# antonilo/unsupervised_detection

Measured on AMD Instinct MI355X. Metric: frame-pairs/sec per adversarial step, DAVIS 480p batch4, 1/2/4/8 GPU, higher is better.
Workload: dtype f32

## Files before the change

include/udet_debug.h:

```cpp
#ifndef UDET_DEBUG_H
#define UDET_DEBUG_H
#include <stddef.h>
#ifdef __cplusplus
extern "C" {
#endif
void udet_debug_force_conv(int bm, int bn, int ks);
void udet_debug_conv_fp16(int on);
void udet_debug_conv_fp16_grad_scale(float s);
void udet_debug_force_wgrad(int nsplit, int dma);
int udet_debug_last_wgrad(void);
int udet_debug_last_wgrad_reduce(void);
int udet_debug_conv2d_backward_filter_ex(const float* x, int ldx, int x_coff, const float* dy, int ldy, int y_coff, const float* y_saved, int act,
                                         float alpha, const float* w, const float* b, const float* gamma, float bn_c, float* dw, float* db,
                                         float* dgamma, float* dbeta, int n, int h, int wd, int cin, int cout, int k, int stride, int dilation,
                                         int up, void* workspace, size_t workspace_bytes, void* stream);
void udet_debug_upb_min_pixels(long v);
void udet_debug_set_tuning(int on);
void udet_debug_force_pair(int on);
int udet_debug_last_pair(void);
int udet_debug_conv2d_pair(const float* xa, const float* xb, const float* wa, const float* wb, const float* ba, const float* bb, float* ya, float* yb,
                           int na, int nb, int h, int w, int cin, int cout, int k, int stride, int dilation, int act, float alpha, void* workspace,
                           size_t workspace_bytes, void* stream);
#define UDET_DEBUG_UPCONV_WSETS_OFFSET 6400
size_t udet_debug_upconv_lowres_workspace_bytes(int ldx, int cin, int cout);
int udet_debug_upconv_lowres_fwd(const float* x, int ldx, const float* w, const float* bias, int act, float alpha, float* y, int ldy, int y_coff,
                                 float* xhat, int n, int h, int wd, int cin, int cout, int split, void* workspace, size_t workspace_bytes,
                                 void* stream);
int udet_debug_upconv_lowres_bwd(const float* dy, int ldy, int y_coff, const float* w, float* dx, int ldx, float* dxhat, int n, int h, int wd,
                                 int cin, int cout, void* workspace, size_t workspace_bytes, void* stream);
int udet_debug_upconv_tables(int h, int w, int backward, int* nseg, int* seg, int* seg_tap, int* taps, int taps_cap, int* ntaps);
int udet_debug_max_segs(void);
int udet_debug_last_conv(void);
#ifdef __cplusplus
}
#endif
#endif
```

unsupervised_detection_amd/_devel.py:

```python
from __future__ import annotations

import ctypes
import os

from ._ffi import check as _check, lib as _lib

_PATH = os.path.join(os.path.dirname(os.path.abspath(__file__)), "libudet_debug.so")
if not os.path.exists(_PATH):
    raise RuntimeError(f"{_PATH} is missing: build it with `make -C unsupervised_detection_amd/csrc`")
dbg = ctypes.CDLL(_PATH, mode=ctypes.RTLD_GLOBAL)
dbg.udet_debug_force_conv.restype = None
dbg.udet_debug_force_conv.argtypes = [ctypes.c_int, ctypes.c_int, ctypes.c_int]
dbg.udet_debug_last_conv.restype = ctypes.c_int
dbg.udet_debug_last_conv.argtypes = []
dbg.udet_debug_conv_fp16.restype = None
dbg.udet_debug_conv_fp16.argtypes = [ctypes.c_int]
dbg.udet_debug_conv_fp16_grad_scale.restype = None
dbg.udet_debug_conv_fp16_grad_scale.argtypes = [ctypes.c_float]
dbg.udet_debug_force_wgrad.restype = None
dbg.udet_debug_force_wgrad.argtypes = [ctypes.c_int, ctypes.c_int]
dbg.udet_debug_upb_min_pixels.restype = None
dbg.udet_debug_upb_min_pixels.argtypes = [ctypes.c_long]
dbg.udet_debug_set_tuning.restype = None
dbg.udet_debug_set_tuning.argtypes = [ctypes.c_int]
dbg.udet_debug_last_wgrad.restype = ctypes.c_int
dbg.udet_debug_last_wgrad.argtypes = []
dbg.udet_debug_force_pair.restype = None
dbg.udet_debug_force_pair.argtypes = [ctypes.c_int]
dbg.udet_debug_last_pair.restype = ctypes.c_int
dbg.udet_debug_last_pair.argtypes = []
dbg.udet_debug_conv2d_pair.restype = ctypes.c_int
dbg.udet_debug_conv2d_pair.argtypes = [ctypes.c_void_p] * 8 + [ctypes.c_int] * 10 + [ctypes.c_float, ctypes.c_void_p, ctypes.c_size_t, ctypes.c_void_p]
dbg.udet_debug_last_wgrad_reduce.restype = ctypes.c_int
dbg.udet_debug_last_wgrad_reduce.argtypes = []
_p, _i, _f = ctypes.c_void_p, ctypes.c_int, ctypes.c_float
dbg.udet_debug_conv2d_backward_filter_ex.restype = ctypes.c_int
dbg.udet_debug_conv2d_backward_filter_ex.argtypes = ([_p, _i, _i, _p, _i, _i, _p, _i, _f, _p, _p, _p, _f, _p, _p, _p, _p] + [_i] * 9
                                                     + [_p, ctypes.c_size_t, _p])
UPCONV_WSETS_OFFSET = 6400
dbg.udet_debug_upconv_lowres_workspace_bytes.restype = ctypes.c_size_t
dbg.udet_debug_upconv_lowres_workspace_bytes.argtypes = [_i, _i, _i]
dbg.udet_debug_upconv_lowres_fwd.restype = ctypes.c_int
dbg.udet_debug_upconv_lowres_fwd.argtypes = [_p, _i, _p, _p, _i, _f, _p, _i, _i, _p] + [_i] * 6 + [_p, ctypes.c_size_t, _p]
dbg.udet_debug_upconv_lowres_bwd.restype = ctypes.c_int
dbg.udet_debug_upconv_lowres_bwd.argtypes = [_p, _i, _i, _p, _p, _i, _p] + [_i] * 5 + [_p, ctypes.c_size_t, _p]
dbg.udet_debug_upconv_tables.restype = ctypes.c_int
dbg.udet_debug_upconv_tables.argtypes = [_i, _i, _i] + [_p] * 4 + [_i, _p]
dbg.udet_debug_max_segs.restype = ctypes.c_int
dbg.udet_debug_max_segs.argtypes = []


def upconv_tables(h: int, w: int, backward: bool):
    cap = 1024
    nseg, ntaps = ctypes.c_int(0), ctypes.c_int(0)
    seg, seg_tap, taps = (ctypes.c_int * 64)(), (ctypes.c_int * 17)(), (ctypes.c_int * (3 * cap))()
    st = dbg.udet_debug_upconv_tables(h, w, 1 if backward else 0, ctypes.addressof(nseg), ctypes.addressof(seg), ctypes.addressof(seg_tap),
                                      ctypes.addressof(taps), cap, ctypes.addressof(ntaps))
    _check(st)
    ns, nt = nseg.value, ntaps.value
    return dict(nseg=ns, seg=[tuple(seg[4 * s:4 * s + 4]) for s in range(ns)], seg_tap=list(seg_tap[:ns + 1]),
                taps=[tuple(taps[3 * t:3 * t + 3]) for t in range(nt)])
```

unsupervised_detection_amd/csrc/api_plan.hip:

```cpp
#include <stdlib.h>
#include <string.h>

#include "conv_host.h"
#include "elementwise.h"
#include "plan.h"

using namespace udet;

struct udet_plan {
  Plan* p;
};

extern "C" {

int udet_plan_create(const udet_config* c, udet_plan** out) {
  if (!c || !out) { set_error("plan_create: null argument"); return UDET_ERR_ARG; }
  Config k;
  k.batch = c->batch; k.in_h = c->in_h; k.in_w = c->in_w; k.img_h = c->img_h; k.img_w = c->img_w;
  k.flow_normalizer = c->flow_normalizer; k.cbn = c->cbn; k.epsilon = c->epsilon;
  k.lr = c->lr; k.beta1 = c->beta1; k.beta2 = c->beta2; k.adam_eps = c->adam_eps; k.clip = c->clip;
  k.noise_seed = c->noise_seed;
  k.conv_fp16 = c->conv_fp16 ? 1 : 0;
  Plan* P = plan_build(k);
  if (!P) return UDET_ERR_SHAPE;
  *out = new udet_plan{P};
  return UDET_OK;
}
void udet_plan_destroy(udet_plan* h) {
  if (h) { delete h->p; delete h; }
}
size_t udet_workspace_bytes(const udet_plan* h) { return h->p->arena_floats * sizeof(float); }
int udet_plan_init(udet_plan* h, void* ws, void* stream) { return plan_init_workspace(h->p, (float*)ws, (hipStream_t)stream); }

int udet_param_count(int net) { return (net < 0 || net > 2) ? 0 : (int)net_params(net).p.size(); }
size_t udet_param_total(int net) { return (net < 0 || net > 2) ? 0 : net_params(net).total; }
int udet_param_info(int net, int i, const char** name, int* rank, int* shape, size_t* offset) {
  if (net < 0 || net > 2 || i < 0 || i >= (int)net_params(net).p.size()) { set_error("param_info: out of range"); return UDET_ERR_ARG; }
  const ParamDesc& d = net_params(net).p[i];
  *name = d.name.c_str(); *rank = d.rank; *offset = d.offset;
  for (int k = 0; k < 4; ++k) shape[k] = d.shape[k];
  return UDET_OK;
}
int udet_buffer_count(const udet_plan* h) { return (int)h->p->bufs.size(); }
int udet_buffer_info(const udet_plan* h, int i, const char** name, size_t* offset_bytes, int* dims) {
  if (i < 0 || i >= (int)h->p->bufs.size()) { set_error("buffer_info: out of range"); return UDET_ERR_ARG; }
  const Buf& b = h->p->bufs[i];
  *name = b.name.c_str(); *offset_bytes = b.off * sizeof(float);
  dims[0] = b.n; dims[1] = b.h; dims[2] = b.w; dims[3] = b.ld;
  return UDET_OK;
}
int udet_plan_set_concurrent(udet_plan* h, int on) {
  if (!h) { set_error("plan_set_concurrent: null plan"); return UDET_ERR_ARG; }
  if (on)
    if (h->p->cand.empty()) { set_error("plan_set_concurrent: the plan has no side streams"); return UDET_ERR_UNSUPPORTED; }
  h->p->concurrent = on != 0;
  return UDET_OK;
}
int udet_plan_lane_queues(udet_plan* h, void* stream, int* queue) {
  if (!h || !queue) { set_error("plan_lane_queues: null argument"); return UDET_ERR_ARG; }
  return plan_lane_queues(h->p, (hipStream_t)stream, queue);
}
int udet_plan_pin_lanes(udet_plan* h, void* stream, void* const* side_streams, int n) {
  if (!h || (n > 0 && !side_streams)) { set_error("plan_pin_lanes: null argument"); return UDET_ERR_ARG; }
  return plan_pin_lanes(h->p, (hipStream_t)stream, reinterpret_cast<hipStream_t const*>(side_streams), n);
}
long udet_fp16_overflow_count(udet_plan* h) {
  if (!h) return 0;
  (void)plan_check_overflow(h->p, true);
  return h->p->ovf_skipped;
}
long udet_get_adam_step(const udet_plan* h) {
  plan_settle_adam_step(h->p);
  return h->p->adam_t;
}
void udet_set_adam_step(udet_plan* h, long t) {
  plan_settle_adam_step(h->p);
  h->p->adam_t = t;
}

int udet_pack_pwc(udet_plan* h, const float* w_pwc, void* ws, void* stream) {
  return plan_pack_pwc(h->p, w_pwc, (float*)ws, (hipStream_t)stream);
}
int udet_pack_trainable(udet_plan* h, const float* w_gen, const float* w_rec, void* ws, void* stream) {
  return plan_pack_trainable(h->p, w_gen, w_rec, (float*)ws, (hipStream_t)stream);
}
int udet_pwc_forward(udet_plan* h, const float* img1, const float* img2, void* ws, void* stream) {
  return plan_pwc_forward(h->p, img1, img2, (float*)ws, (hipStream_t)stream);
}
int udet_forward_from_flow(udet_plan* h, int ncalls, void* ws, void* stream) {
  UDET_TRY(plan_check_overflow(h->p, false));
  if (ncalls < 0 || ncalls > 3) { set_error("forward: ncalls must be 0..3"); return UDET_ERR_ARG; }
  return plan_forward(h->p, nullptr, nullptr, ncalls, (float*)ws, (hipStream_t)stream);
}
int udet_generator_forward(udet_plan* h, void* ws, void* stream) {
  UDET_TRY(plan_generator_forward(h->p, (float*)ws, (hipStream_t)stream));
  return plan_recover_forward(h->p, 0, (float*)ws, (hipStream_t)stream);
}
int udet_generator_layers(udet_plan* h, void* ws, void* stream) {
  h->p->ev_next = 0;
  UDET_TRY(plan_generator_layers(h->p, (float*)ws, (hipStream_t)stream));
  return plan_recover_forward(h->p, 0, (float*)ws, (hipStream_t)stream);
}
int udet_recover_forward(udet_plan* h, int n, void* ws, void* stream) {
  if (n < 1 || n > 3) { set_error("recover_forward: n must be 1..3 (multiples of the plan batch)"); return UDET_ERR_ARG; }
  return plan_recover_forward(h->p, n, (float*)ws, (hipStream_t)stream, true);
}
int udet_forward(udet_plan* h, const float* img1, const float* img2, int ncalls, void* ws, void* stream) {
  UDET_TRY(plan_check_overflow(h->p, false));
  if (ncalls < 0 || ncalls > 3) { set_error("forward: ncalls must be 0..3"); return UDET_ERR_ARG; }
  if (!img1 || !img2) { set_error("forward: null image pointer"); return UDET_ERR_ARG; }
  return plan_forward(h->p, img1, img2, ncalls, (float*)ws, (hipStream_t)stream);
}
int udet_prefetch_flow(udet_plan* h, const float* img1, const float* img2, void* ws, void* stream) {
  if (!img1 || !img2) { set_error("prefetch_flow: null image pointer"); return UDET_ERR_ARG; }
  return plan_prefetch(h->p, img1, img2, (float*)ws, (hipStream_t)stream);
}
int udet_prefetch_consume(udet_plan* h, void* ws, void* stream) {
  return plan_prefetch_consume(h->p, (float*)ws, (hipStream_t)stream);
}
int udet_forward_prefetched(udet_plan* h, int ncalls, void* ws, void* stream) {
  UDET_TRY(plan_check_overflow(h->p, false));
  if (ncalls < 0 || ncalls > 3) { set_error("forward: ncalls must be 0..3"); return UDET_ERR_ARG; }
  return plan_forward(h->p, nullptr, nullptr, ncalls, (float*)ws, (hipStream_t)stream, true);
}
int udet_backward(udet_plan* h, int which, const float* w_gen, const float* w_rec, float* g_gen, float* g_rec, void* ws,
                  void* stream) {
  UDET_TRY(plan_check_overflow(h->p, false));
  if (which < 1 || which > 3) { set_error("backward: which must be 1 (generator), 2 (recover) or 3 (both)"); return UDET_ERR_ARG; }
  return plan_backward(h->p, which, w_gen, w_rec, g_gen, g_rec, (float*)ws, (hipStream_t)stream);
}
int udet_apply(udet_plan* h, int net, float* w, float* g, float* m, float* v, void* ws, void* stream) {
  return plan_apply(h->p, net, w, g, m, v, (float*)ws, (hipStream_t)stream);
}
int udet_train_step(udet_plan* h, int which, const float* img1, const float* img2, float* w_gen, float* w_rec, float* g_gen,
                    float* g_rec, float* m_gen, float* v_gen, float* m_rec, float* v_rec, void* ws, void* stream) {
  UDET_TRY(udet_pack_trainable(h, w_gen, w_rec, ws, stream));
  UDET_TRY(udet_forward(h, img1, img2, 3, ws, stream));
  UDET_TRY(udet_backward(h, which, w_gen, w_rec, g_gen, g_rec, ws, stream));
  if (which & 1) UDET_TRY(udet_apply(h, NET_GEN, w_gen, g_gen, m_gen, v_gen, ws, stream));
  if (which & 2) UDET_TRY(udet_apply(h, NET_REC, w_rec, g_rec, m_rec, v_rec, ws, stream));
  return UDET_OK;
}

int udet_autotune(udet_plan* h, const float* w_gen, const float* w_rec, float* g_gen, float* g_rec, void* ws_, void* stream) {
  Plan* P = h->p;
  float* ws = (float*)ws_;
  hipStream_t s = (hipStream_t)stream;
  if (!P->pwc_packed) { set_error("autotune: pack the PWC-Net and trainable weights first"); return UDET_ERR_ARG; }
  const size_t lo = P->packed_floats, hi = P->small_off;
  UDET_TRY(launch_fill_uniform(ws + lo, (long)(hi - lo), 0x5eedull, -0.5f, 0.5f, s));
  const size_t img_floats = (size_t)P->cfg.batch * P->cfg.in_h * P->cfg.in_w * 3;
  if (P->wgrad_floats < 2 * img_floats) { set_error("autotune: workspace too small for the probe images"); return UDET_ERR_ARG; }
  const float* img1 = ws + P->wgrad_off[0];
  const float* img2 = img1 + img_floats;
  const bool was_concurrent = P->concurrent;
  P->concurrent = false;
  conv_set_tuning(1);
  wgrad_set_tuning(1);
  int rc = udet_forward(h, img1, img2, 3, ws_, stream);
  if (rc == UDET_OK) rc = udet_backward(h, 3, w_gen, w_rec, g_gen, g_rec, ws_, stream);
  conv_set_tuning(0);
  wgrad_set_tuning(0);
  P->concurrent = was_concurrent;
  UDET_HIP(hipMemsetAsync(ws + lo, 0, (hi - lo) * sizeof(float), s));
  UDET_HIP(hipStreamSynchronize(s));
  return rc;
}
int udet_tuned_shapes(void) { return tuned_shapes(); }
int udet_tune_save(const char* path) {
  FILE* f = path ? fopen(path, "w") : nullptr;
  if (!f) { set_error("tune_save: cannot open %s", path ? path : "(null)"); return UDET_ERR_ARG; }
  fprintf(f, "udet-tune 2 abi %d\n", UDET_TUNE_ABI);
  tune_dump(f);
  fclose(f);
  return UDET_OK;
}
int udet_tune_load(const char* path) {
  FILE* f = path ? fopen(path, "r") : nullptr;
  if (!f) { set_error("tune_load: cannot open %s", path ? path : "(null)"); return UDET_ERR_ARG; }
  char line[256];
  int n = 0, ver = 0, abi = -1;
  if (!fgets(line, sizeof(line), f) || sscanf(line, "udet-tune %d abi %d", &ver, &abi) != 2 || ver != 2 || abi != UDET_TUNE_ABI) {
    fclose(f);
    set_error("tune_load: %s is not a udet-tune 2 file of this build (abi %d)", path, UDET_TUNE_ABI);
    return UDET_ERR_ARG;
  }
  while (fgets(line, sizeof(line), f)) n += tune_put_line(line) ? 1 : 0;
  fclose(f);
  return n;
}

int udet_profile_begin(udet_plan* h) {
  for (auto* r : h->p->prof) delete r;
  h->p->prof.clear();
  h->p->profiling = true;
  return UDET_OK;
}
int udet_profile_end(udet_plan* h, double* out, int ncat, void* stream) {
  Plan* P = h->p;
  P->profiling = false;
  g_launch_sink = nullptr;
  UDET_HIP(hipStreamSynchronize((hipStream_t)stream));
  for (int i = 0; i < ncat * 5; ++i) out[i] = 0.0;
  FILE* dump = nullptr;
  if (const char* path = getenv("UDET_PROF_DUMP")) dump = fopen(path, "a");
  for (auto* r : P->prof) {
    float wall = 0.f;
    (void)hipEventElapsedTime(&wall, r->a, r->b);
    double kern = 0.0;
    std::string each;
    for (int k = 0; k < r->sink.n; ++k) {
      float ms = 0.f;
      if (hipEventElapsedTime(&ms, r->kev[2 * k], r->kev[2 * k + 1]) == hipSuccess) kern += ms;
      char buf[32];
      snprintf(buf, sizeof(buf), "%s%.1f", k ? "+" : "", ms * 1e3f);
      each += buf;
      (void)hipEventDestroy(r->kev[2 * k]);
      (void)hipEventDestroy(r->kev[2 * k + 1]);
    }
    if (r->sink.n == 0) kern = wall;
    if (dump)
      fprintf(dump, "%d,%s,%.4f,%.4f,%.4f,%.4f,%d,%s,%.4f\n", r->cat, r->name.c_str(), kern, r->flops * 1e-9, r->bytes * 1e-6, wall, r->sink.n,
              each.c_str(), r->flops * r->mfma_scale * 1e-9);
    if (r->cat < ncat) {
      out[r->cat * 5 + 0] += 1.0;
      out[r->cat * 5 + 1] += kern;
      out[r->cat * 5 + 2] += r->flops;
      out[r->cat * 5 + 3] += r->bytes;
      out[r->cat * 5 + 4] += wall;
    }
    (void)hipEventDestroy(r->a);
    (void)hipEventDestroy(r->b);
    delete r;
  }
  if (dump) fclose(dump);
  P->prof.clear();
  return UDET_OK;
}

int udet_generator_backward(udet_plan* h, const float* w_gen, float* g_gen, void* ws, void* stream) {
  if (!w_gen || !g_gen) { set_error("generator_backward: null argument"); return UDET_ERR_ARG; }
  return plan_backward(h->p, 1, w_gen, nullptr, g_gen, nullptr, (float*)ws, (hipStream_t)stream);
}
int udet_recover_backward(udet_plan* h, const float* w_rec, float* g_rec, void* ws, void* stream) {
  if (!w_rec || !g_rec) { set_error("recover_backward: null argument"); return UDET_ERR_ARG; }
  return plan_backward(h->p, 2, nullptr, w_rec, nullptr, g_rec, (float*)ws, (hipStream_t)stream);
}
int udet_grad_absmean(udet_plan* h, int net, const float* g, float* out2, void* ws_, void* stream) {
  if ((net != NET_GEN && net != NET_REC) || !g || !out2) { set_error("grad_absmean: net must be 1 or 2, g / out2 non-null"); return UDET_ERR_ARG; }
  Plan* P = h->p;
  float* ws = (float*)ws_;
  const NetParams& np = net_params(net);
  const long* tab = reinterpret_cast<const long*>(ws + P->seg_off[net]);
  return launch_grad_absmean(g, tab, tab + np.p.size(), (int)np.p.size(), ws + P->small_off + 2048, 1e-5f, out2, (hipStream_t)stream);
}
int udet_stream_wait_grads(udet_plan* h, int net, void* stream) {
  if (net != NET_GEN && net != NET_REC) { set_error("stream_wait_grads: net must be 1 or 2"); return UDET_ERR_ARG; }
  if (!h->p->grad_ev[net]) { set_error("stream_wait_grads: no udet_backward has produced that gradient yet"); return UDET_ERR_ARG; }
  UDET_HIP(hipStreamWaitEvent((hipStream_t)stream, h->p->grad_ev[net], 0));
  return UDET_OK;
}
int udet_tune_rejected(void) { return conv_tune_rejected(); }

}
```

unsupervised_detection_amd/csrc/devel/api_debug.hip:

```cpp
#include <string.h>

#include <vector>

#include "../../../include/udet_debug.h"
#include "../conv_host.h"
#include "../plan_run.h"

using namespace udet;

extern "C" {
int udet_debug_last_conv(void) { return conv_last_config(); }
void udet_debug_force_conv(int bm, int bn, int ks) { conv_force_config(bm, bn, ks); }
void udet_debug_conv_fp16(int on) { conv_debug_f16(on); }
void udet_debug_conv_fp16_grad_scale(float s) { conv_debug_f16_grad_scale(s); }
void udet_debug_force_wgrad(int nsplit, int dma) { wgrad_force(nsplit, dma); }
int udet_debug_last_wgrad(void) { return wgrad_last_config(); }
int udet_debug_last_wgrad_reduce(void) { return wgrad_last_reduce(); }
int udet_debug_conv2d_backward_filter_ex(const float* x, int ldx, int x_coff, const float* dy, int ldy, int y_coff, const float* y_saved, int act,
                                         float alpha, const float* w, const float* b, const float* gamma, float bn_c, float* dw, float* db,
                                         float* dgamma, float* dbeta, int n, int h, int wd, int cin, int cout, int k, int stride, int dilation,
                                         int up, void* workspace, size_t workspace_bytes, void* stream_) {
  hipStream_t stream = (hipStream_t)stream_;
  if (!x || !dy || !dw || n < 1 || h < 1 || wd < 1 || cin < 1 || cout < 1 || k < 1 || k * k > UDET_MAX_TAPS || dilation < 1 ||
      (stride != 1 && stride != 2) || up < 0 || up > 2) {
    set_error("debug_backward_filter_ex: bad argument");
    return UDET_ERR_ARG;
  }
  if (ldx % 4 || x_coff % 4 || ldy % 4 || y_coff % 4) {
    set_error("debug_backward_filter_ex: ldx=%d x_coff=%d ldy=%d y_coff=%d must be multiples of 4", ldx, x_coff, ldy, y_coff);
    return UDET_ERR_ALIGN;
  }
  if (x_coff < 0 || y_coff < 0 || x_coff + round_up(cin, 4) > ldx || y_coff + round_up(cout, 4) > ldy) {
    set_error("debug_backward_filter_ex: channel window outside the buffer (x %d+%d of %d, dy %d+%d of %d)", x_coff, cin, ldx, y_coff, cout, ldy);
    return UDET_ERR_SHAPE;
  }
  if (gamma && (!w || !b || !db || !dgamma || !dbeta)) {
    set_error("debug_backward_filter_ex: a BN-folded layer needs w, b, db, dgamma and dbeta");
    return UDET_ERR_ARG;
  }
  if (up == 2 && (!gamma || y_saved || k != 3 || stride != 1 || dilation != 1)) {
    set_error("debug_backward_filter_ex: the class-structured form is a BN-folded 3x3 stride-1 layer on dU");
    return UDET_ERR_ARG;
  }
  if (!workspace || (reinterpret_cast<uintptr_t>(workspace) & 63) || workspace_bytes < 128 * sizeof(float)) {
    set_error("debug_backward_filter_ex: workspace must be 64-byte aligned and hold the zero block");
    return UDET_ERR_ARG;
  }
  float* zero = reinterpret_cast<float*>(workspace);
  const int us = up ? 1 : 0;
  WgradParams p;
  memset(&p, 0, sizeof(p));
  p.x = x; p.ldx = ldx; p.x_coff = x_coff; p.N = n; p.Cin = cin;
  p.dy = dy; p.ldy = ldy; p.y_coff = y_coff; p.Cout = cout;
  if (y_saved && act != UDET_ACT_NONE) { p.ya = y_saved; p.yact = act; p.yalpha = alpha; }
  p.dw = dw; p.db = db;
  p.partial = zero + 64; p.partial_floats = workspace_bytes / sizeof(float) - 64;
  p.zero16 = zero;
  p.f16_yscale = conv_debug_f16_grad_scale_now();
  if (gamma) { p.w = w; p.b = b; p.gamma = gamma; p.dgamma = dgamma; p.dbeta = dbeta; p.bn_c = bn_c; }
  ConvParams g;
  memset(&g, 0, sizeof(g));
  conv_setup_fwd(g, n, h << us, wd << us, k, k, stride, dilation);
  p.H = h << us; p.W = wd << us; p.up_shift = us;
  p.OH = g.OH; p.OW = g.OW; p.isy = p.isx = stride;
  p.ntaps = g.ntaps;
  memcpy(p.taps, g.taps, sizeof(g.taps));
  UDET_HIP(hipMemsetAsync(zero, 0, 64 * sizeof(float), stream));
  if (up == 2) return launch_wgrad_up_T(p, h, wd, stream);
  return launch_wgrad_T(p, k * k, stream);
}
void udet_debug_upb_min_pixels(long v) { plan_debug_upb_min_pixels(v); }
void udet_debug_force_pair(int on) { conv_force_pair(on); }
int udet_debug_last_pair(void) { return conv_last_pair(); }
int udet_debug_conv2d_pair(const float* xa, const float* xb, const float* wa, const float* wb, const float* ba, const float* bb, float* ya, float* yb,
                           int na, int nb, int h, int w, int cin, int cout, int k, int stride, int dilation, int act, float alpha, void* workspace,
                           size_t workspace_bytes, void* stream_) {
  hipStream_t stream = (hipStream_t)stream_;
  if (cin % 8 != 0 || k * k > UDET_MAX_TAPS) { set_error("debug_conv2d_pair: cin must be a multiple of 8"); return UDET_ERR_SHAPE; }
  const int kc = cin, ldw = round_up(cout, 4);
  const size_t wfl = ((size_t)k * k * kc * ldw + 63) & ~(size_t)63, part_fl = (size_t)4 << 20, zero_fl = 64 + UDET_MAX_TICKETS;
  if (workspace_bytes < (2 * wfl + part_fl + zero_fl) * sizeof(float)) { set_error("debug_conv2d_pair: workspace too small"); return UDET_ERR_ARG; }
  float* wpa = reinterpret_cast<float*>(workspace);
  float* wpb = wpa + wfl;
  float* part = wpb + wfl;
  float* zero = part + part_fl;
  UDET_HIP(hipMemsetAsync(zero, 0, zero_fl * sizeof(float), stream));
  UDET_TRY(launch_pack_weights(wa, wpa, k * k, cin, cout, kc, ldw, kc, 0, 0, nullptr, stream));
  UDET_TRY(launch_pack_weights(wb, wpb, k * k, cin, cout, kc, ldw, kc, 0, 0, nullptr, stream));
  ConvParams p[2];
  for (int i = 0; i < 2; ++i) {
    memset(&p[i], 0, sizeof(ConvParams));
    conv_setup_fwd(p[i], i ? nb : na, h, w, k, k, stride, dilation);
    p[i].x = i ? xb : xa; p[i].ldx = cin; p[i].wp = i ? wpb : wpa; p[i].Kc = kc; p[i].ldw = ldw; p[i].bias = i ? bb : ba;
    p[i].y = i ? yb : ya; p[i].ldy = cout; p[i].Cout = cout; p[i].act = act; p[i].alpha = alpha;
    p[i].partial = part; p[i].partial_cap = part_fl; p[i].zero16 = zero; p[i].tickets = reinterpret_cast<int*>(zero + 64);
  }
  return launch_conv_pair(p[0], p[1], stream);
}
}
namespace {
enum { UPC_TICKETS = 64, UPC_JOBS = UPC_TICKETS + UDET_MAX_TICKETS, UPC_JOBS_CAP = 192, UPC_TAB = UPC_JOBS + UPC_JOBS_CAP, UPC_TAB_CAP = 2048,
       UPC_WSETS = UPC_TAB + UPC_TAB_CAP, UPC_MIN_SLAB = 1 << 20 };
static_assert(UPC_WSETS == UDET_DEBUG_UPCONV_WSETS_OFFSET && UPC_WSETS % 64 == 0 && 8 * sizeof(PackJob) <= UPC_JOBS_CAP * sizeof(float), "workspace layout");
size_t upc_align64(size_t v) { return (v + 63) & ~(size_t)63; }
int upc_kct(int cout) { return round_up(cout, cout <= 4 ? 4 : 8); }
size_t upc_floats(int kc, int ldw) { return UPC_WSETS + upc_align64((size_t)4 * 36 * kc * ldw) + UPC_MIN_SLAB; }
int upc_check(const char* who, const void* a, const void* b, const void* c, const void* d, int n, int h, int wd, int cin, int cout, void* workspace,
              size_t workspace_bytes, size_t need_floats) {
  if (!a || !b || !c || !d || n < 1 || cin < 1 || cout < 1) { set_error("%s: bad argument", who); return UDET_ERR_ARG; }
  if (h < 2 || wd < 2) { set_error("%s: the source grid %d x %d must be at least 2 x 2 (one interior row / column and the last one)", who, h, wd); return UDET_ERR_SHAPE; }
  if ((long)n * (2 * h) * (2 * wd) >= (1L << 28)) { set_error("%s: grid too large", who); return UDET_ERR_SHAPE; }
  if (!workspace || (reinterpret_cast<uintptr_t>(workspace) & 63) || workspace_bytes < need_floats * sizeof(float)) {
    set_error("%s: workspace must be 64-byte aligned and hold %zu bytes", who, need_floats * sizeof(float));
    return UDET_ERR_ARG;
  }
  return UDET_OK;
}
int upc_stage(const Layer::SegLaunch& tab, const std::vector<PackJob>& jobs, const float* w, float* ws, hipStream_t stream) {
  if (tab.taps.size() * sizeof(ConvTap) > UPC_TAB_CAP * sizeof(float) || jobs.size() * sizeof(PackJob) > UPC_JOBS_CAP * sizeof(float)) {
    set_error("debug_upconv_lowres: table larger than its workspace slot");
    return UDET_ERR_ARG;
  }
  UDET_HIP(hipMemsetAsync(ws, 0, UPC_JOBS * sizeof(float), stream));
  UDET_HIP(hipMemcpyAsync(ws + UPC_JOBS, jobs.data(), jobs.size() * sizeof(PackJob), hipMemcpyHostToDevice, stream));
  UDET_HIP(hipMemcpyAsync(ws + UPC_TAB, tab.taps.data(), tab.taps.size() * sizeof(ConvTap), hipMemcpyHostToDevice, stream));
  return launch_pack_jobs(reinterpret_cast<const PackJob*>(ws + UPC_JOBS), (int)jobs.size(), w, ws, BN_C, stream);
}
UpbLane upc_lane(float* ws, size_t ws_floats, size_t sets_floats) {
  const size_t off = UPC_WSETS + upc_align64(sets_floats);
  return UpbLane{ws + off, ws_floats - off, ws, reinterpret_cast<int*>(ws + UPC_TICKETS), 0};
}
}
extern "C" {

size_t udet_debug_upconv_lowres_workspace_bytes(int ldx, int cin, int cout) {
  if (ldx < 1 || cin < 1 || cout < 1) return 0;
  const size_t f = upc_floats(ldx, round_up(cout, 4)), b = upc_floats(upc_kct(cout), round_up(cin, 4));
  return (f > b ? f : b) * sizeof(float);
}
int udet_debug_max_segs(void) { return UDET_MAX_SEGS; }

int udet_debug_upconv_lowres_fwd(const float* x, int ldx, const float* w, const float* bias, int act, float alpha, float* y, int ldy, int y_coff,
                                 float* xhat, int n, int h, int wd, int cin, int cout, int split, void* workspace, size_t workspace_bytes,
                                 void* stream_) {
  hipStream_t stream = (hipStream_t)stream_;
  const char* who = "debug_upconv_lowres_fwd";
  if (act != UDET_ACT_NONE && act != UDET_ACT_LEAKY && act != UDET_ACT_ELU) { set_error("%s: bad argument", who); return UDET_ERR_ARG; }
  if (ldx % 4 || ldy % 4 || y_coff % 4) { set_error("%s: ldx=%d ldy=%d y_coff=%d must be multiples of 4", who, ldx, ldy, y_coff); return UDET_ERR_ALIGN; }
  if (ldx < 4 || ldy < 4 || cin > ldx || y_coff < 0 || (cout >= 1 && y_coff + cout > ldy)) {
    set_error("%s: channel window outside the buffer (x %d of %d, y %d+%d of %d)", who, cin, ldx, y_coff, cout, ldy);
    return UDET_ERR_SHAPE;
  }
  if (split && cout > 16) { set_error("%s: the split form is the plan's for cout <= 16 only", who); return UDET_ERR_ARG; }
  Layer L;
  L.cin = cin; L.cout = cout;
  L.Kc = ldx; L.ldw = round_up(cout, 4);
  L.k_split = round_up(cin, cin <= 4 ? 4 : 8); L.k_gap = 0;
  L.upb = true; L.upb_bwd = false; L.upb_split = split != 0;
  L.wupb_off = UPC_WSETS;
  const size_t sets = (size_t)4 * 36 * L.Kc * L.ldw;
  UDET_TRY(upc_check(who, x, w, y, xhat, n, h, wd, cin, cout, workspace, workspace_bytes, upc_floats(L.Kc, L.ldw)));
  float* ws = reinterpret_cast<float*>(workspace);
  build_upb_launches(L, h, wd);
  std::vector<PackJob> jobs;
  PackJob base;
  memset(&base, 0, sizeof(base));
  base.gamma_off = base.beta_off = -1;
  upb_pack_jobs(L, base, jobs);
  int st = upc_stage(L.upb_f, jobs, w, ws, stream);
  if (st == UDET_OK) {
    UpbFwd a;
    a.N = n; a.h = h; a.w = wd;
    a.src = x; a.xhat = xhat; a.ld = ldx;
    a.wsets = ws + L.wupb_off; a.Kc = L.Kc; a.ldw = L.ldw; a.bias = bias;
    a.y = y; a.ldy = ldy; a.y_coff = y_coff; a.cout = cout; a.act = act; a.alpha = alpha;
    a.tab = &L.upb_f; a.tab_dev = reinterpret_cast<const ConvTap*>(ws + UPC_TAB); a.split = L.upb_split;
    a.lane = upc_lane(ws, workspace_bytes / sizeof(float), sets);
    st = upb_forward(a, stream);
  }
  (void)hipStreamSynchronize(stream);
  return st;
}

int udet_debug_upconv_lowres_bwd(const float* dy, int ldy, int y_coff, const float* w, float* dx, int ldx, float* dxhat, int n, int h, int wd,
                                 int cin, int cout, void* workspace, size_t workspace_bytes, void* stream_) {
  hipStream_t stream = (hipStream_t)stream_;
  const char* who = "debug_upconv_lowres_bwd";
  if (ldx % 4 || ldy % 4 || y_coff % 4) { set_error("%s: ldx=%d ldy=%d y_coff=%d must be multiples of 4", who, ldx, ldy, y_coff); return UDET_ERR_ALIGN; }
  const int kct = cout >= 1 ? upc_kct(cout) : 0;
  if (ldx < 4 || ldy < 4 || cin > ldx || y_coff < 0 || y_coff + kct > ldy) {
    set_error("%s: channel window outside the buffer (dy %d+%d of %d, dx %d of %d)", who, y_coff, kct, ldy, cin, ldx);
    return UDET_ERR_SHAPE;
  }
  Layer L;
  L.cin = cin; L.cout = cout;
  L.Kc = ldx; L.ldw = round_up(cout, 4);
  L.k_split = round_up(cin, cin <= 4 ? 4 : 8); L.k_gap = 0;
  L.KcT = kct; L.ldwT = round_up(cin, 4);
  L.upb = true; L.upb_bwd = true;
  L.wupbT_off = UPC_WSETS;
  const size_t sets = (size_t)4 * 36 * L.KcT * L.ldwT;
  UDET_TRY(upc_check(who, dy, w, dx, dxhat, n, h, wd, cin, cout, workspace, workspace_bytes, upc_floats(L.KcT, L.ldwT)));
  float* ws = reinterpret_cast<float*>(workspace);
  build_upb_launches(L, h, wd);
  std::vector<PackJob> all, jobs;
  PackJob base;
  memset(&base, 0, sizeof(base));
  base.gamma_off = base.beta_off = -1;
  upb_pack_jobs(L, base, all);
  for (const PackJob& j : all)
    if (j.mode == 10) jobs.push_back(j);
  int st = upc_stage(L.upb_b, jobs, w, ws, stream);
  if (st == UDET_OK) {
    UpbBwd a;
    a.N = n; a.h = h; a.w = wd;
    a.du = dy; a.lddu = ldy; a.du_coff = y_coff;
    a.wsetsT = ws + L.wupbT_off; a.KcT = L.KcT; a.ldwT = L.ldwT; a.cout = cout;
    a.dxhat = dxhat; a.dsrc = dx; a.ld = ldx; a.cin = cin;
    a.tab = &L.upb_b; a.tab_dev = reinterpret_cast<const ConvTap*>(ws + UPC_TAB);
    a.lane = upc_lane(ws, workspace_bytes / sizeof(float), sets);
    a.f16_xscale = conv_debug_f16_grad_scale_now();
    st = upb_dgrad(a, stream);
  }
  (void)hipStreamSynchronize(stream);
  return st;
}

int udet_debug_upconv_tables(int h, int w, int backward, int* nseg, int* seg, int* seg_tap, int* taps, int taps_cap, int* ntaps) {
  if (!nseg || !seg || !seg_tap || !taps || !ntaps || taps_cap < 0) { set_error("debug_upconv_tables: bad argument"); return UDET_ERR_ARG; }
  if (h < 2 || w < 2) { set_error("debug_upconv_tables: the source grid %d x %d must be at least 2 x 2", h, w); return UDET_ERR_SHAPE; }
  Layer L;
  build_upb_launches(L, h, w);
  const Layer::SegLaunch& g = backward ? L.upb_b : L.upb_f;
  *nseg = g.nseg;
  *ntaps = (int)g.taps.size();
  if (*ntaps > taps_cap) { set_error("debug_upconv_tables: %d taps, room for %d", *ntaps, taps_cap); return UDET_ERR_ARG; }
  for (int s = 0; s < g.nseg; ++s) {
    seg[4 * s] = g.seg[s].oy; seg[4 * s + 1] = g.seg[s].ox; seg[4 * s + 2] = g.seg[s].h; seg[4 * s + 3] = g.seg[s].w;
    seg_tap[s] = g.seg_tap[s];
  }
  seg_tap[g.nseg] = g.seg_tap[g.nseg];
  for (int t = 0; t < *ntaps; ++t) { taps[3 * t] = g.taps[t].dy; taps[3 * t + 1] = g.taps[t].dx; taps[3 * t + 2] = g.taps[t].widx; }
  return UDET_OK;
}

void udet_debug_set_tuning(int on) {
  conv_set_tuning(on);
  wgrad_set_tuning(on);
}
}
```

unsupervised_detection_amd/csrc/elementwise.h:

```cpp
#pragma once
#include "common.h"
namespace udet {
int launch_resize_bilinear_fwd(const float* x, int ldx, int x_coff, int N, int H, int W, float* y, int ldy, int y_coff,
                               int OH, int OW, int C, float mul, float div, hipStream_t s);
int launch_resize_bilinear_bwd(const float* dy, int ldy, int y_coff, int N, int OH, int OW, float* dx, int ldx, int x_coff,
                               int H, int W, int C, int accumulate, hipStream_t s);
int launch_upb_ring(const float* x, int ld, int N, int H, int W, float* xh, hipStream_t s);
int launch_upb_ring_fold(const float* dxh, int ld, int N, int H, int W, float* dx, hipStream_t s);
int launch_share_samples(float* buf, long P, int ld, int coff, int C, int copies, hipStream_t s);
int launch_fold_samples(float* buf, long P, int ld, int coff, int C, int copies, hipStream_t s);
int launch_emit_du(const float* d, const float* a, float* u, long P, int ld, int coff, int C, int act, float alpha, hipStream_t s);
int launch_pool2x2_sum(const float* du, float* dx, int N, int H, int W, int C, hipStream_t s);
int launch_pack_pwc_input(const float* i1, const float* i2, float* x8, long P, hipStream_t s);
int launch_gen_input(const float* img, const float* f, double* part, float* gin, int B, long HW, hipStream_t s);
size_t flow_stats_doubles(int B);
int launch_mask_rec_inputs(const float* logits, const float* f, float* mask, float* fin, long P, int ncalls, hipStream_t s);
int launch_pack_imgin(const float* img, float* imgin, long P, int ncalls, hipStream_t s);
int launch_losses(const float* f, const float* mask, const float* pred, long HW, int B, float cbn, float eps,
                  float num_pixels, float* part, float* losses, float* coef, float* sums, hipStream_t s);
size_t loss_part_floats(int B);
int launch_rec_loss_bwd(const float* f, const float* mask, const float* pred, float* dpred, long BHW, float cbn,
                        float inv_np, hipStream_t s);
int launch_gen_loss_bwd(const float* f, const float* mask, const float* pred, const float* coef, float* dpred,
                        float* dmask, long HW, int B, float cbn, hipStream_t s);
int launch_mask_bwd(const float* dmask, const float* dfin, const float* f, const float* mask, float* dlogits, long P,
                    hipStream_t s);
int launch_grad_absmean(const float* g, const long* seg_off, const long* seg_len, int nvars, float* vmean, float thresh,
                        float* out, hipStream_t s);
int launch_adam(float* w, float* g, float* m, float* v, long n, float lr_t, float b1, float b2, float eps, float clip,
                const float* flag, uint64_t seed, uint64_t step, hipStream_t s, int mode = 0, const int* skip = nullptr);
int launch_nonfinite_count(const float* g, long n, int* out, hipStream_t s);
int launch_flow_normalize(const float* f, double* part, float* out, int B, long HW, hipStream_t s);
int launch_charbonnier(const float* gt, const float* pred, const float* mask, int mc, int B, long HW, float cbn, float* part,
                       float* out, hipStream_t s);
int launch_crop_flip_resize(const void* src, int src_u8, int nearest, int N, int H, int W, int C, const int* prm, float* dst, int OH,
                            int OW, float div, float add, hipStream_t s);
int launch_crop_flip_resize_ragged(const void* src, int src_u8, int nearest, int N, int C, const long long* offsets, const int* hw,
                                   const int* prm, float* dst, int OH, int OW, float div, float add, hipStream_t s);
int launch_mask_stats(const float* pred, const float* gt, int N, int H, int W, float threshold, float gt_threshold, double* out,
                      hipStream_t s);
int launch_boundary_stats(const float* pred, const float* gt, const double* stats8, int N, int H, int W, float threshold,
                          float gt_threshold, int radius, unsigned long long* counts4, unsigned char* bmap_pred,
                          unsigned char* bmap_gt, hipStream_t s);
size_t restore_workspace_bytes(int n);
int launch_restore_masks_ragged(const float* masks, int n, int mh, int mw, const long long* offsets, const int* tab, const int* coef,
                                int max_h, int max_w, unsigned char* out, int* amax, unsigned char* binary, double threshold,
                                void* workspace, hipStream_t s);
size_t components_workspace_bytes(size_t total_pixels, int n);
int launch_select_components_ragged(const unsigned char* binary, const unsigned char* gt, int n, const long long* offsets, const int* hw,
                                    int max_h, int max_w, size_t total_pixels, int connectivity, int mode, int* labels,
                                    unsigned char* selected, long long* info, void* workspace, hipStream_t s);
size_t component_boxes_workspace_bytes(size_t total_pixels, int n);
int launch_component_boxes_ragged(const int* labels, const unsigned char* score, int n, const long long* offsets, const int* hw, int max_h,
                                  int max_w, size_t total_pixels, int min_area, int k, long long* dets, long long* counts, void* workspace,
                                  hipStream_t s);
int launch_draw_boxes_ragged(unsigned char* rgb, int n, const long long* offsets, const int* hw, const long long* dets,
                             const long long* counts, int k, int thickness, unsigned colour, hipStream_t s);
size_t link_detections_workspace_bytes(size_t total_pixels, int carry_h, int carry_w);
int launch_link_detections_ragged(const int* labels, int n, const long long* offsets, const int* hw, int max_h, int max_w,
                                  size_t total_pixels, const long long* dets, const long long* counts, int k, const int* link,
                                  const int* carry_labels, int carry_h, int carry_w, const long long* carry_dets,
                                  const long long* carry_counts, const int* carry_ids, const int* carry_next_id, int min_iou_permille,
                                  long long* inter, int* match, int* ids, int* linked, int* seq_tracks, int* next_id, void* workspace,
                                  hipStream_t s);
size_t link_detections_gap_workspace_bytes(size_t total_pixels, int m, int hist_h, int hist_w);
int launch_link_detections_gap_ragged(const int* labels, int n, const long long* offsets, const int* hw, int max_h, int max_w,
                                      size_t total_pixels, const long long* dets, const long long* counts, int k, const int* link,
                                      int max_gap, int m, const int* hist_labels, int hist_h, int hist_w, const long long* hist_dets,
                                      const long long* hist_counts, const int* hist_ids, int* hist_open, const int* hist_next_id,
                                      int min_iou_permille, long long* inter, int* match, int* ids, int* linked, int* seq_tracks,
                                      int* next_id, long long* gap_inter, int* back, int* prev, int* open, void* workspace,
                                      hipStream_t s);
int launch_draw_track_boxes_ragged(unsigned char* rgb, int n, const long long* offsets, const int* hw, const long long* dets,
                                   const long long* counts, int k, const int* ids, int thickness, const unsigned* palette,
                                   int palette_size, hipStream_t s);
int launch_fill_uniform(float* x, long n, uint64_t seed, float lo, float hi, hipStream_t s);
int launch_axpy(const float* x, float* y, long n, float a, int accumulate, hipStream_t s);
}
```

unsupervised_detection_amd/csrc/elementwise.hip:

```cpp
#include "common.h"
#include "elementwise.h"

namespace udet {

static inline int grid_for(long total, int cap = 4096) {
  long nb = (total + 255) / 256;
  if (nb > cap) nb = cap;
  if (nb < 1) nb = 1;
  return (int)nb;
}

template <typename T>
__device__ __forceinline__ T wave_sum(T v) {
#pragma unroll
  for (int o = 32; o > 0; o >>= 1) v += __shfl_down(v, o, 64);
  return v;
}
template <typename T>
__device__ __forceinline__ T block_sum(T v, T* sm ) {
  v = wave_sum(v);
  __syncthreads();
  if ((threadIdx.x & 63) == 0) sm[threadIdx.x >> 6] = v;
  __syncthreads();
  return sm[0] + sm[1] + sm[2] + sm[3];
}

__device__ __forceinline__ void legacy_coord(int i, float scale, int in, int& lo, int& hi, float& t) {
  const float src = (float)i * scale;
  lo = (int)src;
  hi = min(lo + 1, in - 1);
  t = src - (float)lo;
}

__global__ __launch_bounds__(256) void resize_bilinear_fwd_kernel(const float* __restrict__ x, int ldx, int x_coff, int N,
                                                                  int H, int W, float* __restrict__ y, int ldy, int y_coff,
                                                                  int OH, int OW, int C, float mul, float div) {
  const float sy = (float)H / (float)OH, sx = (float)W / (float)OW;
  const long total = (long)N * OH * OW * C;
  for (long e = (long)blockIdx.x * 256 + threadIdx.x; e < total; e += (long)gridDim.x * 256) {
    const int c = (int)(e % C);
    const long pix = e / C;
    const int ox = (int)(pix % OW), oy = (int)((pix / OW) % OH), n = (int)(pix / ((long)OW * OH));
    int y0, y1, x0, x1;
    float ty, tx;
    legacy_coord(oy, sy, H, y0, y1, ty);
    legacy_coord(ox, sx, W, x0, x1, tx);
    const float* b = x + x_coff + c;
    const float tl = b[(((long)n * H + y0) * W + x0) * ldx], tr = b[(((long)n * H + y0) * W + x1) * ldx];
    const float bl = b[(((long)n * H + y1) * W + x0) * ldx], br = b[(((long)n * H + y1) * W + x1) * ldx];
    const float top = tl + (tr - tl) * tx, bot = bl + (br - bl) * tx;
    float v = top + (bot - top) * ty;
    v = v * mul;
    if (div != 1.f) v = v / div;
    y[pix * ldy + y_coff + c] = v;
  }
}
template <typename T, int NEAREST>
__global__ __launch_bounds__(256) void crop_flip_resize_kernel(const T* __restrict__ src, int N, int H, int W, int C,
                                                               const int* __restrict__ prm, float* __restrict__ dst, int OH, int OW,
                                                               float div, float add) {
  const long total = (long)N * OH * OW * C;
  for (long e = (long)blockIdx.x * 256 + threadIdx.x; e < total; e += (long)gridDim.x * 256) {
    const int c = (int)(e % C);
    const long pix = e / C;
    const int ox = (int)(pix % OW), oy = (int)((pix / OW) % OH), n = (int)(pix / ((long)OW * OH));
    int y0 = 0, x0 = 0, ch = H, cw = W, flr = 0, ftd = 0;
    if (prm) { y0 = prm[n * 6]; x0 = prm[n * 6 + 1]; ch = prm[n * 6 + 2]; cw = prm[n * 6 + 3]; flr = prm[n * 6 + 4]; ftd = prm[n * 6 + 5]; }
    const float sy = (float)ch / (float)OH, sx = (float)cw / (float)OW;
    auto tap = [&](int cy, int cx) -> float {
      int yy = y0 + cy, xx = x0 + cx;
      if (ftd) yy = H - 1 - yy;
      if (flr) xx = W - 1 - xx;
      float v = (float)src[(((long)n * H + yy) * W + xx) * C + c];
      if (div != 1.f) v = v / div;
      return v + add;
    };
    float v;
    if (NEAREST) {
      const int cy = min((int)floorf((float)oy * sy), ch - 1), cx = min((int)floorf((float)ox * sx), cw - 1);
      v = tap(cy, cx);
    } else {
      int ly, hy, lx, hx;
      float ty, tx;
      legacy_coord(oy, sy, ch, ly, hy, ty);
      legacy_coord(ox, sx, cw, lx, hx, tx);
      const float tl = tap(ly, lx), tr = tap(ly, hx), bl = tap(hy, lx), br = tap(hy, hx);
      const float top = tl + (tr - tl) * tx, bot = bl + (br - bl) * tx;
      v = top + (bot - top) * ty;
    }
    dst[e] = v;
  }
}
int launch_crop_flip_resize(const void* src, int src_u8, int nearest, int N, int H, int W, int C, const int* prm, float* dst, int OH,
                            int OW, float div, float add, hipStream_t s) {
  const long total = (long)N * OH * OW * C;
  const dim3 g(grid_for(total, 8192)), b(256);
  if (src_u8 && nearest) hipLaunchKernelGGL((crop_flip_resize_kernel<unsigned char, 1>), g, b, 0, s, (const unsigned char*)src, N, H, W, C, prm, dst, OH, OW, div, add);
  else if (src_u8) hipLaunchKernelGGL((crop_flip_resize_kernel<unsigned char, 0>), g, b, 0, s, (const unsigned char*)src, N, H, W, C, prm, dst, OH, OW, div, add);
  else if (nearest) hipLaunchKernelGGL((crop_flip_resize_kernel<float, 1>), g, b, 0, s, (const float*)src, N, H, W, C, prm, dst, OH, OW, div, add);
  else hipLaunchKernelGGL((crop_flip_resize_kernel<float, 0>), g, b, 0, s, (const float*)src, N, H, W, C, prm, dst, OH, OW, div, add);
  UDET_HIP(hipGetLastError());
  return UDET_OK;
}

template <typename T, int NEAREST>
__global__ __launch_bounds__(256) void crop_flip_resize_ragged_kernel(const T* __restrict__ src, int N, int C,
                                                                      const long long* __restrict__ offsets, const int* __restrict__ hw,
                                                                      const int* __restrict__ prm, float* __restrict__ dst, int OH,
                                                                      int OW, float div, float add) {
  const long npix = (long)OH * OW;
  for (int n = blockIdx.y; n < N; n += gridDim.y) {
    const T* __restrict__ img = src + offsets[n];
    const int H = hw[n * 2], W = hw[n * 2 + 1];
    int y0 = 0, x0 = 0, ch = H, cw = W, flr = 0, ftd = 0;
    if (prm) { y0 = prm[n * 6]; x0 = prm[n * 6 + 1]; ch = prm[n * 6 + 2]; cw = prm[n * 6 + 3]; flr = prm[n * 6 + 4]; ftd = prm[n * 6 + 5]; }
    const float sy = (float)ch / (float)OH, sx = (float)cw / (float)OW;
    float* __restrict__ out = dst + (long)n * npix * C;
    for (long pix = (long)blockIdx.x * 256 + threadIdx.x; pix < npix; pix += (long)gridDim.x * 256) {
      const int ox = (int)(pix % OW), oy = (int)(pix / OW);
      auto tap = [&](int cy, int cx, int c) -> float {
        int yy = y0 + cy, xx = x0 + cx;
        if (ftd) yy = H - 1 - yy;
        if (flr) xx = W - 1 - xx;
        float v = (float)img[((long)yy * W + xx) * C + c];
        if (div != 1.f) v = v / div;
        return v + add;
      };
      if (NEAREST) {
        const int cy = min((int)floorf((float)oy * sy), ch - 1), cx = min((int)floorf((float)ox * sx), cw - 1);
        for (int c = 0; c < C; ++c) out[pix * C + c] = tap(cy, cx, c);
      } else {
        int ly, hy, lx, hx;
        float ty, tx;
        legacy_coord(oy, sy, ch, ly, hy, ty);
        legacy_coord(ox, sx, cw, lx, hx, tx);
        for (int c = 0; c < C; ++c) {
          const float tl = tap(ly, lx, c), tr = tap(ly, hx, c), bl = tap(hy, lx, c), br = tap(hy, hx, c);
          const float top = tl + (tr - tl) * tx, bot = bl + (br - bl) * tx;
          out[pix * C + c] = top + (bot - top) * ty;
        }
      }
    }
  }
}
int launch_crop_flip_resize_ragged(const void* src, int src_u8, int nearest, int N, int C, const long long* offsets, const int* hw,
                                   const int* prm, float* dst, int OH, int OW, float div, float add, hipStream_t s) {
  const int gy = N < 65535 ? N : 65535;
  const dim3 g(grid_for((long)OH * OW, 1024), gy), b(256);
  if (src_u8 && nearest) hipLaunchKernelGGL((crop_flip_resize_ragged_kernel<unsigned char, 1>), g, b, 0, s, (const unsigned char*)src, N, C, offsets, hw, prm, dst, OH, OW, div, add);
  else if (src_u8) hipLaunchKernelGGL((crop_flip_resize_ragged_kernel<unsigned char, 0>), g, b, 0, s, (const unsigned char*)src, N, C, offsets, hw, prm, dst, OH, OW, div, add);
  else if (nearest) hipLaunchKernelGGL((crop_flip_resize_ragged_kernel<float, 1>), g, b, 0, s, (const float*)src, N, C, offsets, hw, prm, dst, OH, OW, div, add);
  else hipLaunchKernelGGL((crop_flip_resize_ragged_kernel<float, 0>), g, b, 0, s, (const float*)src, N, C, offsets, hw, prm, dst, OH, OW, div, add);
  UDET_HIP(hipGetLastError());
  return UDET_OK;
}

__global__ __launch_bounds__(256) void resize_bilinear_fwd4_kernel(const float* __restrict__ x, int ldx, int x_coff, int N, int H,
                                                                   int W, float* __restrict__ y, int ldy, int y_coff, int OH,
                                                                   int OW, int C4, float mul, float div) {
  const float sy = (float)H / (float)OH, sx = (float)W / (float)OW;
  const long total = (long)N * OH * OW * C4;
  for (long e = (long)blockIdx.x * 256 + threadIdx.x; e < total; e += (long)gridDim.x * 256) {
    const int c4 = (int)(e % C4);
    const long pix = e / C4;
    const int ox = (int)(pix % OW), oy = (int)((pix / OW) % OH), n = (int)(pix / ((long)OW * OH));
    int y0, y1, x0, x1;
    float ty, tx;
    legacy_coord(oy, sy, H, y0, y1, ty);
    legacy_coord(ox, sx, W, x0, x1, tx);
    const float* b = x + x_coff + c4 * 4;
    const float4 tl = *reinterpret_cast<const float4*>(b + (((long)n * H + y0) * W + x0) * ldx);
    const float4 tr = *reinterpret_cast<const float4*>(b + (((long)n * H + y0) * W + x1) * ldx);
    const float4 bl = *reinterpret_cast<const float4*>(b + (((long)n * H + y1) * W + x0) * ldx);
    const float4 br = *reinterpret_cast<const float4*>(b + (((long)n * H + y1) * W + x1) * ldx);
    auto lerp = [&](float a, float bq, float c, float d) {
      const float top = a + (bq - a) * tx, bot = c + (d - c) * tx;
      float v = (top + (bot - top) * ty) * mul;
      if (div != 1.f) v = v / div;
      return v;
    };
    float4 o;
    o.x = lerp(tl.x, tr.x, bl.x, br.x);
    o.y = lerp(tl.y, tr.y, bl.y, br.y);
    o.z = lerp(tl.z, tr.z, bl.z, br.z);
    o.w = lerp(tl.w, tr.w, bl.w, br.w);
    *reinterpret_cast<float4*>(y + pix * ldy + y_coff + c4 * 4) = o;
  }
}
int launch_resize_bilinear_fwd(const float* x, int ldx, int x_coff, int N, int H, int W, float* y, int ldy, int y_coff,
                               int OH, int OW, int C, float mul, float div, hipStream_t s) {
  if (C % 4 == 0 && ldx % 4 == 0 && ldy % 4 == 0 && x_coff % 4 == 0 && y_coff % 4 == 0 &&
      !((reinterpret_cast<uintptr_t>(x) | reinterpret_cast<uintptr_t>(y)) & 15)) {
    const long total4 = (long)N * OH * OW * (C / 4);
    hipLaunchKernelGGL(resize_bilinear_fwd4_kernel, dim3(grid_for(total4, 8192)), dim3(256), 0, s, x, ldx, x_coff, N, H, W, y, ldy,
                       y_coff, OH, OW, C / 4, mul, div);
    UDET_HIP(hipGetLastError());
    return UDET_OK;
  }
  const long total = (long)N * OH * OW * C;
  hipLaunchKernelGGL(resize_bilinear_fwd_kernel, dim3(grid_for(total)), dim3(256), 0, s, x, ldx, x_coff, N, H, W, y, ldy,
                     y_coff, OH, OW, C, mul, div);
  UDET_HIP(hipGetLastError());
  return UDET_OK;
}

__device__ __forceinline__ float legacy_weight(int o, float scale, int in, int i) {
  int lo, hi;
  float t;
  legacy_coord(o, scale, in, lo, hi, t);
  float w = 0.f;
  if (lo == i) w += 1.f - t;
  if (hi == i) w += t;
  return w;
}
__global__ __launch_bounds__(256) void resize_bilinear_bwd_kernel(const float* __restrict__ dy, int ldy, int y_coff, int N,
                                                                  int OH, int OW, float* __restrict__ dx, int ldx,
                                                                  int x_coff, int H, int W, int C, int accumulate) {
  const float sy = (float)H / (float)OH, sx = (float)W / (float)OW;
  const float isy = (float)OH / (float)H, isx = (float)OW / (float)W;
  const long total = (long)N * H * W * C;
  for (long e = (long)blockIdx.x * 256 + threadIdx.x; e < total; e += (long)gridDim.x * 256) {
    const int c = (int)(e % C);
    const long pix = e / C;
    const int ix = (int)(pix % W), iy = (int)((pix / W) % H), n = (int)(pix / ((long)W * H));
    const int oy_lo = max(0, (int)floorf((float)(iy - 1) * isy) - 1), oy_hi = min(OH - 1, (int)ceilf((float)(iy + 1) * isy) + 1);
    const int ox_lo = max(0, (int)floorf((float)(ix - 1) * isx) - 1), ox_hi = min(OW - 1, (int)ceilf((float)(ix + 1) * isx) + 1);
    float acc = 0.f;
    for (int oy = oy_lo; oy <= oy_hi; ++oy) {
      const float wy = legacy_weight(oy, sy, H, iy);
      if (wy == 0.f) continue;
      for (int ox = ox_lo; ox <= ox_hi; ++ox) {
        const float wx = legacy_weight(ox, sx, W, ix);
        if (wx == 0.f) continue;
        acc += wy * wx * dy[(((long)n * OH + oy) * OW + ox) * ldy + y_coff + c];
      }
    }
    float* d = dx + pix * ldx + x_coff + c;
    *d = accumulate ? *d + acc : acc;
  }
}
__global__ __launch_bounds__(256) void resize2x_bwd4_kernel(const float* __restrict__ dy, int ldy, int y_coff, int N, int H, int W,
                                                            float* __restrict__ dx, int ldx, int x_coff, int C4, int accumulate) {
  const int OH = 2 * H, OW = 2 * W;
  const long total = (long)N * H * W * C4;
  for (long e = (long)blockIdx.x * 256 + threadIdx.x; e < total; e += (long)gridDim.x * 256) {
    const int c4 = (int)(e % C4);
    const long pix = e / C4;
    const int ix = (int)(pix % W), iy = (int)((pix / W) % H), n = (int)(pix / ((long)W * H));
    float wy[3], wx[3];
    wy[0] = iy > 0 ? 0.5f : 0.f; wy[1] = 1.f; wy[2] = iy == H - 1 ? 1.f : 0.5f;
    wx[0] = ix > 0 ? 0.5f : 0.f; wx[1] = 1.f; wx[2] = ix == W - 1 ? 1.f : 0.5f;
    float4 acc = make_float4(0.f, 0.f, 0.f, 0.f);
#pragma unroll
    for (int a = 0; a < 3; ++a) {
      const int oy = 2 * iy - 1 + a;
      if (oy < 0) continue;
#pragma unroll
      for (int b = 0; b < 3; ++b) {
        const int ox = 2 * ix - 1 + b;
        if (ox < 0) continue;
        const float w = wy[a] * wx[b];
        const float4 g = *reinterpret_cast<const float4*>(dy + (((long)n * OH + oy) * OW + ox) * ldy + y_coff + c4 * 4);
        acc.x += w * g.x; acc.y += w * g.y; acc.z += w * g.z; acc.w += w * g.w;
      }
    }
    float4* d = reinterpret_cast<float4*>(dx + pix * ldx + x_coff + c4 * 4);
    if (accumulate) { const float4 o = *d; acc.x += o.x; acc.y += o.y; acc.z += o.z; acc.w += o.w; }
    *d = acc;
  }
}
int launch_resize_bilinear_bwd(const float* dy, int ldy, int y_coff, int N, int OH, int OW, float* dx, int ldx, int x_coff,
                               int H, int W, int C, int accumulate, hipStream_t s) {
  if (OH == 2 * H && OW == 2 * W && C % 4 == 0 && ldx % 4 == 0 && ldy % 4 == 0 && x_coff % 4 == 0 && y_coff % 4 == 0 &&
      !((reinterpret_cast<uintptr_t>(dx) | reinterpret_cast<uintptr_t>(dy)) & 15)) {
    const long total4 = (long)N * H * W * (C / 4);
    hipLaunchKernelGGL(resize2x_bwd4_kernel, dim3(grid_for(total4, 8192)), dim3(256), 0, s, dy, ldy, y_coff, N, H, W, dx, ldx, x_coff,
                       C / 4, accumulate);
    UDET_HIP(hipGetLastError());
    return UDET_OK;
  }
  const long total = (long)N * H * W * C;
  hipLaunchKernelGGL(resize_bilinear_bwd_kernel, dim3(grid_for(total)), dim3(256), 0, s, dy, ldy, y_coff, N, OH, OW, dx,
                     ldx, x_coff, H, W, C, accumulate);
  UDET_HIP(hipGetLastError());
  return UDET_OK;
}

__global__ __launch_bounds__(256) void pool2x2_sum_kernel(const float* __restrict__ du, float* __restrict__ dx, int N, int H,
                                                          int W, int C) {
  const int c4n = C >> 2;
  const long total = (long)N * H * W * c4n;
  for (long e = (long)blockIdx.x * 256 + threadIdx.x; e < total; e += (long)gridDim.x * 256) {
    const int c4 = (int)(e % c4n);
    const long pix = e / c4n;
    const int x = (int)(pix % W), y = (int)((pix / W) % H), n = (int)(pix / ((long)W * H));
    const float* b = du + ((((long)n * 2 * H + 2 * y) * 2 * W) + 2 * x) * C + c4 * 4;
    const float4 a0 = *reinterpret_cast<const float4*>(b), a1 = *reinterpret_cast<const float4*>(b + C);
    const float4 a2 = *reinterpret_cast<const float4*>(b + (long)2 * W * C), a3 = *reinterpret_cast<const float4*>(b + (long)2 * W * C + C);
    float4 o;
    o.x = (a0.x + a1.x) + (a2.x + a3.x);
    o.y = (a0.y + a1.y) + (a2.y + a3.y);
    o.z = (a0.z + a1.z) + (a2.z + a3.z);
    o.w = (a0.w + a1.w) + (a2.w + a3.w);
    *reinterpret_cast<float4*>(dx + pix * C + c4 * 4) = o;
  }
}
int launch_pool2x2_sum(const float* du, float* dx, int N, int H, int W, int C, hipStream_t s) {
  hipLaunchKernelGGL(pool2x2_sum_kernel, dim3(grid_for((long)N * H * W * (C / 4))), dim3(256), 0, s, du, dx, N, H, W, C);
  UDET_HIP(hipGetLastError());
  return UDET_OK;
}

__global__ __launch_bounds__(256) void emit_du_kernel(const float* __restrict__ d, const float* __restrict__ a,
                                                      float* __restrict__ u, long P, int ld, int coff, int C, int act,
                                                      float alpha) {
  const long total = P * C;
  for (long e = (long)blockIdx.x * 256 + threadIdx.x; e < total; e += (long)gridDim.x * 256) {
    const long pix = e / C;
    const long o = pix * ld + coff + (e - pix * C);
    u[o] = d[o] * act_dfo(a[o], act, alpha);
  }
}
int launch_emit_du(const float* d, const float* a, float* u, long P, int ld, int coff, int C, int act, float alpha, hipStream_t s) {
  hipLaunchKernelGGL(emit_du_kernel, dim3(grid_for(P * C)), dim3(256), 0, s, d, a, u, P, ld, coff, C, act, alpha);
  UDET_HIP(hipGetLastError());
  return UDET_OK;
}

template <int V, bool FOLD>
__global__ __launch_bounds__(256) void share_fold_kernel(float* __restrict__ buf, long P, int ld, int coff, int C, int copies) {
  const int CV = C / V;
  const long total = P * CV;
  for (long e = (long)blockIdx.x * 256 + threadIdx.x; e < total; e += (long)gridDim.x * 256) {
    const long pix = e / CV;
    const long o = pix * ld + coff + (e - pix * CV) * V;
    if (V == 4) {
      float4 v = *reinterpret_cast<const float4*>(buf + o);
      for (int k = 1; k < copies; ++k) {
        float4* q = reinterpret_cast<float4*>(buf + o + (long)k * P * ld);
        if (FOLD) {
          const float4 w = *q;
          v.x += w.x; v.y += w.y; v.z += w.z; v.w += w.w;
        } else {
          *q = v;
        }
      }
      if (FOLD) *reinterpret_cast<float4*>(buf + o) = v;
    } else {
      float v = buf[o];
      for (int k = 1; k < copies; ++k) {
        if (FOLD) v += buf[o + (long)k * P * ld];
        else buf[o + (long)k * P * ld] = v;
      }
      if (FOLD) buf[o] = v;
    }
  }
}
static int launch_share_fold(float* buf, long P, int ld, int coff, int C, int copies, bool fold, hipStream_t s) {
  if (copies < 2 || C < 1) return UDET_OK;
  const bool v4 = (ld % 4 == 0) && (coff % 4 == 0) && (C % 4 == 0);
  const long n = P * (v4 ? C / 4 : C);
  if (v4) {
    if (fold) hipLaunchKernelGGL((share_fold_kernel<4, true>), dim3(grid_for(n)), dim3(256), 0, s, buf, P, ld, coff, C, copies);
    else hipLaunchKernelGGL((share_fold_kernel<4, false>), dim3(grid_for(n)), dim3(256), 0, s, buf, P, ld, coff, C, copies);
  } else {
    if (fold) hipLaunchKernelGGL((share_fold_kernel<1, true>), dim3(grid_for(n)), dim3(256), 0, s, buf, P, ld, coff, C, copies);
    else hipLaunchKernelGGL((share_fold_kernel<1, false>), dim3(grid_for(n)), dim3(256), 0, s, buf, P, ld, coff, C, copies);
  }
  UDET_HIP(hipGetLastError());
  return UDET_OK;
}
int launch_share_samples(float* buf, long P, int ld, int coff, int C, int copies, hipStream_t s) {
  return launch_share_fold(buf, P, ld, coff, C, copies, false, s);
}
int launch_fold_samples(float* buf, long P, int ld, int coff, int C, int copies, hipStream_t s) {
  return launch_share_fold(buf, P, ld, coff, C, copies, true, s);
}

__global__ __launch_bounds__(256) void pack_pwc_input_kernel(const float* __restrict__ i1, const float* __restrict__ i2,
                                                             float* __restrict__ x8, long P) {
  for (long e = (long)blockIdx.x * 256 + threadIdx.x; e < 2 * P; e += (long)gridDim.x * 256) {
    const float* s = e < P ? i1 + e * 3 : i2 + (e - P) * 3;
    float4 a = make_float4(s[0] + 0.5f, s[1] + 0.5f, s[2] + 0.5f, 0.f);
    *reinterpret_cast<float4*>(x8 + e * 4) = a;
  }
}
int launch_pack_pwc_input(const float* i1, const float* i2, float* x8, long P, hipStream_t s) {
  hipLaunchKernelGGL(pack_pwc_input_kernel, dim3(grid_for(2 * P)), dim3(256), 0, s, i1, i2, x8, P);
  UDET_HIP(hipGetLastError());
  return UDET_OK;
}

#define FS_BLOCKS 32
__global__ __launch_bounds__(256) void flow_stats_kernel(const float* __restrict__ f, long HW, double* __restrict__ part) {
  __shared__ double sm[4];
  const int n = blockIdx.y;
  double s0 = 0, s1 = 0, q0 = 0, q1 = 0;
  for (long p = (long)blockIdx.x * 256 + threadIdx.x; p < HW; p += (long)gridDim.x * 256) {
    const float2 v = *reinterpret_cast<const float2*>(f + ((long)n * HW + p) * 2);
    s0 += v.x; s1 += v.y;
    q0 += (double)v.x * v.x; q1 += (double)v.y * v.y;
  }
  s0 = block_sum(s0, sm); s1 = block_sum(s1, sm); q0 = block_sum(q0, sm); q1 = block_sum(q1, sm);
  if (threadIdx.x == 0) {
    double* o = part + ((long)n * FS_BLOCKS + blockIdx.x) * 4;
    o[0] = s0; o[1] = s1; o[2] = q0; o[3] = q1;
  }
}
__global__ __launch_bounds__(256) void pack_gen_input_kernel(const float* __restrict__ img, const float* __restrict__ f,
                                                             const double* __restrict__ part, float* __restrict__ gin,
                                                             long HW) {
  __shared__ float st[4];
  const int n = blockIdx.y;
  if (threadIdx.x < 2) {
    double s = 0, q = 0;
    for (int b = 0; b < FS_BLOCKS; ++b) {
      s += part[((long)n * FS_BLOCKS + b) * 4 + threadIdx.x];
      q += part[((long)n * FS_BLOCKS + b) * 4 + 2 + threadIdx.x];
    }
    const double mean = s / (double)HW, var = q / (double)HW - mean * mean;
    st[threadIdx.x] = (float)mean;
    st[2 + threadIdx.x] = sqrtf((float)var);
  }
  __syncthreads();
  const float m0 = st[0], m1 = st[1], d0 = st[2], d1 = st[3];
  for (long p = (long)blockIdx.x * 256 + threadIdx.x; p < HW; p += (long)gridDim.x * 256) {
    const long q = (long)n * HW + p;
    const float2 v = *reinterpret_cast<const float2*>(f + q * 2);
    *reinterpret_cast<float4*>(gin + q * 8) = make_float4(img[q * 3], img[q * 3 + 1], img[q * 3 + 2], (v.x - m0) / d0);
    *reinterpret_cast<float4*>(gin + q * 8 + 4) = make_float4((v.y - m1) / d1, 0.f, 0.f, 0.f);
  }
}
int launch_gen_input(const float* img, const float* f, double* part, float* gin, int B, long HW, hipStream_t s) {
  hipLaunchKernelGGL(flow_stats_kernel, dim3(FS_BLOCKS, B), dim3(256), 0, s, f, HW, part);
  hipLaunchKernelGGL(pack_gen_input_kernel, dim3(grid_for(HW, 256), B), dim3(256), 0, s, img, f, part, gin, HW);
  UDET_HIP(hipGetLastError());
  return UDET_OK;
}
size_t flow_stats_doubles(int B) { return (size_t)B * FS_BLOCKS * 4; }
__global__ __launch_bounds__(256) void flow_normalize_kernel(const float* __restrict__ f, const double* __restrict__ part,
                                                             float* __restrict__ out, long HW) {
  __shared__ float st[4];
  const int n = blockIdx.y;
  if (threadIdx.x < 2) {
    double s = 0, q = 0;
    for (int b = 0; b < FS_BLOCKS; ++b) {
      s += part[((long)n * FS_BLOCKS + b) * 4 + threadIdx.x];
      q += part[((long)n * FS_BLOCKS + b) * 4 + 2 + threadIdx.x];
    }
    const double mean = s / (double)HW, var = q / (double)HW - mean * mean;
    st[threadIdx.x] = (float)mean;
    st[2 + threadIdx.x] = sqrtf((float)var);
  }
  __syncthreads();
  const float m0 = st[0], m1 = st[1], d0 = st[2], d1 = st[3];
  for (long p = (long)blockIdx.x * 256 + threadIdx.x; p < HW; p += (long)gridDim.x * 256) {
    const long q = (long)n * HW + p;
    const float2 v = *reinterpret_cast<const float2*>(f + q * 2);
    *reinterpret_cast<float2*>(out + q * 2) = make_float2((v.x - m0) / d0, (v.y - m1) / d1);
  }
}
int launch_flow_normalize(const float* f, double* part, float* out, int B, long HW, hipStream_t s) {
  hipLaunchKernelGGL(flow_stats_kernel, dim3(FS_BLOCKS, B), dim3(256), 0, s, f, HW, part);
  hipLaunchKernelGGL(flow_normalize_kernel, dim3(grid_for(HW, 256), B), dim3(256), 0, s, f, part, out, HW);
  UDET_HIP(hipGetLastError());
  return UDET_OK;
}

__global__ __launch_bounds__(256) void mask_rec_inputs_kernel(const float* __restrict__ logits ,
                                                              const float* __restrict__ f, float* __restrict__ mask,
                                                              float* __restrict__ fin, long P, int ncalls) {
  for (long q = (long)blockIdx.x * 256 + threadIdx.x; q < P; q += (long)gridDim.x * 256) {
    const float l0 = logits[q * 8] / 10.f, l1 = logits[q * 8 + 1] / 10.f;
    const float mx = fmaxf(l0, l1);
    const float e0 = expf(l0 - mx), e1 = expf(l1 - mx);
    const float m = e0 / (e0 + e1);
    mask[q] = m;
    const float cm = 1.f - m;
    const float2 v = *reinterpret_cast<const float2*>(f + q * 2);
    const float a0 = 1.f - m, a1 = 1.f - cm;
    if (ncalls > 0) {
      *reinterpret_cast<float4*>(fin + q * 4) = make_float4(v.x * a0, v.y * a0, 1.f, a0);
    }
    if (ncalls > 1) {
      *reinterpret_cast<float4*>(fin + (P + q) * 4) = make_float4(v.x * a1, v.y * a1, 1.f, a1);
    }
    if (ncalls > 2) {
      *reinterpret_cast<float4*>(fin + (2 * P + q) * 4) = make_float4(0.f, 0.f, 1.f, 0.f);
    }
  }
}
int launch_mask_rec_inputs(const float* logits, const float* f, float* mask, float* fin, long P, int ncalls, hipStream_t s) {
  hipLaunchKernelGGL(mask_rec_inputs_kernel, dim3(grid_for(P)), dim3(256), 0, s, logits, f, mask, fin, P, ncalls);
  UDET_HIP(hipGetLastError());
  return UDET_OK;
}
__global__ __launch_bounds__(256) void pack_imgin_kernel(const float* __restrict__ img, float* __restrict__ imgin, long P,
                                                         int ncalls) {
  for (long q = (long)blockIdx.x * 256 + threadIdx.x; q < P; q += (long)gridDim.x * 256) {
    const float4 im = make_float4(img[q * 3], img[q * 3 + 1], img[q * 3 + 2], 0.f);
    for (int k = 0; k < ncalls; ++k) *reinterpret_cast<float4*>(imgin + (k * P + q) * 4) = im;
  }
}
int launch_pack_imgin(const float* img, float* imgin, long P, int ncalls, hipStream_t s) {
  hipLaunchKernelGGL(pack_imgin_kernel, dim3(grid_for(P)), dim3(256), 0, s, img, imgin, P, ncalls);
  UDET_HIP(hipGetLastError());
  return UDET_OK;
}

__device__ __forceinline__ float charb(float e, float cbn) {
  const float s = e * e + 0.001f * 0.001f;
  return cbn == 0.5f ? sqrtf(s) : powf(s, cbn);
}
__device__ __forceinline__ float charb_d(float e, float cbn) {
  const float s = e * e + 0.001f * 0.001f;
  return cbn == 0.5f ? e / sqrtf(s) : cbn * powf(s, cbn - 1.f) * 2.f * e;
}
#define LS_BLOCKS 64
__global__ __launch_bounds__(256) void loss_sums_kernel(const float* __restrict__ f, const float* __restrict__ mask,
                                                        const float* __restrict__ pred , long HW, int B,
                                                        float cbn, float* __restrict__ part ) {
  __shared__ float sm[4];
  const int n = blockIdx.y;
  float R = 0, Rc = 0, Pp = 0, Dr = 0, Dc = 0;
  for (long p = (long)blockIdx.x * 256 + threadIdx.x; p < HW; p += (long)gridDim.x * 256) {
    const long q = (long)n * HW + p;
    const float2 fl = *reinterpret_cast<const float2*>(f + q * 2);
    const float2 a = *reinterpret_cast<const float2*>(pred + q * 2);
    const float2 b = *reinterpret_cast<const float2*>(pred + ((long)B * HW + q) * 2);
    const float2 c = *reinterpret_cast<const float2*>(pred + ((long)2 * B * HW + q) * 2);
    const float m = mask[q], cm = 1.f - m;
    const float pa = charb(fl.x - a.x, cbn) + charb(fl.y - a.y, cbn);
    const float pb = charb(fl.x - b.x, cbn) + charb(fl.y - b.y, cbn);
    const float pc = charb(fl.x - c.x, cbn) + charb(fl.y - c.y, cbn);
    R += pa * m; Rc += pb * cm; Pp += pc; Dr += pc * m; Dc += pc * cm;
  }
  R = block_sum(R, sm); Rc = block_sum(Rc, sm); Pp = block_sum(Pp, sm); Dr = block_sum(Dr, sm); Dc = block_sum(Dc, sm);
  if (threadIdx.x == 0) {
    float* o = part + ((long)n * LS_BLOCKS + blockIdx.x) * 5;
    o[0] = R; o[1] = Rc; o[2] = Pp; o[3] = Dr; o[4] = Dc;
  }
}
__global__ void loss_finish_kernel(const float* __restrict__ part, int B, float eps, float num_pixels,
                                   float* __restrict__ losses, float* __restrict__ coef, float* __restrict__ sums) {
  if (threadIdx.x != 0 || blockIdx.x != 0) return;
  float red = 0.f, redc = 0.f, rs = 0.f;
  for (int b = 0; b < B; ++b) {
    float v[5] = {0, 0, 0, 0, 0};
    for (int k = 0; k < LS_BLOCKS; ++k)
      for (int j = 0; j < 5; ++j) v[j] += part[((long)b * LS_BLOCKS + k) * 5 + j];
    const float D = v[3] + eps, Dc = v[4] + eps;
    red += 1.f - v[0] / D;
    redc += 1.f - v[1] / Dc;
    rs += v[0] + v[1] + v[2];
    coef[b * 4 + 0] = -1.f / (B * D);
    coef[b * 4 + 1] = v[0] / (B * D * D);
    coef[b * 4 + 2] = -1.f / (B * Dc);
    coef[b * 4 + 3] = v[1] / (B * Dc * Dc);
    for (int j = 0; j < 5; ++j) sums[b * 5 + j] = v[j];
    if (b == 0) { losses[4] = v[0]; losses[5] = v[1]; losses[6] = D; losses[7] = Dc; }
  }
  red /= B; redc /= B;
  losses[0] = red + redc;
  losses[1] = rs / num_pixels;
  losses[2] = red;
  losses[3] = redc;
}
int launch_losses(const float* f, const float* mask, const float* pred, long HW, int B, float cbn, float eps,
                  float num_pixels, float* part, float* losses, float* coef, float* sums, hipStream_t s) {
  hipLaunchKernelGGL(loss_sums_kernel, dim3(LS_BLOCKS, B), dim3(256), 0, s, f, mask, pred, HW, B, cbn, part);
  hipLaunchKernelGGL(loss_finish_kernel, dim3(1), dim3(64), 0, s, part, B, eps, num_pixels, losses, coef, sums);
  UDET_HIP(hipGetLastError());
  return UDET_OK;
}
size_t loss_part_floats(int B) { return (size_t)B * LS_BLOCKS * 5; }

__global__ __launch_bounds__(256) void charbonnier_sum_kernel(const float* __restrict__ gt, const float* __restrict__ pred,
                                                              const float* __restrict__ mask, int mc, long HW, float cbn,
                                                              float* __restrict__ part ) {
  __shared__ float sm[4];
  const int n = blockIdx.y;
  float acc = 0.f;
  for (long p = (long)blockIdx.x * 256 + threadIdx.x; p < HW; p += (long)gridDim.x * 256) {
    const long q = (long)n * HW + p;
    const float2 a = *reinterpret_cast<const float2*>(gt + q * 2);
    const float2 b = *reinterpret_cast<const float2*>(pred + q * 2);
    const float m0 = mask ? mask[q * mc] : 1.f, m1 = mask ? mask[q * mc + (mc - 1)] : 1.f;
    acc += charb(a.x - b.x, cbn) * m0 + charb(a.y - b.y, cbn) * m1;
  }
  acc = block_sum(acc, sm);
  if (threadIdx.x == 0) part[(long)n * LS_BLOCKS + blockIdx.x] = acc;
}
__global__ void charbonnier_finish_kernel(const float* __restrict__ part, int B, float* __restrict__ out) {
  const int b = blockIdx.x * blockDim.x + threadIdx.x;
  if (b >= B) return;
  float v = 0.f;
  for (int k = 0; k < LS_BLOCKS; ++k) v += part[(long)b * LS_BLOCKS + k];
  out[b] = v;
}
int launch_charbonnier(const float* gt, const float* pred, const float* mask, int mc, int B, long HW, float cbn, float* part,
                       float* out, hipStream_t s) {
  hipLaunchKernelGGL(charbonnier_sum_kernel, dim3(LS_BLOCKS, B), dim3(256), 0, s, gt, pred, mask, mc, HW, cbn, part);
  hipLaunchKernelGGL(charbonnier_finish_kernel, dim3((B + 63) / 64), dim3(64), 0, s, part, B, out);
  UDET_HIP(hipGetLastError());
  return UDET_OK;
}

__global__ __launch_bounds__(256) void rec_loss_bwd_kernel(const float* __restrict__ f, const float* __restrict__ mask,
                                                           const float* __restrict__ pred, float* __restrict__ dpred,
                                                           long BHW, float cbn, float inv_np) {
  for (long q = (long)blockIdx.x * 256 + threadIdx.x; q < BHW; q += (long)gridDim.x * 256) {
    const float2 fl = *reinterpret_cast<const float2*>(f + q * 2);
    const float m = mask[q], cm = 1.f - m;
    const float2 a = *reinterpret_cast<const float2*>(pred + q * 2);
    const float2 b = *reinterpret_cast<const float2*>(pred + (BHW + q) * 2);
    const float2 c = *reinterpret_cast<const float2*>(pred + (2 * BHW + q) * 2);
    *reinterpret_cast<float2*>(dpred + q * 2) = make_float2(-charb_d(fl.x - a.x, cbn) * m * inv_np, -charb_d(fl.y - a.y, cbn) * m * inv_np);
    *reinterpret_cast<float2*>(dpred + (BHW + q) * 2) = make_float2(-charb_d(fl.x - b.x, cbn) * cm * inv_np, -charb_d(fl.y - b.y, cbn) * cm * inv_np);
    *reinterpret_cast<float2*>(dpred + (2 * BHW + q) * 2) = make_float2(-charb_d(fl.x - c.x, cbn) * inv_np, -charb_d(fl.y - c.y, cbn) * inv_np);
  }
}
int launch_rec_loss_bwd(const float* f, const float* mask, const float* pred, float* dpred, long BHW, float cbn,
                        float inv_np, hipStream_t s) {
  hipLaunchKernelGGL(rec_loss_bwd_kernel, dim3(grid_for(BHW)), dim3(256), 0, s, f, mask, pred, dpred, BHW, cbn, inv_np);
  UDET_HIP(hipGetLastError());
  return UDET_OK;
}

__global__ __launch_bounds__(256) void gen_loss_bwd_kernel(const float* __restrict__ f, const float* __restrict__ mask,
                                                           const float* __restrict__ pred, const float* __restrict__ coef,
                                                           float* __restrict__ dpred, float* __restrict__ dmask, long HW,
                                                           int B, float cbn) {
  const long BHW = (long)B * HW;
  for (long q = (long)blockIdx.x * 256 + threadIdx.x; q < BHW; q += (long)gridDim.x * 256) {
    const int n = (int)(q / HW);
    const float cR = coef[n * 4], cD = coef[n * 4 + 1], cRc = coef[n * 4 + 2], cDc = coef[n * 4 + 3];
    const float2 fl = *reinterpret_cast<const float2*>(f + q * 2);
    const float m = mask[q], cm = 1.f - m;
    const float2 a = *reinterpret_cast<const float2*>(pred + q * 2);
    const float2 b = *reinterpret_cast<const float2*>(pred + (BHW + q) * 2);
    const float2 c = *reinterpret_cast<const float2*>(pred + (2 * BHW + q) * 2);
    *reinterpret_cast<float2*>(dpred + q * 2) = make_float2(-cR * charb_d(fl.x - a.x, cbn) * m, -cR * charb_d(fl.y - a.y, cbn) * m);
    *reinterpret_cast<float2*>(dpred + (BHW + q) * 2) = make_float2(-cRc * charb_d(fl.x - b.x, cbn) * cm, -cRc * charb_d(fl.y - b.y, cbn) * cm);
    const float pa = charb(fl.x - a.x, cbn) + charb(fl.y - a.y, cbn);
    const float pb = charb(fl.x - b.x, cbn) + charb(fl.y - b.y, cbn);
    const float pc = charb(fl.x - c.x, cbn) + charb(fl.y - c.y, cbn);
    dmask[q] = cR * pa + cD * pc - cRc * pb - cDc * pc;
  }
}
int launch_gen_loss_bwd(const float* f, const float* mask, const float* pred, const float* coef, float* dpred,
                        float* dmask, long HW, int B, float cbn, hipStream_t s) {
  hipLaunchKernelGGL(gen_loss_bwd_kernel, dim3(grid_for((long)B * HW)), dim3(256), 0, s, f, mask, pred, coef, dpred, dmask,
                     HW, B, cbn);
  UDET_HIP(hipGetLastError());
  return UDET_OK;
}

__global__ __launch_bounds__(256) void mask_bwd_kernel(const float* __restrict__ dmask, const float* __restrict__ dfin,
                                                       const float* __restrict__ f, const float* __restrict__ mask,
                                                       float* __restrict__ dlogits , long P) {
  for (long q = (long)blockIdx.x * 256 + threadIdx.x; q < P; q += (long)gridDim.x * 256) {
    const float4 g0 = *reinterpret_cast<const float4*>(dfin + q * 4);
    const float4 g1 = *reinterpret_cast<const float4*>(dfin + (P + q) * 4);
    const float2 fl = *reinterpret_cast<const float2*>(f + q * 2);
    float dm = dmask[q];
    dm -= g0.x * fl.x + g0.y * fl.y + g0.w;
    dm += g1.x * fl.x + g1.y * fl.y + g1.w;
    const float m = mask[q];
    const float d0 = dm * m * (1.f - m) / 10.f;
    dlogits[q * 8] = d0;
    dlogits[q * 8 + 1] = -d0;
  }
}
int launch_mask_bwd(const float* dmask, const float* dfin, const float* f, const float* mask, float* dlogits, long P,
                    hipStream_t s) {
  hipLaunchKernelGGL(mask_bwd_kernel, dim3(grid_for(P)), dim3(256), 0, s, dmask, dfin, f, mask, dlogits, P);
  UDET_HIP(hipGetLastError());
  return UDET_OK;
}

#define GA_SPLIT 8
__global__ __launch_bounds__(256) void grad_absmean_kernel(const float* __restrict__ g, const long* __restrict__ seg_off,
                                                           const long* __restrict__ seg_len, float* __restrict__ vpart) {
  __shared__ float sm[4];
  const long off = seg_off[blockIdx.x], len = seg_len[blockIdx.x];
  const long b = len * blockIdx.y / GA_SPLIT, e = len * (blockIdx.y + 1) / GA_SPLIT;
  float s0 = 0.f, s1 = 0.f, s2 = 0.f, s3 = 0.f;
  long i = b + threadIdx.x;
  for (; i + 768 < e; i += 1024) {
    s0 += fabsf(g[off + i]);
    s1 += fabsf(g[off + i + 256]);
    s2 += fabsf(g[off + i + 512]);
    s3 += fabsf(g[off + i + 768]);
  }
  for (; i < e; i += 256) s0 += fabsf(g[off + i]);
  const float s = block_sum((s0 + s1) + (s2 + s3), sm);
  if (threadIdx.x == 0) vpart[blockIdx.x * GA_SPLIT + blockIdx.y] = s;
}
__global__ void grad_flag_kernel(const float* __restrict__ vpart, const long* __restrict__ seg_len, int nvars, float thresh,
                                 float* __restrict__ out ) {
  if (threadIdx.x == 0 && blockIdx.x == 0) {
    float s = 0.f;
    for (int i = 0; i < nvars; ++i) {
      float v = 0.f;
      for (int j = 0; j < GA_SPLIT; ++j) v += vpart[i * GA_SPLIT + j];
      s += v / (float)seg_len[i];
    }
    s /= (float)nvars;
    out[0] = s;
    out[1] = s < thresh ? 1.f : 0.f;
  }
}
int launch_grad_absmean(const float* g, const long* seg_off, const long* seg_len, int nvars, float* vmean, float thresh,
                        float* out, hipStream_t s) {
  hipLaunchKernelGGL(grad_absmean_kernel, dim3(nvars, GA_SPLIT), dim3(256), 0, s, g, seg_off, seg_len, vmean);
  hipLaunchKernelGGL(grad_flag_kernel, dim3(1), dim3(64), 0, s, vmean, seg_len, nvars, thresh, out);
  UDET_HIP(hipGetLastError());
  return UDET_OK;
}

__device__ __host__ __forceinline__ float udet_uniform01(uint64_t seed, uint64_t step, uint64_t idx) {
  uint64_t z = seed * 0x9E3779B97F4A7C15ull + step * 0xBF58476D1CE4E5B9ull + idx + 0x94D049BB133111EBull;
  z = (z ^ (z >> 30)) * 0xBF58476D1CE4E5B9ull;
  z = (z ^ (z >> 27)) * 0x94D049BB133111EBull;
  z = z ^ (z >> 31);
  return (float)(z >> 40) * (1.0f / 16777216.0f);
}

__global__ __launch_bounds__(256) void adam_kernel(float* __restrict__ w, float* __restrict__ g, float* __restrict__ m,
                                                   float* __restrict__ v, long n, float lr_t, float b1, float b2, float eps,
                                                   float clip, const float* __restrict__ flag, uint64_t seed,
                                                   uint64_t step, int mode, const int* __restrict__ skip) {
  if (skip && *skip != 0) return;
  const bool noise = flag && flag[1] != 0.f;
  for (long i = (long)blockIdx.x * 256 + threadIdx.x; i < n; i += (long)gridDim.x * 256) {
    float gi = g[i];
    if (mode != 2) {
      if (noise) gi = fabsf((udet_uniform01(seed, step, (uint64_t)i) * 2.f - 1.f) * clip);
      else gi = fminf(fmaxf(gi, -clip), clip);
      g[i] = gi;
      if (mode == 1) continue;
    }
    const float mi = m[i] + (gi - m[i]) * (1.f - b1);
    const float vi = v[i] + (gi * gi - v[i]) * (1.f - b2);
    m[i] = mi;
    v[i] = vi;
    w[i] = w[i] - lr_t * mi / (sqrtf(vi) + eps);
  }
}
__global__ __launch_bounds__(256) void fill_uniform_kernel(float* __restrict__ x, long n, uint64_t seed, float lo, float hi) {
  for (long i = (long)blockIdx.x * 256 + threadIdx.x; i < n; i += (long)gridDim.x * 256)
    x[i] = lo + (hi - lo) * udet_uniform01(seed, 0, (uint64_t)i);
}
int launch_fill_uniform(float* x, long n, uint64_t seed, float lo, float hi, hipStream_t s) {
  hipLaunchKernelGGL(fill_uniform_kernel, dim3(grid_for(n, 8192)), dim3(256), 0, s, x, n, seed, lo, hi);
  UDET_HIP(hipGetLastError());
  return UDET_OK;
}
__global__ __launch_bounds__(256) void mask_stats_kernel(const float* __restrict__ pred, const float* __restrict__ gt, int H, int W,
                                                         float threshold, float gt_threshold, double* __restrict__ out) {
  __shared__ double sm[4];
  const int n = blockIdx.x;
  const long HW = (long)H * W;
  double v[8] = {0, 0, 0, 0, 0, 0, 0, 0};
  for (long q = threadIdx.x; q < HW; q += 256) {
    const int y = (int)(q / W), x = (int)(q - (long)y * W);
    const float g = gt[n * HW + q];
    const bool pr = pred[n * HW + q] > threshold, gb = g > gt_threshold;
    const int strips = (y < 2) + (y >= H - 2) + (x < 2) + (x >= W - 2);
    const double a1 = fabs((double)g - 1.0), a0 = fabs((double)g);
    if (pr) {
      v[0] += strips; v[1] += 1.0; v[4] += a1; v[7] += a0;
      if (gb) v[3] += 1.0;
    } else {
      v[5] += a0; v[6] += a1;
    }
    if (gb) v[2] += 1.0;
  }
  for (int k = 0; k < 8; ++k) {
    const double s = block_sum(v[k], sm);
    if (threadIdx.x == 0) out[(long)n * 8 + k] = s;
    __syncthreads();
  }
}
int launch_mask_stats(const float* pred, const float* gt, int N, int H, int W, float threshold, float gt_threshold, double* out,
                      hipStream_t s) {
  hipLaunchKernelGGL(mask_stats_kernel, dim3(N), dim3(256), 0, s, pred, gt, H, W, threshold, gt_threshold, out);
  UDET_HIP(hipGetLastError());
  return UDET_OK;
}
int launch_adam(float* w, float* g, float* m, float* v, long n, float lr_t, float b1, float b2, float eps, float clip,
                const float* flag, uint64_t seed, uint64_t step, hipStream_t s, int mode, const int* skip) {
  hipLaunchKernelGGL(adam_kernel, dim3(grid_for(n, 2048)), dim3(256), 0, s, w, g, m, v, n, lr_t, b1, b2, eps, clip, flag, seed,
                     step, mode, skip);
  UDET_HIP(hipGetLastError());
  return UDET_OK;
}
__global__ __launch_bounds__(256) void nonfinite_count_kernel(const float* __restrict__ g, long n, int* __restrict__ out) {
  int c = 0;
  for (long i = (long)blockIdx.x * 256 + threadIdx.x; i < n; i += (long)gridDim.x * 256) c += !(fabsf(g[i]) <= 3.402823466e38f);
#pragma unroll
  for (int o = 32; o > 0; o >>= 1) c += __shfl_xor(c, o);
  if ((threadIdx.x & 63) == 0 && c) {
    atomicAdd(out, c);
    atomicAdd(out + 1, c);
  }
}
int launch_nonfinite_count(const float* g, long n, int* out, hipStream_t s) {
  UDET_HIP(hipMemsetAsync(out, 0, sizeof(int), s));
  hipLaunchKernelGGL(nonfinite_count_kernel, dim3(grid_for(n, 1024)), dim3(256), 0, s, g, n, out);
  UDET_HIP(hipGetLastError());
  return UDET_OK;
}

__global__ __launch_bounds__(256) void upb_ring_kernel(const float* __restrict__ x, int ldx, int N, int H, int W, float* __restrict__ xh, int C4) {
  const int PH = H + 2, PW = W + 2;
  const long total = (long)N * PH * PW * C4;
  for (long e = (long)blockIdx.x * 256 + threadIdx.x; e < total; e += (long)gridDim.x * 256) {
    const int c4 = (int)(e % C4);
    const long pix = e / C4;
    const int C = (int)(pix % PW), R = (int)((pix / PW) % PH), n = (int)(pix / ((long)PW * PH));
    const int cy = R < 1 ? 0 : (R - 1 > H - 1 ? H - 1 : R - 1), cx = C < 1 ? 0 : (C - 1 > W - 1 ? W - 1 : C - 1);
    const float sg = ((R == 0) != (C == 0)) ? -1.f : 1.f;
    const float4 v = *reinterpret_cast<const float4*>(x + (((long)n * H + cy) * W + cx) * ldx + c4 * 4);
    *reinterpret_cast<float4*>(xh + pix * ldx + c4 * 4) = make_float4(v.x * sg, v.y * sg, v.z * sg, v.w * sg);
  }
}
int launch_upb_ring(const float* x, int ld, int N, int H, int W, float* xh, hipStream_t s) {
  const long total = (long)N * (H + 2) * (W + 2) * (ld / 4);
  hipLaunchKernelGGL(upb_ring_kernel, dim3(grid_for(total, 8192)), dim3(256), 0, s, x, ld, N, H, W, xh, ld / 4);
  UDET_HIP(hipGetLastError());
  return UDET_OK;
}
__global__ __launch_bounds__(256) void upb_ring_fold_kernel(const float* __restrict__ dxh, int ld, int N, int H, int W, float* __restrict__ dx, int C4) {
  const int PW = W + 2, PH = H + 2;
  const long total = (long)N * H * W * C4;
  for (long e = (long)blockIdx.x * 256 + threadIdx.x; e < total; e += (long)gridDim.x * 256) {
    const int c4 = (int)(e % C4);
    const long pix = e / C4;
    const int i = (int)(pix % W), j = (int)((pix / W) % H), n = (int)(pix / ((long)W * H));
    float4 a = make_float4(0.f, 0.f, 0.f, 0.f);
#pragma unroll
    for (int ry = 0; ry < 2; ++ry) {
      int R;
      float sy = 1.f;
      if (ry == 0) R = j + 1;
      else if (j == 0) { R = 0; sy = -1.f; }
      else if (j == H - 1) R = H + 1;
      else continue;
#pragma unroll
      for (int rx = 0; rx < 2; ++rx) {
        int C;
        float sx = 1.f;
        if (rx == 0) C = i + 1;
        else if (i == 0) { C = 0; sx = -1.f; }
        else if (i == W - 1) C = W + 1;
        else continue;
        const float4 v = *reinterpret_cast<const float4*>(dxh + (((long)n * PH + R) * PW + C) * ld + c4 * 4);
        const float sg = sy * sx;
        a.x += sg * v.x; a.y += sg * v.y; a.z += sg * v.z; a.w += sg * v.w;
      }
    }
    *reinterpret_cast<float4*>(dx + pix * ld + c4 * 4) = a;
  }
}
int launch_upb_ring_fold(const float* dxh, int ld, int N, int H, int W, float* dx, hipStream_t s) {
  if (H < 2 || W < 2) { set_error("upb_ring_fold: source grid must be at least 2x2"); return UDET_ERR_SHAPE; }
  const long total = (long)N * H * W * (ld / 4);
  hipLaunchKernelGGL(upb_ring_fold_kernel, dim3(grid_for(total, 8192)), dim3(256), 0, s, dxh, ld, N, H, W, dx, ld / 4);
  UDET_HIP(hipGetLastError());
  return UDET_OK;
}
__global__ __launch_bounds__(256) void axpy_kernel(const float* __restrict__ x, float* __restrict__ y, long n, float a,
                                                   int accumulate) {
  for (long i = (long)blockIdx.x * 256 + threadIdx.x; i < n; i += (long)gridDim.x * 256)
    y[i] = accumulate ? y[i] + a * x[i] : a * x[i];
}
int launch_axpy(const float* x, float* y, long n, float a, int accumulate, hipStream_t s) {
  hipLaunchKernelGGL(axpy_kernel, dim3(grid_for(n)), dim3(256), 0, s, x, y, n, a, accumulate);
  UDET_HIP(hipGetLastError());
  return UDET_OK;
}

}
```

unsupervised_detection_amd/csrc/plan.h:

```cpp
#pragma once
#include <map>
#include <string>
#include <vector>

#include "common.h"

namespace udet {

struct ParamDesc {
  std::string name;
  int rank;
  int shape[4];
  size_t offset, count;
};
struct NetParams {
  std::vector<ParamDesc> p;
  size_t total = 0;
  int add(const std::string& name, int a, int b = 0, int c = 0, int d = 0);
  int find(const std::string& name) const;
};
enum { NET_PWC = 0, NET_GEN = 1, NET_REC = 2 };
const NetParams& net_params(int net);

struct Buf {
  std::string name;
  size_t off;
  int n, h, w, ld;
  size_t floats() const { return (size_t)n * h * w * ld; }
};

struct Layer {
  std::string name;
  int net;
  int kh, kw, cin, cout, stride, dil;
  bool transposed = false;
  bool up = false;
  int act = ACT_NONE;
  float alpha = 0.f;
  int w_idx = -1, b_idx = -1, g_idx = -1, be_idx = -1;
  int Kc = 0, ldw = 0, k_split = 0, k_gap = 0;
  size_t wp_off = 0;
  int KcT = 0, ldwT = 0;
  size_t wpT_off = 0;
  size_t bias_f_off = 0, scale_off = 0;
  size_t wu_off = 0, wuT_off = 0;
  size_t wino_off = 0, winoT_off = 0;
  int wino_np = 0, winoT_np = 0;
  bool upb = false;
  bool upb_bwd = false;
  bool upb_split = false;
  int xhat = -1, src = -1;
  size_t wupb_off = 0, wupbT_off = 0;
  struct SegLaunch {
    int nseg = 0;
    ConvSeg seg[UDET_MAX_SEGS];
    int seg_tap[UDET_MAX_SEGS + 1];
    std::vector<ConvTap> taps;
    size_t tab_off = 0;
  } upb_f, upb_b;
  int x = -1, x_coff = 0, y = -1, y_coff = 0;
  int res = -1, res_coff = 0, y2 = -1;
  int H = 0, W = 0;
  bool col2im = false;
  int ldz = 0, zbuf = -1;
  size_t wz_off = 0;
  bool x_in_slab = false, y_fanned_out = false;
  std::string pair_name;
};

struct Resolved {
  struct {
    int pyr[7][3];
    int est[7][5], flow[7], ctx[7][7];
    int up_feat[7], up_flow[7];
  } pwc;
  struct {
    int enc[2][9];
    int deconv[6], flow[6], upflow[6];
  } rec;
  int image, flow, mask, pred, image_next, flow_next, d_mask, flow_full;
  int pwc_x8, pwc_rflow2, pwc_c[7], pwc_slab[7];
  int gen_in, gen_a17, gen_d[18], gen_u[18];
  int rec_imgin, rec_fin, rec_conv6, rec_concat[6], rec_r[7], rec_rf[6], rec_flow[6];
  struct Grad {
    int pred, fin, conv6, u_conv6;
    int flow[6], concat[6], u_concat[6], r[7], rf[6];
    int p[6];
    int enc_du[2][9];
    int enc_dx[2][9], enc_ux[2][9];
  } grad[2];
};

struct Config {
  int batch, in_h, in_w, img_h, img_w;
  float flow_normalizer, cbn, epsilon;
  float lr, beta1, beta2, adam_eps, clip;
  unsigned long long noise_seed;
  int conv_fp16 = 0;
};

struct Plan {
  Config cfg;
  std::vector<Buf> bufs;
  std::map<std::string, int> buf_by_name;
  std::vector<Layer> pwc, gen, rec;
  size_t packed_floats = 0;
  size_t arena_floats = 0;
  enum { NLANE = 6, NCAND = 8, MAXCAND = 32 };
  std::vector<hipStream_t> cand;
  struct Placement {
    hipStream_t main = nullptr;
    hipStream_t lane[NLANE] = {};
    int queue[NLANE] = {};
    int nqueues = 1;
  };
  std::vector<Placement> placements;
  int placed = -1;
  hipEvent_t prefetch_ev = nullptr;
  hipEvent_t grad_ev[3] = {nullptr, nullptr, nullptr};
  bool prefetch_pending = false;
  std::vector<hipEvent_t> ev_pool, ev_pool_prefetch;
  size_t ev_next = 0, ev_next_prefetch = 0;
  bool in_prefetch = false;
  bool concurrent = true;
  bool enc_a_shared = false;
  size_t scratch_off[NLANE] = {}, scratch_floats = 0;
  size_t wgrad_off[NLANE] = {}, wgrad_floats = 0;
  ~Plan();
  size_t small_off = 0;
  size_t ticket_off = 0;
  size_t seg_off[3] = {0, 0, 0};
  size_t jobs_off[3] = {0, 0, 0};
  int njobs[3] = {0, 0, 0};
  struct ProfRec {
    int cat; double flops, bytes; hipEvent_t a, b; std::string name;
    double mfma_scale = 1.0;
    enum { MAXK = 16 };
    hipEvent_t kev[2 * MAXK];
    LaunchSink sink;
  };
  bool profiling = false;
  std::vector<ProfRec*> prof;
  long adam_t = 0;
  int* ovf_host = nullptr;
  hipEvent_t ovf_ev[3] = {nullptr, nullptr, nullptr};
  bool ovf_pending[3] = {false, false, false};
  long ovf_skipped = 0;
  int ovf_report_values = 0, ovf_report_nets = 0;
  bool pwc_packed = false;
  Resolved R;
  int add_buf(const std::string& name, int n, int h, int w, int ld);
  const Buf& buf(int id) const { return bufs[id]; }
  int bid(const std::string& name) const;
};

#define UDET_PACKJOB_CAP(layers) (8 * (layers) + 32)
#define UDET_SMALL_NOISE 256
#define UDET_SMALL_OVF 300
#define UDET_SMALL_SUMS 1024
Plan* plan_build(const Config& cfg);
void plan_debug_upb_min_pixels(long v);
void build_upb_launches(Layer& L, int h, int w);
void upb_pack_jobs(const Layer& L, const PackJob& base, std::vector<PackJob>& jobs);
enum { UDET_KNOB_ENC_A_LANE = 0, UDET_KNOB_REC_DEC_WGRAD_LANE = 1, UDET_KNOB_REC_ENC_WGRAD_LANE = 2, UDET_KNOB_GEN_WGRAD_LATE = 3, UDET_KNOB_NO_WGRAD_WINO = 6, UDET_KNOB_SKIP = 7, UDET_KNOB_NO_PAIRS = 8, UDET_KNOB_COUNT = 12 };
#ifdef UDET_EXPERIMENT
void plan_debug_knob(int id, long v);
long plan_knob(int id);
#else
constexpr long plan_knob(int) { return 0; }
#endif

int plan_init_workspace(Plan* P, float* ws, hipStream_t s);
int plan_pack_pwc(Plan* P, const float* w_pwc, float* ws, hipStream_t s);
int plan_pack_trainable(Plan* P, const float* w_gen, const float* w_rec, float* ws, hipStream_t s);
int plan_pwc_forward(Plan* P, const float* img1, const float* img2, float* ws, hipStream_t s);
int plan_forward(Plan* P, const float* img1, const float* img2, int ncalls, float* ws, hipStream_t s, bool prefetched = false);
int plan_prefetch(Plan* P, const float* img1, const float* img2, float* ws, hipStream_t s);
int plan_prefetch_consume(Plan* P, float* ws, hipStream_t s);
int plan_generator_forward(Plan* P, float* ws, hipStream_t s);
int plan_generator_layers(Plan* P, float* ws, hipStream_t s);
int plan_recover_forward(Plan* P, int ncalls, float* ws, hipStream_t s, bool inputs_prepacked = false, bool skip_enc_a = false, bool enc_a_input_packed = false);
int plan_losses(Plan* P, float* ws, hipStream_t s);
int plan_backward(Plan* P, int which, const float* w_gen, const float* w_rec, float* g_gen, float* g_rec, float* ws, hipStream_t s);
int plan_apply(Plan* P, int net, float* w, float* g, float* m, float* v, float* ws, hipStream_t s);
int plan_check_overflow(Plan* P, bool wait);
void plan_settle_adam_step(Plan* P);
int plan_lane_queues(Plan* P, hipStream_t s, int* queue);
int plan_pin_lanes(Plan* P, hipStream_t main, hipStream_t const* streams, int n);
enum { PROF_CONV_FWD = 0, PROF_CONV_DGRAD = 1, PROF_CONV_WGRAD = 2, PROF_WARP = 3, PROF_CORR = 4, PROF_NCAT = 5 };
void prof_begin(Plan* P, int cat, double flops, double bytes, hipStream_t s, const char* name = "");
void prof_end(Plan* P, hipStream_t s);

}
```

unsupervised_detection_amd/csrc/plan_exec.hip:

```cpp
#include <string.h>

#include "conv_select.h"
#include "elementwise.h"
#include "plan_run.h"

namespace udet {

static double layer_flops(const Layer& L, int N) {
  const int up = L.up ? 1 : 0;
  double oh, ow;
  if (L.transposed) { oh = 2.0 * L.H; ow = 2.0 * L.W; }
  else { oh = (double)(((L.H << up) + L.stride - 1) / L.stride); ow = (double)(((L.W << up) + L.stride - 1) / L.stride); }
  double taps = (double)L.kh * L.kw;
  if (L.transposed) taps /= 4.0;
  return 2.0 * N * oh * ow * L.cout * L.cin * taps;
}
static double layer_bytes(const Layer& L, int N) {
  const int up = L.up ? 1 : 0;
  const double ih = (double)(L.H << up), iw = (double)(L.W << up);
  double oh, ow;
  if (L.transposed) { oh = 2.0 * L.H; ow = 2.0 * L.W; }
  else { oh = (double)(((L.H << up) + L.stride - 1) / L.stride); ow = (double)(((L.W << up) + L.stride - 1) / L.stride); }
  return 4.0 * (N * ih * iw * L.cin + N * oh * ow * L.cout + (double)L.kh * L.kw * L.cin * L.cout + L.cout);
}

static inline bool skip_launch(int kind, int net) {
  const long k = plan_knob(UDET_KNOB_SKIP);
  if (!k) return false;
  const int bit = kind == 2 ? (net == NET_GEN ? 0 : 1) : (kind == 1 ? (net == NET_GEN ? 2 : 3) : (net == NET_PWC ? 4 : (net == NET_GEN ? 5 : 6)));
  return (k >> bit) & 1;
}

static inline int up_off(int parity, int t) { return parity == 0 ? (t == 0 ? -1 : 0) : (t == 0 ? 0 : 1); }
void setup_up_fwd(ConvParams& p, int N, int H, int W) {
  p.N = N; p.H = H; p.W = W;
  p.OH = 2 * H; p.OW = 2 * W; p.OHq = H; p.OWq = W;
  p.osy = p.osx = 2; p.ooy = p.oox = 0; p.isy = p.isx = 1;
  p.ncls = 4; p.ntaps = 16;
  for (int c = 0; c < 4; ++c) {
    p.cls_tap[c] = 4 * c;
    for (int t = 0; t < 4; ++t) {
      ConvTap& tp = p.taps[4 * c + t];
      tp.dy = up_off(c >> 1, t >> 1); tp.dx = up_off(c & 1, t & 1); tp.widx = 4 * c + t;
    }
  }
  p.cls_tap[4] = 16;
}
static void setup_up_dgrad(ConvParams& p, int N, int H, int W) {
  p.N = N; p.H = 2 * H; p.W = 2 * W;
  p.OH = H; p.OW = W; p.OHq = H; p.OWq = W;
  p.osy = p.osx = 1; p.ooy = p.oox = 0; p.isy = p.isx = 2;
  p.ncls = 1; p.ntaps = 16;
  for (int c = 0; c < 4; ++c)
    for (int t = 0; t < 4; ++t) {
      ConvTap& tp = p.taps[4 * c + t];
      tp.dy = (c >> 1) - 2 * up_off(c >> 1, t >> 1); tp.dx = (c & 1) - 2 * up_off(c & 1, t & 1); tp.widx = 4 * c + t;
    }
}

static void fill_segments(ConvParams& p, const Layer::SegLaunch& g, const ConvTap* tab_dev, int first = 0) {
  p.nseg = g.nseg - first;
  memcpy(p.seg, g.seg + first, sizeof(ConvSeg) * p.nseg);
  memcpy(p.seg_tap, g.seg_tap + first, sizeof(int) * (p.nseg + 1));
  p.tap_tab = tab_dev;
}
static void fill_lane(ConvParams& p, const UpbLane& ln, float f16_xscale) {
  p.partial = ln.partial; p.partial_cap = ln.partial_cap;
  p.zero16 = ln.zero16; p.tickets = ln.tickets;
  p.f16 = ln.f16; p.f16_xscale = f16_xscale;
}
int upb_forward(const UpbFwd& a, hipStream_t s) {
  const int h = a.h, w = a.w;
  UDET_TRY(launch_upb_ring(a.src, a.ld, a.N, h, w, a.xhat, s));
  ConvParams p;
  memset(&p, 0, sizeof(p));
  p.N = a.N; p.H = h + 2; p.W = w + 2;
  p.OH = 2 * h; p.OW = 2 * w;
  p.osy = p.osx = 2; p.isy = p.isx = 1;
  p.x = a.xhat; p.ldx = a.ld; p.x_coff = 0;
  p.wp = a.wsets; p.Kc = a.Kc; p.ldw = a.ldw; p.bias = a.bias;
  p.y = a.y; p.ldy = a.ldy; p.y_coff = a.y_coff; p.Cout = a.cout;
  p.act = a.act; p.alpha = a.alpha;
  fill_lane(p, a.lane, 1.f);
  const Layer::SegLaunch& F = *a.tab;
  if (a.split) {
    ConvParams q = p;
    q.OHq = h - 1; q.OWq = w - 1;
    q.ncls = 4;
    for (int c = 0; c < 4; ++c) {
      q.cls_tap[c] = q.ntaps;
      for (int t = F.seg_tap[c]; t < F.seg_tap[c + 1]; ++t) q.taps[q.ntaps++] = F.taps[t];
    }
    q.cls_tap[4] = q.ntaps;
    UDET_TRY(launch_conv(q, s));
    fill_segments(p, F, a.tab_dev, 4);
  } else {
    fill_segments(p, F, a.tab_dev);
  }
  return launch_conv(p, s);
}
int upb_dgrad(const UpbBwd& a, hipStream_t s) {
  const int h = a.h, w = a.w;
  ConvParams p;
  memset(&p, 0, sizeof(p));
  p.N = a.N; p.H = 2 * h; p.W = 2 * w;
  p.OH = h + 2; p.OW = w + 2;
  p.osy = p.osx = 1; p.isy = p.isx = 2;
  fill_segments(p, *a.tab, a.tab_dev);
  p.x = a.du; p.ldx = a.lddu; p.x_coff = a.du_coff;
  p.wp = a.wsetsT; p.Kc = a.KcT; p.ldw = a.ldwT; p.kreal = a.cout;
  p.y = a.dxhat; p.ldy = a.ld; p.y_coff = 0; p.Cout = a.cin;
  fill_lane(p, a.lane, a.f16_xscale);
  UDET_TRY(launch_conv(p, s));
  return launch_upb_ring_fold(a.dxhat, a.ld, a.N, h, w, a.dsrc, s);
}

#define UDET_F16_GRAD_SCALE 4096.f
static void fill_common(Plan* P, ConvParams& p, float* ws, int slot) {
  p.partial = ws + P->scratch_off[slot];
  p.partial_cap = P->scratch_floats;
  p.zero16 = ws + P->small_off + 60000;
  p.tickets = reinterpret_cast<int*>(ws + P->ticket_off) + (size_t)slot * UDET_MAX_TICKETS;
  p.f16 = P->cfg.conv_fp16;
  p.f16_xscale = 1.f;
}

static void bind_x(ConvParams& p, const Buf& b, int coff, float* ws) { p.x = ws + b.off; p.ldx = b.ld; p.x_coff = coff; }
static void bind_y(ConvParams& p, const Buf& b, int coff, int cout, float* ws) { p.y = ws + b.off; p.ldy = b.ld; p.y_coff = coff; p.Cout = cout; }
static void bind_w(ConvParams& p, size_t off, int Kc, int ldw, float* ws) { p.wp = ws + off; p.Kc = Kc; p.ldw = ldw; }
static void bind_res(ConvParams& p, const Buf& b, int coff, float* ws) { p.res = ws + b.off; p.ldres = b.ld; p.res_coff = coff; }
static void bind_y2(ConvParams& p, const Buf& b, float* ws) { p.y2 = ws + b.off; p.ldy2 = b.ld; p.y2_coff = 0; }
static void bind_wino(ConvParams& p, size_t off, int np, float* ws) { p.wino_u = ws + off; p.wino_np = np; }
static void bind_emit(Plan* P, ConvParams& p, const Emit& em, int coff, float* ws) {
  const Buf &bu = P->buf(em.ubuf), &bua = P->buf(em.abuf);
  p.uo = ws + bu.off; p.ldu = bu.ld; p.u_coff = coff;
  p.ua = ws + bua.off; p.ldua = bua.ld; p.ua_coff = coff;
  p.uact = em.act; p.ualpha = em.alpha; p.u_c0 = em.c0; p.u_c1 = em.c1;
}

static UpbLane upb_lane(Plan* P, float* ws, int slot) {
  ConvParams c;
  fill_common(P, c, ws, slot);
  return UpbLane{c.partial, c.partial_cap, c.zero16, c.tickets, c.f16};
}

static int run_fwd_upb(Plan* P, const Layer& L, int N, float* ws, const Lane& ln) {
  hipStream_t s = ln.s;
  const Buf &bs = P->buf(L.src), &bp = P->buf(L.xhat), &by = P->buf(L.y);
  prof_begin(P, PROF_CONV_FWD, layer_flops(L, N) * 9.0 / 16.0, layer_bytes(L, N), s, L.name.c_str());
  UpbFwd a;
  a.N = N; a.h = bs.h; a.w = bs.w;
  a.src = ws + bs.off; a.xhat = ws + bp.off; a.ld = bp.ld;
  a.wsets = ws + L.wupb_off; a.Kc = L.Kc; a.ldw = L.ldw; a.bias = ws + L.bias_f_off;
  a.y = ws + by.off; a.ldy = by.ld; a.y_coff = L.y_coff; a.cout = L.cout;
  a.act = L.act; a.alpha = L.alpha;
  a.tab = &L.upb_f; a.tab_dev = reinterpret_cast<const ConvTap*>(ws + L.upb_f.tab_off); a.split = L.upb_split;
  a.lane = upb_lane(P, ws, ln.slot);
  UDET_TRY(upb_forward(a, s));
  prof_end(P, s);
  return UDET_OK;
}

int run_dgrad_upb(Plan* P, const Layer& L, int N, int du, int dxhat, int dsrc, float* ws, const Lane& ln) {
  hipStream_t s = ln.s;
  if (skip_launch(1, L.net)) return UDET_OK;
  const Buf &bu = P->buf(du), &bp = P->buf(dxhat), &bd = P->buf(dsrc);
  prof_begin(P, PROF_CONV_DGRAD, layer_flops(L, N) * 9.0 / 16.0, layer_bytes(L, N), s, L.name.c_str());
  UpbBwd a;
  a.N = N; a.h = bd.h; a.w = bd.w;
  a.du = ws + bu.off; a.lddu = bu.ld; a.du_coff = L.y_coff;
  a.wsetsT = ws + L.wupbT_off; a.KcT = L.KcT; a.ldwT = L.ldwT; a.cout = L.cout;
  a.dxhat = ws + bp.off; a.dsrc = ws + bd.off; a.ld = bp.ld; a.cin = L.cin;
  a.tab = &L.upb_b; a.tab_dev = reinterpret_cast<const ConvTap*>(ws + L.upb_b.tab_off);
  a.lane = upb_lane(P, ws, ln.slot);
  a.f16_xscale = UDET_F16_GRAD_SCALE;
  UDET_TRY(upb_dgrad(a, s));
  prof_end(P, s);
  return UDET_OK;
}

static bool up_form(const Layer& L) { return L.up && L.wu_off; }
static int fwd_launches(const Layer& L) { return L.transposed ? conv_dgrad_classes(2, 2 * L.H, 2 * L.W) : 1; }
static bool fwd_is_plain(const Layer& L) { return !L.transposed && !L.up && !L.upb && !L.col2im; }
static bool fwd_params(Plan* P, const Layer& L, int N, int cls, float* ws, int slot, ConvParams& p) {
  memset(&p, 0, sizeof(p));
  if (L.transposed) {
    if (!conv_setup_dgrad(p, cls, N, 2 * L.H, 2 * L.W, L.kh, L.kw, 2, 1)) return false;
  } else if (up_form(L)) {
    setup_up_fwd(p, N, L.H, L.W);
  } else {
    conv_setup_fwd(p, N, L.H << (L.up ? 1 : 0), L.W << (L.up ? 1 : 0), L.kh, L.kw, L.stride, L.dil);
    p.up_shift = L.up ? 1 : 0;
  }
  bind_x(p, P->buf(L.x), L.x_coff, ws);
  bind_w(p, up_form(L) ? L.wu_off : L.wp_off, L.Kc, L.ldw, ws); p.bias = ws + L.bias_f_off;
  bind_y(p, P->buf(L.y), L.y_coff, L.cout, ws);
  p.act = L.act; p.alpha = L.alpha;
  if (L.res >= 0) bind_res(p, P->buf(L.res), L.res_coff, ws);
  if (L.y2 >= 0) bind_y2(p, P->buf(L.y2), ws);
  if (L.wino_off) bind_wino(p, L.wino_off, L.wino_np, ws);
  fill_common(P, p, ws, slot);
  return true;
}

int run_fwd(Plan* P, const Layer& L, int N, float* ws, const Lane& ln) {
  hipStream_t s = ln.s;
  if (skip_launch(0, L.net)) return UDET_OK;
  if (L.upb) return run_fwd_upb(P, L, N, ws, ln);
  const Buf &bx = P->buf(L.x), &by = P->buf(L.y);
  prof_begin(P, PROF_CONV_FWD, layer_flops(L, N) * (up_form(L) ? 4.0 / 9.0 : 1.0), layer_bytes(L, N), s, L.name.c_str());
  bool direct_head = false;
  if (L.col2im && !P->cfg.conv_fp16 && L.Kc <= 64) {
    ConvParams q;
    memset(&q, 0, sizeof(q));
    if (L.transposed) (void)conv_setup_dgrad(q, 0, N, 2 * L.H, 2 * L.W, L.kh, L.kw, 2, 1);
    else conv_setup_fwd(q, N, L.H, L.W, L.kh, L.kw, L.stride, L.dil);
    q.Kc = L.Kc; q.ldw = L.ldw; q.Cout = L.cout;
    if (q.ncls != 4) { q.ncls = 1; q.cls_tap[0] = 0; q.cls_tap[1] = q.ntaps; }
    direct_head = conv_thin_n_ok(q);
  }
  if (L.col2im && !direct_head && fwd_launches(L) == 1) {
    const Buf& bz = P->buf(L.zbuf);
    ConvParams p;
    memset(&p, 0, sizeof(p));
    conv_setup_fwd(p, N, L.H, L.W, 1, 1, 1, 1);
    bind_x(p, bx, L.x_coff, ws);
    bind_w(p, L.wz_off, L.Kc, L.ldz, ws);
    bind_y(p, bz, 0, L.kh * L.kw * L.cout, ws);
    fill_common(P, p, ws, ln.slot);
    UDET_TRY(launch_conv(p, s));
    ConvParams g;
    memset(&g, 0, sizeof(g));
    if (L.transposed) conv_setup_dgrad(g, 0, N, 2 * L.H, 2 * L.W, L.kh, L.kw, 2, 1);
    else conv_setup_fwd(g, N, L.H, L.W, L.kh, L.kw, 1, 1);
    g.H = L.H; g.W = L.W;
    g.bias = ws + L.bias_f_off;
    bind_y(g, by, L.y_coff, L.cout, ws);
    UDET_TRY(launch_tap_gather(g, ws + bz.off, bz.ld, s));
    prof_end(P, s);
    return UDET_OK;
  }
  for (int cls = 0; cls < fwd_launches(L); ++cls) {
    ConvParams p;
    if (!fwd_params(P, L, N, cls, ws, ln.slot, p)) continue;
    UDET_TRY(launch_conv(p, s));
    if (P->profiling && (conv_last_config() & 0xff) == FAM_WINO) P->prof.back()->mfma_scale = 4.0 / 9.0;
  }
  prof_end(P, s);
  return UDET_OK;
}

static bool up_form_T(const Layer& L) { return L.up && L.wuT_off; }
static int dgrad_launches(const Layer& L) { return up_form_T(L) ? 1 : conv_dgrad_classes(L.stride, L.H << (L.up ? 1 : 0), L.W << (L.up ? 1 : 0)); }
static bool dgrad_is_plain(const Layer& L) { return !L.up && !L.upb && !L.transposed && dgrad_launches(L) == 1; }
static bool dgrad_params(Plan* P, const Layer& L, int N, int cls, int dy, bool dy_is_du, int dx, int dx_coff, int accumulate, int res,
                         const Emit& em, float* ws, int slot, ConvParams& p) {
  const int up = L.up ? 1 : 0;
  memset(&p, 0, sizeof(p));
  if (up_form_T(L)) setup_up_dgrad(p, N, L.H, L.W);
  else if (!conv_setup_dgrad(p, cls, N, L.H << up, L.W << up, L.kh, L.kw, L.stride, L.dil)) return false;
  bind_x(p, P->buf(dy), L.y_coff, ws);
  if (L.act != ACT_NONE && !dy_is_du) { p.xa = ws + P->buf(L.y2 >= 0 ? L.y2 : L.y).off; p.xact = L.act; p.xalpha = L.alpha; }
  bind_w(p, up_form_T(L) ? L.wuT_off : L.wpT_off, L.KcT, L.ldwT, ws); p.kreal = L.cout;
  bind_y(p, P->buf(dx), dx_coff, L.cin, ws);
  p.accumulate = accumulate;
  if (res >= 0) bind_res(p, P->buf(res), 0, ws);
  if (em.ubuf >= 0) bind_emit(P, p, em, dx_coff, ws);
  if (L.winoT_off && !up_form_T(L)) bind_wino(p, L.winoT_off, L.winoT_np, ws);
  fill_common(P, p, ws, slot);
  p.f16_xscale = UDET_F16_GRAD_SCALE;
  return true;
}

int run_dgrad(Plan* P, const Layer& L, int N, int dy, bool dy_is_du, int dx, int dx_coff, int accumulate, int res, const Emit& em, float* ws,
              const Lane& ln) {
  hipStream_t s = ln.s;
  if (skip_launch(1, L.net)) return UDET_OK;
  const Buf &bdy = P->buf(dy), &ba = P->buf(L.y2 >= 0 ? L.y2 : L.y);
  if (ba.ld != bdy.ld) {
    set_error("dgrad(%s): gradient/activation layout mismatch (%d vs %d)", L.name.c_str(), bdy.ld, ba.ld);
    return UDET_ERR_SHAPE;
  }
  prof_begin(P, PROF_CONV_DGRAD, layer_flops(L, N) * (up_form_T(L) ? 4.0 / 9.0 : 1.0), layer_bytes(L, N), s, L.name.c_str());
  for (int cls = 0; cls < dgrad_launches(L); ++cls) {
    ConvParams p;
    if (!dgrad_params(P, L, N, cls, dy, dy_is_du, dx, dx_coff, accumulate, res, em, ws, ln.slot, p)) continue;
    UDET_TRY(launch_conv(p, s));
    if (P->profiling && (conv_last_config() & 0xff) == FAM_WINO) P->prof.back()->mfma_scale = 4.0 / 9.0;
  }
  prof_end(P, s);
  return UDET_OK;
}

int run_wgrad(Plan* P, const Layer& L, int N, int dy, bool dy_is_du, const float* w_flat, float* g_flat, float* ws, const Lane& ln) {
  hipStream_t s = ln.s;
  if (skip_launch(2, L.net)) return UDET_OK;
  const NetParams& np = net_params(L.net);
  const int act_buf = L.y2 >= 0 ? L.y2 : L.y;
  const Buf &bx = P->buf(L.x), &bdy = P->buf(dy), &ba = P->buf(act_buf);
  const int up = L.up ? 1 : 0;
  ConvParams g;
  memset(&g, 0, sizeof(g));
  conv_setup_fwd(g, N, L.H << up, L.W << up, L.kh, L.kw, L.stride, L.dil);
  WgradParams q;
  memset(&q, 0, sizeof(q));
  q.x = ws + bx.off; q.ldx = bx.ld; q.x_coff = L.x_coff;
  q.N = N; q.H = L.H << up; q.W = L.W << up; q.up_shift = up; q.Cin = L.cin;
  q.dy = ws + bdy.off; q.ldy = bdy.ld; q.y_coff = L.y_coff; q.Cout = L.cout;
  if (L.act != ACT_NONE && !dy_is_du) { q.ya = ws + ba.off; q.yact = L.act; q.yalpha = L.alpha; }
  q.OH = g.OH; q.OW = g.OW; q.isy = q.isx = L.stride;
  q.ntaps = g.ntaps;
  memcpy(q.taps, g.taps, sizeof(g.taps));
  q.dw = g_flat + np.p[L.w_idx].offset;
  q.db = g_flat + np.p[L.b_idx].offset;
  q.partial = ws + P->wgrad_off[ln.slot];
  q.zero16 = ws + P->small_off + 60000;
  q.partial_floats = P->wgrad_floats;
  q.f16 = P->cfg.conv_fp16;
  q.f16_yscale = UDET_F16_GRAD_SCALE;
  if (L.g_idx >= 0) {
    q.w = w_flat + np.p[L.w_idx].offset;
    q.b = w_flat + np.p[L.b_idx].offset;
    q.gamma = w_flat + np.p[L.g_idx].offset;
    q.dgamma = g_flat + np.p[L.g_idx].offset;
    q.dbeta = g_flat + np.p[L.be_idx].offset;
    q.bn_c = BN_C;
  }
  if (L.up && L.wu_off && L.g_idx >= 0 && dy_is_du) {
    prof_begin(P, PROF_CONV_WGRAD, layer_flops(L, N) * 4.0 / 9.0, layer_bytes(L, N), s, L.name.c_str());
    const int rc = launch_wgrad_up_T(q, L.H, L.W, s);
    prof_end(P, s);
    return rc;
  }
  prof_begin(P, PROF_CONV_WGRAD, layer_flops(L, N), layer_bytes(L, N), s, L.name.c_str());
  const int rc = launch_wgrad_T(q, L.kh * L.kw, s);
  if (P->profiling && (wgrad_last_config() >> 20) == 3) P->prof.back()->mfma_scale = 4.0 / 9.0;
  prof_end(P, s);
  return rc;
}

int run_fwd_pair(Plan* P, const Layer& La, int Na, const Layer& Lb, int Nb, float* ws, const Lane& ln) {
  if (!pairs_on(P) || !fwd_is_plain(La) || !fwd_is_plain(Lb)) {
    UDET_TRY(run_fwd(P, La, Na, ws, ln));
    return run_fwd(P, Lb, Nb, ws, ln);
  }
  if (skip_launch(0, La.net)) return UDET_OK;
  ConvParams a, b;
  fwd_params(P, La, Na, 0, ws, ln.slot, a);
  fwd_params(P, Lb, Nb, 0, ws, ln.slot, b);
  a.wino_u = b.wino_u = nullptr; a.wino_np = b.wino_np = 0;
  prof_begin(P, PROF_CONV_FWD, layer_flops(La, Na) + layer_flops(Lb, Nb), layer_bytes(La, Na) + layer_bytes(Lb, Nb), ln.s, La.pair_name.c_str());
  const int rc = launch_conv_pair(a, b, ln.s);
  prof_end(P, ln.s);
  return rc;
}
int run_dgrad_pair(Plan* P, const DgradJob& ja, const DgradJob& jb, float* ws, const Lane& ln) {
  ConvParams a, b;
  auto one_launch = [&](const DgradJob& j, ConvParams& p) {
    return dgrad_is_plain(*j.L) && dgrad_params(P, *j.L, j.N, 0, j.dy, true, j.dx, j.dx_coff, j.accumulate, -1, j.em, ws, ln.slot, p);
  };
  if (!pairs_on(P, 1) || !one_launch(ja, a) || !one_launch(jb, b)) {
    UDET_TRY(run_dgrad(P, *ja.L, ja.N, ja.dy, true, ja.dx, ja.dx_coff, ja.accumulate, -1, ja.em, ws, ln));
    return run_dgrad(P, *jb.L, jb.N, jb.dy, true, jb.dx, jb.dx_coff, jb.accumulate, -1, jb.em, ws, ln);
  }
  if (skip_launch(1, ja.L->net)) return UDET_OK;
  a.wino_u = b.wino_u = nullptr;
  prof_begin(P, PROF_CONV_DGRAD, layer_flops(*ja.L, ja.N) + layer_flops(*jb.L, jb.N), layer_bytes(*ja.L, ja.N) + layer_bytes(*jb.L, jb.N), ln.s,
             ja.L->pair_name.c_str());
  const int rc = launch_conv_pair(a, b, ln.s);
  prof_end(P, ln.s);
  return rc;
}

}
```

unsupervised_detection_amd/csrc/plan_pack.hip:

```cpp
#include <string.h>

#include "conv_host.h"
#include "plan_run.h"

namespace udet {

void upb_pack_jobs(const Layer& L, const PackJob& base, std::vector<PackJob>& jobs) {
  PackJob j = base;
  for (int r = 0; r < 4; ++r) {
    j.T = 36; j.gamma_off = -1;
    j.dst_off = (long)(L.wupb_off + (size_t)r * 36 * L.Kc * L.ldw); j.R = L.cin; j.C = L.cout; j.Kc = L.Kc; j.ldw = L.ldw; j.k_split = L.k_split; j.k_gap = L.k_gap;
    j.mode = 9; j.beta_off = (long)((r & 1) * 3 + (r >> 1)); j.total = (long)L.Kc * L.ldw;
    jobs.push_back(j);
    if (L.upb_bwd) {
      j.dst_off = (long)(L.wupbT_off + (size_t)r * 36 * L.KcT * L.ldwT); j.Kc = L.KcT; j.ldw = L.ldwT; j.k_split = L.KcT; j.k_gap = 0;
      j.mode = 10; j.total = (long)L.KcT * L.ldwT;
      jobs.push_back(j);
    }
  }
}

int plan_init_workspace(Plan* P, float* ws, hipStream_t s) {
  UDET_HIP(hipMemsetAsync(ws, 0, P->arena_floats * sizeof(float), s));
  for (int net = 1; net <= 2; ++net) {
    const NetParams& np = net_params(net);
    std::vector<long> tab(2 * np.p.size());
    for (size_t i = 0; i < np.p.size(); ++i) {
      tab[i] = (long)np.p[i].offset;
      tab[np.p.size() + i] = (long)np.p[i].count;
    }
    UDET_HIP(hipMemcpyAsync(ws + P->seg_off[net], tab.data(), tab.size() * sizeof(long), hipMemcpyHostToDevice, s));
    UDET_HIP(hipStreamSynchronize(s));
  }
  for (int net = 1; net <= 2; ++net) {
    const NetParams& np = net_params(net);
    const std::vector<Layer>& layers = net == NET_GEN ? P->gen : P->rec;
    std::vector<PackJob> jobs;
    for (const auto& L : layers) {
      const int T = L.kh * L.kw;
      const long goff = L.g_idx >= 0 ? (long)np.p[L.g_idx].offset : -1, beoff = L.be_idx >= 0 ? (long)np.p[L.be_idx].offset : -1;
      PackJob j;
      memset(&j, 0, sizeof(j));
      j.src_off = (long)np.p[L.w_idx].offset; j.gamma_off = goff; j.beta_off = beoff;
      j.T = T;
      j.dst_off = (long)L.wp_off; j.R = L.cin; j.C = L.cout; j.Kc = L.Kc; j.ldw = L.ldw; j.k_split = L.k_split; j.k_gap = L.k_gap;
      j.mode = 0; j.total = (long)T * L.Kc * L.ldw;
      jobs.push_back(j);
      j.dst_off = (long)L.wpT_off; j.Kc = L.KcT; j.ldw = L.ldwT; j.k_split = L.KcT; j.k_gap = 0;
      j.mode = 1; j.total = (long)T * L.KcT * L.ldwT;
      jobs.push_back(j);
      if (L.col2im) {
        j.dst_off = (long)L.wz_off; j.R = L.cin; j.C = L.cout; j.Kc = L.Kc; j.ldw = L.ldz; j.k_split = L.k_split; j.k_gap = L.k_gap;
        j.mode = 3; j.total = (long)L.Kc * L.ldz;
        jobs.push_back(j);
      }
      if (L.up) {
        j.T = 16;
        j.dst_off = (long)L.wu_off; j.R = L.cin; j.C = L.cout; j.Kc = L.Kc; j.ldw = L.ldw; j.k_split = L.Kc; j.k_gap = 0;
        j.mode = 5; j.total = (long)16 * L.Kc * L.ldw;
        jobs.push_back(j);
        j.dst_off = (long)L.wuT_off; j.Kc = L.KcT; j.ldw = L.ldwT; j.k_split = L.KcT; j.k_gap = 0;
        j.mode = 6; j.total = (long)16 * L.KcT * L.ldwT;
        jobs.push_back(j);
        j.T = T;
      }
      if (L.upb) upb_pack_jobs(L, j, jobs);
      if (L.wino_off) {
        j.dst_off = (long)L.wino_off; j.R = L.cin; j.C = L.cout; j.Kc = L.Kc; j.ldw = L.wino_np; j.k_split = L.k_split; j.k_gap = L.k_gap;
        j.mode = 7; j.total = (long)(L.Kc / 8) * 2 * L.wino_np;
        jobs.push_back(j);
      }
      if (L.winoT_off) {
        j.dst_off = (long)L.winoT_off; j.R = L.cin; j.C = L.cout; j.Kc = L.KcT; j.ldw = L.winoT_np; j.k_split = L.KcT; j.k_gap = 0;
        j.mode = 8; j.total = (long)(L.KcT / 8) * 2 * L.winoT_np;
        jobs.push_back(j);
      }
      j.src_off = (long)np.p[L.b_idx].offset; j.dst_off = (long)L.bias_f_off; j.mode = 2; j.total = L.cout;
      jobs.push_back(j);
    }
    if (jobs.size() > UDET_PACKJOB_CAP(layers.size())) {
      set_error("plan_init: %zu weight re-layout jobs for %zu layers exceed the table's %zu entries", jobs.size(), layers.size(),
                (size_t)UDET_PACKJOB_CAP(layers.size()));
      return UDET_ERR_ARG;
    }
    P->njobs[net] = (int)jobs.size();
    UDET_HIP(hipMemcpyAsync(ws + P->jobs_off[net], jobs.data(), jobs.size() * sizeof(PackJob), hipMemcpyHostToDevice, s));
    UDET_HIP(hipStreamSynchronize(s));
  }
  for (const auto& L : P->rec)
    if (L.upb)
      for (const Layer::SegLaunch* g : {&L.upb_f, &L.upb_b})
        if (g == &L.upb_f || L.upb_bwd)
          UDET_HIP(hipMemcpyAsync(ws + g->tab_off, g->taps.data(), g->taps.size() * sizeof(ConvTap), hipMemcpyHostToDevice, s));
  UDET_HIP(hipStreamSynchronize(s));
  P->pwc_packed = false;
  return UDET_OK;
}

static int pack_layer(const Layer& L, const float* w_flat, float* ws, const float* scale, bool trainable, hipStream_t s) {
  const NetParams& np = net_params(L.net);
  const float* w = w_flat + np.p[L.w_idx].offset;
  const int T = L.kh * L.kw;
  if (L.transposed)
    UDET_TRY(launch_pack_weights(w, ws + L.wp_off, T, L.cout, L.cin, L.Kc, L.ldw, L.k_split, L.k_gap, 1, nullptr, s));
  else
    UDET_TRY(launch_pack_weights(w, ws + L.wp_off, T, L.cin, L.cout, L.Kc, L.ldw, L.k_split, L.k_gap, 0, scale, s));
  if (trainable)
    UDET_TRY(launch_pack_weights(w, ws + L.wpT_off, T, L.cin, L.cout, L.KcT, L.ldwT, L.KcT, 0, 1, scale, s));
  if (L.col2im)
    UDET_TRY(launch_pack_taps_into_n(w, ws + L.wz_off, T, L.cin, L.cout, L.Kc, L.ldz, L.k_split, L.k_gap, L.transposed ? 1 : 0, s));
  if (L.wino_off && !trainable)
    UDET_TRY(launch_wino_pack(w, ws + L.wino_off, L.cin, L.cout, L.Kc, L.wino_np, L.k_split, L.k_gap, 0, s));
  return UDET_OK;
}

int plan_pack_pwc(Plan* P, const float* w, float* ws, hipStream_t s) {
  const NetParams& np = net_params(NET_PWC);
  for (const auto& L : P->pwc) {
    UDET_TRY(pack_layer(L, w, ws, nullptr, false, s));
    UDET_TRY(launch_copy_channels(w + np.p[L.b_idx].offset, L.cout, 0, ws + L.bias_f_off, L.cout, 0, 1, L.cout, 1.f, 0.f, s));
  }
  P->pwc_packed = true;
  return UDET_OK;
}

int plan_pack_trainable(Plan* P, const float* w_gen, const float* w_rec, float* ws, hipStream_t s) {
  if (w_gen)
    UDET_TRY(launch_pack_jobs(reinterpret_cast<const PackJob*>(ws + P->jobs_off[NET_GEN]), P->njobs[NET_GEN], w_gen, ws, BN_C, s));
  if (w_rec)
    UDET_TRY(launch_pack_jobs(reinterpret_cast<const PackJob*>(ws + P->jobs_off[NET_REC]), P->njobs[NET_REC], w_rec, ws, BN_C, s));
  return UDET_OK;
}

}
```

unsupervised_detection_amd/csrc/plan_run.h:

```cpp
#pragma once
#include "plan.h"

namespace udet {

static const float BN_C = 0.99950037468777316f;

struct Lane {
  hipStream_t s;
  int slot;
};
Lane lane_of(Plan* P, hipStream_t main, int i);
hipEvent_t next_event(Plan* P);
void order_after(Plan* P, const Lane& from, const Lane& to);

struct Emit {
  int ubuf = -1, abuf = -1, c0 = 0, c1 = 0, act = ACT_NONE;
  float alpha = 0.f;
};
struct DgradJob {
  const Layer* L;
  int N, dy, dx, dx_coff, accumulate;
  Emit em;
};
inline bool pairs_on(const Plan* P, int dir = 0) { return !P->cfg.conv_fp16 && !((plan_knob(UDET_KNOB_NO_PAIRS) >> dir) & 1); }
int run_fwd(Plan* P, const Layer& L, int N, float* ws, const Lane& ln);
int run_fwd_pair(Plan* P, const Layer& La, int Na, const Layer& Lb, int Nb, float* ws, const Lane& ln);
int run_dgrad(Plan* P, const Layer& L, int N, int dy, bool dy_is_du, int dx, int dx_coff, int accumulate, int res, const Emit& em, float* ws,
              const Lane& ln);
int run_dgrad_pair(Plan* P, const DgradJob& ja, const DgradJob& jb, float* ws, const Lane& ln);
int run_dgrad_upb(Plan* P, const Layer& L, int N, int du, int dxhat, int dsrc, float* ws, const Lane& ln);
int run_wgrad(Plan* P, const Layer& L, int N, int dy, bool dy_is_du, const float* w_flat, float* g_flat, float* ws, const Lane& ln);
struct UpbLane {
  float* partial;
  size_t partial_cap;
  const float* zero16;
  int* tickets;
  int f16;
};
struct UpbFwd {
  int N, h, w;
  const float* src;
  float* xhat;
  int ld;
  const float* wsets;
  int Kc, ldw;
  const float* bias;
  float* y;
  int ldy, y_coff, cout, act;
  float alpha;
  const Layer::SegLaunch* tab;
  const ConvTap* tab_dev;
  bool split;
  UpbLane lane;
};
struct UpbBwd {
  int N, h, w;
  const float* du;
  int lddu, du_coff;
  const float* wsetsT;
  int KcT, ldwT, cout;
  float* dxhat;
  float* dsrc;
  int ld, cin;
  const Layer::SegLaunch* tab;
  const ConvTap* tab_dev;
  float f16_xscale;
  UpbLane lane;
};
int upb_forward(const UpbFwd& a, hipStream_t s);
int upb_dgrad(const UpbBwd& a, hipStream_t s);

}
```

unsupervised_detection_amd/csrc/plan_step.hip:

```cpp
#include "conv_host.h"
#include "elementwise.h"
#include "plan_run.h"

namespace udet {

static const int PWC_CH[7] = {0, 16, 32, 64, 96, 128, 196};
static const char* const WARP_NAME[7] = {"", "", "warp_costvol2", "warp_costvol3", "warp_costvol4", "warp_costvol5", "warp_costvol6"};

static int pwc_forward_on(Plan* P, const float* img1, const float* img2, float* ws, const Lane& L0, const Lane& LH) {
  if (!P->pwc_packed) {
    set_error("pwc_forward: call udet_pack_pwc first");
    return UDET_ERR_ARG;
  }
  const Config& c = P->cfg;
  const Resolved& R = P->R;
  const int B = c.batch;
  hipStream_t s = L0.s;
  auto fwd = [&](int layer, int N, const Lane& ln) { return run_fwd(P, P->pwc[layer], N, ws, ln); };
  UDET_TRY(launch_pack_pwc_input(img1, img2, ws + P->buf(R.pwc_x8).off, (long)B * c.in_h * c.in_w, s));
  for (int l = 1; l <= 6; ++l)
    for (int j = 0; j < 3; ++j) UDET_TRY(fwd(R.pwc.pyr[l][j], 2 * B, L0));
  for (int l = 6; l >= 2; --l) {
    const int h = c.in_h >> l, w = c.in_w >> l, C = PWC_CH[l];
    const Buf& cb = P->buf(R.pwc_c[l]);
    const Buf& slab = P->buf(R.pwc_slab[l]);
    const float* c1 = ws + cb.off;
    const float* c2 = ws + cb.off + (size_t)B * h * w * C;
    const bool warped = l != 6;
    const double px = (double)B * h * w;
    prof_begin(P, PROF_CORR, 2.0 * px * 81.0 * C, px * ((warped ? 3.0 * C + 2.0 : 2.0 * C) + 81.0) * 4.0, s, WARP_NAME[l]);
    UDET_TRY(launch_warp_cost_volume(c1, c2, warped ? ws + slab.off : nullptr, slab.ld, 532 + C, 20.0f / (float)(1 << l), ws + slab.off,
                                     slab.ld, 448, warped ? 532 : -1, nullptr, B, h, w, C, s));
    prof_end(P, s);
    for (int i = 0; i < 5; ++i) UDET_TRY(fwd(R.pwc.est[l][i], B, L0));
    order_after(P, L0, LH);
    UDET_TRY(fwd(R.pwc.flow[l], B, LH));
    if (l != 2) UDET_TRY(fwd(R.pwc.up_feat[l], B, LH));
    for (int i = 0; i < 6; ++i) UDET_TRY(fwd(R.pwc.ctx[l][i], B, L0));
    order_after(P, LH, L0);
    UDET_TRY(fwd(R.pwc.ctx[l][6], B, L0));
    if (l != 2) UDET_TRY(fwd(R.pwc.up_flow[l], B, L0));
  }
  const Buf& fr = P->buf(R.pwc_rflow2);
  const Buf& ff = P->buf(R.flow_full);
  return launch_resize_bilinear_fwd(ws + fr.off, fr.ld, 0, B, fr.h, fr.w, ws + ff.off, 2, 0, c.in_h, c.in_w, 2, 4.0f, 1.f, s);
}

int plan_pwc_forward(Plan* P, const float* img1, const float* img2, float* ws, hipStream_t s) {
  P->ev_next = 0;
  if (P->prefetch_pending) (void)hipStreamWaitEvent(s, P->prefetch_ev, 0);
  return pwc_forward_on(P, img1, img2, ws, lane_of(P, s, 0), lane_of(P, s, 2));
}

static int plan_prepare_image(Plan* P, const float* img1, int dst, float* ws, hipStream_t s) {
  const Config& c = P->cfg;
  return launch_resize_bilinear_fwd(img1, 3, 0, c.batch, c.in_h, c.in_w, ws + P->buf(dst).off, 3, 0, c.img_h, c.img_w,
                                    3, 1.f, 1.f, s);
}
static int plan_prepare_flow(Plan* P, int dst, float* ws, hipStream_t s) {
  const Config& c = P->cfg;
  const Buf& ff = P->buf(P->R.flow_full);
  return launch_resize_bilinear_fwd(ws + ff.off, 2, 0, c.batch, c.in_h, c.in_w, ws + P->buf(dst).off, 2, 0, c.img_h,
                                    c.img_w, 2, 1.f, c.flow_normalizer, s);
}

int plan_prefetch(Plan* P, const float* img1, const float* img2, float* ws, hipStream_t s) {
  const Lane L0 = lane_of(P, s, 0), LC = lane_of(P, s, 4), LH = lane_of(P, s, 5);
  P->in_prefetch = true;
  P->ev_next_prefetch = 0;
  order_after(P, L0, LC);
  int rc = pwc_forward_on(P, img1, img2, ws, LC, LH);
  P->in_prefetch = false;
  UDET_TRY(rc);
  UDET_TRY(plan_prepare_flow(P, P->R.flow_next, ws, LC.s));
  UDET_TRY(plan_prepare_image(P, img1, P->R.image_next, ws, LC.s));
  if (!P->prefetch_ev) (void)hipEventCreateWithFlags(&P->prefetch_ev, hipEventDisableTiming);
  (void)hipEventRecord(P->prefetch_ev, LC.s);
  P->prefetch_pending = true;
  return UDET_OK;
}

int plan_generator_forward(Plan* P, float* ws, hipStream_t s) {
  const Config& c = P->cfg;
  const long HW = (long)c.img_h * c.img_w;
  const Lane L0 = lane_of(P, s, 0);
  double* part = reinterpret_cast<double*>(ws + P->small_off + 4096);
  UDET_TRY(launch_gen_input(ws + P->buf(P->R.image).off, ws + P->buf(P->R.flow).off, part, ws + P->buf(P->R.gen_in).off, c.batch, HW, s));
  for (const auto& L : P->gen) UDET_TRY(run_fwd(P, L, c.batch, ws, L0));
  return UDET_OK;
}
int plan_generator_layers(Plan* P, float* ws, hipStream_t s) {
  const Lane L0 = lane_of(P, s, 0);
  for (const auto& L : P->gen) UDET_TRY(run_fwd(P, L, P->cfg.batch, ws, L0));
  return UDET_OK;
}

static int rec_resize(Plan* P, int src, int dst, int N, float* ws, hipStream_t s) {
  const Buf &a = P->buf(src), &b = P->buf(dst);
  return launch_resize_bilinear_fwd(ws + a.off, a.ld, 0, N, a.h, a.w, ws + b.off, b.ld, 0, b.h, b.w, a.ld, 1.f, 1.f, s);
}
static int dec_src(const Resolved& R, int k) { return k == 5 ? R.rec_conv6 : R.rec_concat[k + 1]; }

static int share_enc_a_output(Plan* P, const Layer& L, int ncalls, float* ws, hipStream_t s) {
  const Buf& y = P->buf(L.y);
  if (ncalls > 1 && L.y_fanned_out) return launch_share_samples(ws + y.off, (long)P->cfg.batch * y.h * y.w, y.ld, L.y_coff, L.cout, ncalls, s);
  return UDET_OK;
}
static int plan_rec_image_branch(Plan* P, int ncalls, float* ws, const Lane& ln, bool with_layers = true) {
  const Config& c = P->cfg;
  if (ncalls < 1) return UDET_OK;
  const long Ppix = (long)c.batch * c.img_h * c.img_w;
  UDET_TRY(launch_pack_imgin(ws + P->buf(P->R.image).off, ws + P->buf(P->R.rec_imgin).off, Ppix, 1, ln.s));
  if (!with_layers) return UDET_OK;
  for (int i = 0; i < 9; ++i) {
    const Layer& L = P->rec[P->R.rec.enc[0][i]];
    UDET_TRY(run_fwd(P, L, c.batch, ws, ln));
    UDET_TRY(share_enc_a_output(P, L, ncalls, ws, ln.s));
  }
  P->enc_a_shared = true;
  return UDET_OK;
}

int plan_recover_forward(Plan* P, int ncalls, float* ws, hipStream_t s, bool inputs_prepacked, bool skip_enc_a, bool enc_a_input_packed) {
  const Config& c = P->cfg;
  const Resolved& R = P->R;
  const int B = c.batch, N = ncalls * B;
  const long Ppix = (long)B * c.img_h * c.img_w;
  const Lane L0 = lane_of(P, s, 0);
  if (!inputs_prepacked)
    UDET_TRY(launch_mask_rec_inputs(ws + P->buf(R.gen_a17).off, ws + P->buf(R.flow).off, ws + P->buf(R.mask).off, ws + P->buf(R.rec_fin).off,
                                    Ppix, ncalls, s));
  if (ncalls < 1) return UDET_OK;
  auto enc = [&](int e, int i) -> const Layer& { return P->rec[R.rec.enc[e][i]]; };
  if (!skip_enc_a && pairs_on(P)) {
    if (!inputs_prepacked && !enc_a_input_packed) UDET_TRY(plan_rec_image_branch(P, ncalls, ws, L0, false));
    for (int i = 0; i < 9; ++i) {
      const Layer& La = enc(0, i);
      UDET_TRY(run_fwd_pair(P, La, inputs_prepacked ? N : B, enc(1, i), N, ws, L0));
      if (!inputs_prepacked) UDET_TRY(share_enc_a_output(P, La, ncalls, ws, s));
    }
    P->enc_a_shared = !inputs_prepacked;
  } else {
    if (!skip_enc_a) {
      if (inputs_prepacked) {
        for (int i = 0; i < 9; ++i) UDET_TRY(run_fwd(P, enc(0, i), N, ws, L0));
        P->enc_a_shared = false;
      } else {
        UDET_TRY(plan_rec_image_branch(P, ncalls, ws, L0));
      }
    }
    for (int i = 0; i < 9; ++i) UDET_TRY(run_fwd(P, enc(1, i), N, ws, L0));
  }
  for (int k = 5; k >= 1; --k) {
    const Layer& dcl = P->rec[R.rec.deconv[k]];
    if (!dcl.upb) UDET_TRY(rec_resize(P, dec_src(R, k), R.rec_r[k + 1], N, ws, s));
    UDET_TRY(run_fwd(P, dcl, N, ws, L0));
    if (k < 5) {
      UDET_TRY(rec_resize(P, R.rec_flow[k + 1], R.rec_rf[k + 1], N, ws, s));
      UDET_TRY(run_fwd(P, P->rec[R.rec.upflow[k]], N, ws, L0));
    }
    UDET_TRY(run_fwd(P, P->rec[R.rec.flow[k]], N, ws, L0));
  }
  const Buf& f1 = P->buf(R.rec_flow[1]);
  return launch_resize_bilinear_fwd(ws + f1.off, f1.ld, 0, N, f1.h, f1.w, ws + P->buf(R.pred).off, 2, 0, c.img_h, c.img_w, 2, 1.f, 1.f, s);
}

int plan_losses(Plan* P, float* ws, hipStream_t s) {
  const Config& c = P->cfg;
  float* sm = ws + P->small_off;
  const long HW = (long)c.img_h * c.img_w;
  return launch_losses(ws + P->buf(P->R.flow).off, ws + P->buf(P->R.mask).off, ws + P->buf(P->R.pred).off, HW,
                       c.batch, c.cbn, c.epsilon, (float)(c.img_w * c.img_h * c.batch), sm + 8192, sm, sm + 16, sm + UDET_SMALL_SUMS, s);
}

int plan_prefetch_consume(Plan* P, float* ws, hipStream_t s) {
  if (!P->prefetch_pending) {
    set_error("forward_prefetched: no udet_prefetch_flow is pending");
    return UDET_ERR_ARG;
  }
  (void)hipStreamWaitEvent(s, P->prefetch_ev, 0);
  P->prefetch_pending = false;
  const Buf &fn = P->buf(P->R.flow_next), &in = P->buf(P->R.image_next);
  UDET_HIP(hipMemcpyAsync(ws + P->buf(P->R.flow).off, ws + fn.off, fn.floats() * sizeof(float), hipMemcpyDeviceToDevice, s));
  UDET_HIP(hipMemcpyAsync(ws + P->buf(P->R.image).off, ws + in.off, in.floats() * sizeof(float), hipMemcpyDeviceToDevice, s));
  return UDET_OK;
}

int plan_forward(Plan* P, const float* img1, const float* img2, int ncalls, float* ws, hipStream_t s, bool prefetched) {
  P->ev_next = 0;
  const Lane L0 = lane_of(P, s, 0), LI = lane_of(P, s, 1);
  if (prefetched) {
    UDET_TRY(plan_prefetch_consume(P, ws, s));
    img1 = img2 = nullptr;
  } else if (img1 && P->prefetch_pending) {
    (void)hipStreamWaitEvent(s, P->prefetch_ev, 0);
  }
  order_after(P, L0, LI);
  if (img1) UDET_TRY(plan_prepare_image(P, img1, P->R.image, ws, LI.s));
  hipEvent_t e_img = nullptr;
  if (LI.s != L0.s) {
    e_img = next_event(P);
    (void)hipEventRecord(e_img, LI.s);
  }
  const bool paired = pairs_on(P);
  UDET_TRY(plan_rec_image_branch(P, ncalls, ws, LI, !paired));
  if (img1) {
    UDET_TRY(pwc_forward_on(P, img1, img2, ws, L0, lane_of(P, s, 2)));
    UDET_TRY(plan_prepare_flow(P, P->R.flow, ws, s));
  }
  if (e_img) (void)hipStreamWaitEvent(s, e_img, 0);
  UDET_TRY(plan_generator_forward(P, ws, s));
  order_after(P, LI, L0);
  UDET_TRY(plan_recover_forward(P, ncalls, ws, s, false, !paired, paired));
  if (ncalls == 3) UDET_TRY(plan_losses(P, ws, s));
  return UDET_OK;
}

static int rec_backward(Plan* P, int N, const Resolved::Grad& G, bool with_wgrad, bool need_dfin, const float* w_rec, float* g_rec, float* ws,
                        const Lane& LD, const Lane& LW, const Lane* LAp = nullptr, const Lane* LWdecp = nullptr) {
  const Config& c = P->cfg;
  const Resolved& R = P->R;
  hipStream_t s = LD.s;
  const Lane LWdec = LWdecp ? *LWdecp : LW;
  auto wgrad_on = [&](const Lane& lw, const Layer& L, int dy, bool is_du, int n) -> int {
    order_after(P, LD, lw);
    return run_wgrad(P, L, n < 0 ? N : n, dy, is_du, w_rec, g_rec, ws, lw);
  };
  auto wgrad = [&](const Layer& L, int dy, bool is_du, int n = -1) -> int { return wgrad_on(LW, L, dy, is_du, n); };
  auto wgrad_dec = [&](const Layer& L, int dy, bool is_du) -> int { return wgrad_on(LWdec, L, dy, is_du, -1); };
  const Lane LA = LAp ? *LAp : LD;
  const bool a_own_lane = LA.s != LD.s;
  const int ncopies = N / c.batch;
  const bool a_shared = P->enc_a_shared && ncopies > 1;
  const Emit none;
  const float LEAK = 0.2f;
  {
    const Buf& df1 = P->buf(G.flow[1]);
    UDET_TRY(launch_resize_bilinear_bwd(ws + P->buf(G.pred).off, 2, 0, N, c.img_h, c.img_w, ws + df1.off, df1.ld, 0, df1.h, df1.w, 2, 0, s));
  }
  for (int k = 1; k <= 5; ++k) {
    const int dconcat = G.concat[k], uconcat = G.u_concat[k];
    const Layer* fl = &P->rec[R.rec.flow[k]];
    const Layer* dc = &P->rec[R.rec.deconv[k]];
    Emit em;
    em.ubuf = uconcat; em.abuf = fl->x; em.c0 = 0; em.c1 = dc->cout; em.act = ACT_LEAKY; em.alpha = LEAK;
    UDET_TRY(run_dgrad(P, *fl, N, G.flow[k], false, dconcat, 0, k == 1 ? 0 : 1, -1, em, ws, LD));
    if (with_wgrad) UDET_TRY(wgrad_dec(*fl, G.flow[k], false));
    if (k < 5) {
      const Layer* uf = &P->rec[R.rec.upflow[k]];
      if (with_wgrad) UDET_TRY(wgrad_dec(*uf, dconcat, false));
      UDET_TRY(run_dgrad(P, *uf, N, dconcat, false, G.rf[k + 1], 0, 0, -1, none, ws, LD));
      const Buf &drf = P->buf(G.rf[k + 1]), &dfn = P->buf(G.flow[k + 1]);
      UDET_TRY(launch_resize_bilinear_bwd(ws + drf.off, drf.ld, 0, N, drf.h, drf.w, ws + dfn.off, dfn.ld, 0, dfn.h, dfn.w, drf.ld, 0, s));
    }
    if (with_wgrad) {
      if (dc->upb) {
        order_after(P, LD, LWdec);
        UDET_TRY(rec_resize(P, dec_src(R, k), R.rec_r[k + 1], N, ws, LWdec.s));
      }
      UDET_TRY(wgrad_dec(*dc, uconcat, true));
    }
    if (dc->upb_bwd) {
      UDET_TRY(run_dgrad_upb(P, *dc, N, uconcat, G.p[k + 1], G.concat[k + 1], ws, LD));
      continue;
    }
    const int dr = G.r[k + 1];
    UDET_TRY(run_dgrad(P, *dc, N, uconcat, true, dr, 0, 0, -1, none, ws, LD));
    const Buf& bdr = P->buf(dr);
    const Buf& dsrc = P->buf(k == 5 ? G.conv6 : G.concat[k + 1]);
    UDET_TRY(launch_resize_bilinear_bwd(ws + bdr.off, bdr.ld, 0, N, bdr.h, bdr.w, ws + dsrc.off, dsrc.ld, 0, dsrc.h, dsrc.w,
                                        bdr.ld, 0, s));
  }
  {
    const Buf &d6 = P->buf(G.conv6), &a6 = P->buf(R.rec_conv6), &u6 = P->buf(G.u_conv6);
    UDET_TRY(launch_emit_du(ws + d6.off, ws + a6.off, ws + u6.off, (long)N * d6.h * d6.w, d6.ld, 0, d6.ld, ACT_LEAKY, LEAK, s));
  }
  if (a_own_lane) order_after(P, LD, LA);
  const bool pair_enc = pairs_on(P, 1) && with_wgrad && !a_own_lane;
  for (int i = 8; i >= 0; --i) {
    DgradJob job[2];
    int njob = 0;
    for (int e = 0; e < 2; ++e) {
      if (e == 0 && !with_wgrad) continue;
      const Layer* L = &P->rec[R.rec.enc[e][i]];
      const int du = G.enc_du[e][i];
      const bool shared = e == 0 && a_shared;
      const int Ne = shared ? c.batch : N;
      const bool own = e == 0 && a_own_lane;
      const Lane& LE = own ? LA : LD;
      hipStream_t se = LE.s;
      if (shared && i == 8) {
        const Buf& u = P->buf(du);
        UDET_TRY(launch_fold_samples(ws + u.off, (long)c.batch * u.h * u.w, u.ld, L->y_coff, L->cout, ncopies, se));
      }
      if (with_wgrad) {
        if (own) UDET_TRY(run_wgrad(P, *L, Ne, du, true, w_rec, g_rec, ws, LA));
        else UDET_TRY(wgrad(*L, du, true, Ne));
      }
      if (i == 0) {
        if (e == 1 && need_dfin) UDET_TRY(run_dgrad(P, *L, N, du, true, G.fin, 0, 0, -1, none, ws, LD));
        continue;
      }
      const int dx = G.enc_dx[e][i];
      const bool slab_in = L->x_in_slab;
      Emit em;
      em.ubuf = G.enc_ux[e][i]; em.abuf = L->x; em.c0 = 0; em.c1 = L->cin; em.act = ACT_LEAKY; em.alpha = LEAK;
      if (shared && slab_in) {
        const Buf& d = P->buf(dx);
        UDET_TRY(launch_fold_samples(ws + d.off, (long)c.batch * d.h * d.w, d.ld, L->x_coff, L->cin, ncopies, se));
      }
      if (pair_enc) {
        job[njob].L = L; job[njob].N = Ne; job[njob].dy = du; job[njob].dx = dx; job[njob].dx_coff = L->x_coff;
        job[njob].accumulate = slab_in ? 1 : 0; job[njob].em = em;
        ++njob;
        continue;
      }
      UDET_TRY(run_dgrad(P, *L, Ne, du, true, dx, L->x_coff, slab_in ? 1 : 0, -1, em, ws, LE));
    }
    if (njob == 2) UDET_TRY(run_dgrad_pair(P, job[0], job[1], ws, LD));
    else if (njob == 1) UDET_TRY(run_dgrad(P, *job[0].L, job[0].N, job[0].dy, true, job[0].dx, job[0].dx_coff, job[0].accumulate, -1, job[0].em, ws, LD));
  }
  if (a_own_lane) order_after(P, LA, LD);
  if (with_wgrad && LWdec.s != LW.s) order_after(P, LWdec, LD);
  return UDET_OK;
}

static int backward_recover(Plan* P, const float* w_rec, float* g_rec, float* ws, const Lane& LD, const Lane& LW, const Lane* LA = nullptr,
                            const Lane* LWdec = nullptr) {
  const Config& c = P->cfg;
  const Resolved& R = P->R;
  const long BHW = (long)c.batch * c.img_h * c.img_w;
  UDET_TRY(launch_rec_loss_bwd(ws + P->buf(R.flow).off, ws + P->buf(R.mask).off, ws + P->buf(R.pred).off, ws + P->buf(R.grad[0].pred).off, BHW,
                               c.cbn, 1.0f / (float)(c.img_w * c.img_h * c.batch), LD.s));
  return rec_backward(P, 3 * c.batch, R.grad[0], true, false, w_rec, g_rec, ws, LD, LW, LA, LWdec);
}

static int backward_generator(Plan* P, const float* w_gen, float* g_gen, float* ws, const Lane& LD, const Lane& LW, const Lane* LWlate = nullptr,
                              int nlate = 0) {
  const Config& c = P->cfg;
  const Resolved& R = P->R;
  const int B = c.batch;
  const long HW = (long)c.img_h * c.img_w;
  hipStream_t s = LD.s;
  float* sm = ws + P->small_off;
  UDET_TRY(launch_gen_loss_bwd(ws + P->buf(R.flow).off, ws + P->buf(R.mask).off, ws + P->buf(R.pred).off, sm + 16,
                               ws + P->buf(R.grad[1].pred).off, ws + P->buf(R.d_mask).off, HW, B, c.cbn, s));
  UDET_TRY(rec_backward(P, 2 * B, R.grad[1], false, true, nullptr, nullptr, ws, LD, LD));
  UDET_TRY(launch_mask_bwd(ws + P->buf(R.d_mask).off, ws + P->buf(R.grad[1].fin).off, ws + P->buf(R.flow).off, ws + P->buf(R.mask).off,
                           ws + P->buf(R.gen_d[17]).off, B * HW, s));
  for (int i = 16; i >= 0; --i) {
    const Layer& L = P->gen[i];
    const bool has_act = L.act != ACT_NONE;
    const int dy = has_act ? R.gen_u[i + 1] : R.gen_d[i + 1];
    const Lane& LWi = (LWlate && i < nlate) ? *LWlate : LW;
    order_after(P, LD, LWi);
    UDET_TRY(run_wgrad(P, L, B, dy, has_act, w_gen, g_gen, ws, LWi));
    if (i == 0) break;
    const int res = i == 6 ? R.gen_d[11] : (i == 3 ? R.gen_d[14] : (i == 1 ? R.gen_d[15] : -1));
    const int dx = R.gen_d[i];
    const Layer& Lp = P->gen[i - 1];
    const int ap = Lp.y2 >= 0 ? Lp.y2 : Lp.y;
    {
      Emit em;
      if (Lp.act != ACT_NONE) { em.ubuf = R.gen_u[i]; em.abuf = ap; em.c0 = 0; em.c1 = L.cin; em.act = Lp.act; em.alpha = Lp.alpha; }
      UDET_TRY(run_dgrad(P, L, B, dy, has_act, dx, 0, 0, res, em, ws, LD));
    }
  }
  return UDET_OK;
}

int plan_backward(Plan* P, int which, const float* w_gen, const float* w_rec, float* g_gen, float* g_rec, float* ws, hipStream_t s) {
  P->ev_next = 0;
  const Lane L0 = lane_of(P, s, 0), L1 = lane_of(P, s, 1), L2 = lane_of(P, s, 2), L3 = lane_of(P, s, 3);
  auto mark = [&](int net) {
    if (!P->grad_ev[net]) (void)hipEventCreateWithFlags(&P->grad_ev[net], hipEventDisableTiming);
    (void)hipEventRecord(P->grad_ev[net], s);
  };
  if (which == 3) {
    order_after(P, L0, L1);
    const int la = (int)plan_knob(UDET_KNOB_ENC_A_LANE);
    const Lane LA = lane_of(P, s, la > 0 && la < Plan::NLANE ? la : 0);
    const int lw = (int)plan_knob(UDET_KNOB_REC_DEC_WGRAD_LANE), le = (int)plan_knob(UDET_KNOB_REC_ENC_WGRAD_LANE);
    const Lane LWD = lane_of(P, s, lw > 0 && lw < Plan::NLANE ? lw : 3);
    const Lane LWE = lane_of(P, s, le > 0 && le < Plan::NLANE ? le : 2);
    UDET_TRY(backward_recover(P, w_rec, g_rec, ws, L0, LWE, la > 0 ? &LA : nullptr, &LWD));
    if (LWE.s != L2.s) order_after(P, LWE, L0);
    const long kl = plan_knob(UDET_KNOB_GEN_WGRAD_LATE);
    const int nlate = kl > 0 ? (int)kl : (kl < 0 ? 0 : 4);
    order_after(P, L2, L0);
    mark(NET_REC);
    UDET_TRY(backward_generator(P, w_gen, g_gen, ws, L1, L3, nlate > 0 ? &L2 : nullptr, nlate));
    order_after(P, L2, L0);
    order_after(P, L1, L0);
    order_after(P, L3, L0);
    mark(NET_GEN);
  } else if (which == 2) {
    UDET_TRY(backward_recover(P, w_rec, g_rec, ws, L0, L2, nullptr, &L3));
    order_after(P, L2, L0);
    mark(NET_REC);
  } else {
    UDET_TRY(backward_generator(P, w_gen, g_gen, ws, L0, L3));
    order_after(P, L3, L0);
    mark(NET_GEN);
  }
  return UDET_OK;
}

}
```

Before: 502.9.

## Run recover call 2 on image lane and cache constant recover input

Adds per-sample offsets to forward conv launches so the recover network's third call (constant-mask input) can run its full encoder and decoder on the image lane, overlapping the PWC and generator forward. The split path sits behind a debug toggle that is off by default. Separately, the constant fourth-channel input for call 2 is now written once and cached (invalidated after autotune and packing), so the per-step mask/input kernel only fills two calls. This saves a little per-step elementwise work but relies on nothing else overwriting that region of the workspace.

```diff
diff --git a/include/udet_debug.h b/include/udet_debug.h
--- a/include/udet_debug.h
+++ b/include/udet_debug.h
@@ -30,6 +30,9 @@
                                  int cin, int cout, void* workspace, size_t workspace_bytes, void* stream);
 int udet_debug_upconv_tables(int h, int w, int backward, int* nseg, int* seg, int* seg_tap, int* taps, int taps_cap, int* ntaps);
 int udet_debug_max_segs(void);
+void udet_debug_rec_call2_split(int on);
+struct udet_plan;
+int udet_debug_plan_run_fwd(struct udet_plan* plan, int net, const char* layer, int n0, int n, void* workspace, void* stream);
 int udet_debug_last_conv(void);
 #ifdef __cplusplus
 }
diff --git a/unsupervised_detection_amd/_devel.py b/unsupervised_detection_amd/_devel.py
--- a/unsupervised_detection_amd/_devel.py
+++ b/unsupervised_detection_amd/_devel.py
@@ -48,6 +48,10 @@
 dbg.udet_debug_upconv_tables.argtypes = [_i, _i, _i] + [_p] * 4 + [_i, _p]
 dbg.udet_debug_max_segs.restype = ctypes.c_int
 dbg.udet_debug_max_segs.argtypes = []
+dbg.udet_debug_rec_call2_split.restype = None
+dbg.udet_debug_rec_call2_split.argtypes = [_i]
+dbg.udet_debug_plan_run_fwd.restype = ctypes.c_int
+dbg.udet_debug_plan_run_fwd.argtypes = [_p, _i, ctypes.c_char_p, _i, _i, _p, _p]
 
 
 def upconv_tables(h: int, w: int, backward: bool):
diff --git a/unsupervised_detection_amd/csrc/api_plan.hip b/unsupervised_detection_amd/csrc/api_plan.hip
--- a/unsupervised_detection_amd/csrc/api_plan.hip
+++ b/unsupervised_detection_amd/csrc/api_plan.hip
@@ -6,10 +6,6 @@
 #include "plan.h"
 
 using namespace udet;
-
-struct udet_plan {
-  Plan* p;
-};
 
 extern "C" {
 
@@ -149,6 +145,7 @@
   if (!P->pwc_packed) { set_error("autotune: pack the PWC-Net and trainable weights first"); return UDET_ERR_ARG; }
   const size_t lo = P->packed_floats, hi = P->small_off;
   UDET_TRY(launch_fill_uniform(ws + lo, (long)(hi - lo), 0x5eedull, -0.5f, 0.5f, s));
+  P->rec_fin_const_valid = false;
   const size_t img_floats = (size_t)P->cfg.batch * P->cfg.in_h * P->cfg.in_w * 3;
   if (P->wgrad_floats < 2 * img_floats) { set_error("autotune: workspace too small for the probe images"); return UDET_ERR_ARG; }
   const float* img1 = ws + P->wgrad_off[0];
@@ -163,6 +160,8 @@
   wgrad_set_tuning(0);
   P->concurrent = was_concurrent;
   UDET_HIP(hipMemsetAsync(ws + lo, 0, (hi - lo) * sizeof(float), s));
+  P->rec_fin_const_valid = false;
+  if (rc == UDET_OK) rc = plan_rec_const_input(P, ws, s);
   UDET_HIP(hipStreamSynchronize(s));
   return rc;
 }
diff --git a/unsupervised_detection_amd/csrc/devel/api_debug.hip b/unsupervised_detection_amd/csrc/devel/api_debug.hip
--- a/unsupervised_detection_amd/csrc/devel/api_debug.hip
+++ b/unsupervised_detection_amd/csrc/devel/api_debug.hip
@@ -244,6 +244,12 @@
   return UDET_OK;
 }
 
+void udet_debug_rec_call2_split(int on) { plan_debug_rec_call2_split(on); }
+int udet_debug_plan_run_fwd(udet_plan* plan, int net, const char* layer, int n0, int n, void* ws, void* stream) {
+  if (!plan || !ws) { set_error("debug_plan_run_fwd: null argument"); return UDET_ERR_ARG; }
+  return plan_debug_run_fwd(plan->p, net, layer, n0, n, (float*)ws, (hipStream_t)stream);
+}
+
 void udet_debug_set_tuning(int on) {
   conv_set_tuning(on);
   wgrad_set_tuning(on);
diff --git a/unsupervised_detection_amd/csrc/elementwise.h b/unsupervised_detection_amd/csrc/elementwise.h
--- a/unsupervised_detection_amd/csrc/elementwise.h
+++ b/unsupervised_detection_amd/csrc/elementwise.h
@@ -15,6 +15,7 @@
 int launch_gen_input(const float* img, const float* f, double* part, float* gin, int B, long HW, hipStream_t s);
 size_t flow_stats_doubles(int B);
 int launch_mask_rec_inputs(const float* logits, const float* f, float* mask, float* fin, long P, int ncalls, hipStream_t s);
+int launch_rec_const_input(float* fin, long P, hipStream_t s);
 int launch_pack_imgin(const float* img, float* imgin, long P, int ncalls, hipStream_t s);
 int launch_losses(const float* f, const float* mask, const float* pred, long HW, int B, float cbn, float eps,
                   float num_pixels, float* part, float* losses, float* coef, float* sums, hipStream_t s);
diff --git a/unsupervised_detection_amd/csrc/elementwise.hip b/unsupervised_detection_amd/csrc/elementwise.hip
--- a/unsupervised_detection_amd/csrc/elementwise.hip
+++ b/unsupervised_detection_amd/csrc/elementwise.hip
@@ -495,6 +495,15 @@
   UDET_HIP(hipGetLastError());
   return UDET_OK;
 }
+__global__ __launch_bounds__(256) void rec_const_input_kernel(float* __restrict__ fin, long P) {
+  for (long q = (long)blockIdx.x * 256 + threadIdx.x; q < P; q += (long)gridDim.x * 256)
+    *reinterpret_cast<float4*>(fin + q * 4) = make_float4(0.f, 0.f, 1.f, 0.f);
+}
+int launch_rec_const_input(float* fin, long P, hipStream_t s) {
+  hipLaunchKernelGGL(rec_const_input_kernel, dim3(grid_for(P)), dim3(256), 0, s, fin, P);
+  UDET_HIP(hipGetLastError());
+  return UDET_OK;
+}
 __global__ __launch_bounds__(256) void pack_imgin_kernel(const float* __restrict__ img, float* __restrict__ imgin, long P,
                                                          int ncalls) {
   for (long q = (long)blockIdx.x * 256 + threadIdx.x; q < P; q += (long)gridDim.x * 256) {
diff --git a/unsupervised_detection_amd/csrc/plan.h b/unsupervised_detection_amd/csrc/plan.h
--- a/unsupervised_detection_amd/csrc/plan.h
+++ b/unsupervised_detection_amd/csrc/plan.h
@@ -124,6 +124,7 @@
   bool in_prefetch = false;
   bool concurrent = true;
   bool enc_a_shared = false;
+  bool rec_fin_const_valid = false;
   size_t scratch_off[NLANE] = {}, scratch_floats = 0;
   size_t wgrad_off[NLANE] = {}, wgrad_floats = 0;
   ~Plan();
@@ -160,6 +161,9 @@
 #define UDET_SMALL_SUMS 1024
 Plan* plan_build(const Config& cfg);
 void plan_debug_upb_min_pixels(long v);
+void plan_debug_rec_call2_split(int on);
+int plan_debug_run_fwd(Plan* P, int net, const char* layer, int n0, int n, float* ws, hipStream_t s);
+int plan_rec_const_input(Plan* P, float* ws, hipStream_t s);
 void build_upb_launches(Layer& L, int h, int w);
 void upb_pack_jobs(const Layer& L, const PackJob& base, std::vector<PackJob>& jobs);
 enum { UDET_KNOB_ENC_A_LANE = 0, UDET_KNOB_REC_DEC_WGRAD_LANE = 1, UDET_KNOB_REC_ENC_WGRAD_LANE = 2, UDET_KNOB_GEN_WGRAD_LATE = 3, UDET_KNOB_NO_WGRAD_WINO = 6, UDET_KNOB_SKIP = 7, UDET_KNOB_NO_PAIRS = 8, UDET_KNOB_COUNT = 12 };
@@ -192,3 +196,7 @@
 void prof_end(Plan* P, hipStream_t s);
 
 }
+
+struct udet_plan {
+  udet::Plan* p;
+};
diff --git a/unsupervised_detection_amd/csrc/plan_exec.hip b/unsupervised_detection_amd/csrc/plan_exec.hip
--- a/unsupervised_detection_amd/csrc/plan_exec.hip
+++ b/unsupervised_detection_amd/csrc/plan_exec.hip
@@ -125,11 +125,14 @@
   p.f16_xscale = 1.f;
 }
 
-static void bind_x(ConvParams& p, const Buf& b, int coff, float* ws) { p.x = ws + b.off; p.ldx = b.ld; p.x_coff = coff; }
-static void bind_y(ConvParams& p, const Buf& b, int coff, int cout, float* ws) { p.y = ws + b.off; p.ldy = b.ld; p.y_coff = coff; p.Cout = cout; }
+static size_t sample_off(const Buf& b, int n0) { return b.off + (size_t)n0 * b.h * b.w * b.ld; }
+static void bind_x(ConvParams& p, const Buf& b, int coff, float* ws, int n0 = 0) { p.x = ws + sample_off(b, n0); p.ldx = b.ld; p.x_coff = coff; }
+static void bind_y(ConvParams& p, const Buf& b, int coff, int cout, float* ws, int n0 = 0) {
+  p.y = ws + sample_off(b, n0); p.ldy = b.ld; p.y_coff = coff; p.Cout = cout;
+}
 static void bind_w(ConvParams& p, size_t off, int Kc, int ldw, float* ws) { p.wp = ws + off; p.Kc = Kc; p.ldw = ldw; }
-static void bind_res(ConvParams& p, const Buf& b, int coff, float* ws) { p.res = ws + b.off; p.ldres = b.ld; p.res_coff = coff; }
-static void bind_y2(ConvParams& p, const Buf& b, float* ws) { p.y2 = ws + b.off; p.ldy2 = b.ld; p.y2_coff = 0; }
+static void bind_res(ConvParams& p, const Buf& b, int coff, float* ws, int n0 = 0) { p.res = ws + sample_off(b, n0); p.ldres = b.ld; p.res_coff = coff; }
+static void bind_y2(ConvParams& p, const Buf& b, float* ws, int n0 = 0) { p.y2 = ws + sample_off(b, n0); p.ldy2 = b.ld; p.y2_coff = 0; }
 static void bind_wino(ConvParams& p, size_t off, int np, float* ws) { p.wino_u = ws + off; p.wino_np = np; }
 static void bind_emit(Plan* P, ConvParams& p, const Emit& em, int coff, float* ws) {
   const Buf &bu = P->buf(em.ubuf), &bua = P->buf(em.abuf);
@@ -144,15 +147,15 @@
   return UpbLane{c.partial, c.partial_cap, c.zero16, c.tickets, c.f16};
 }
 
-static int run_fwd_upb(Plan* P, const Layer& L, int N, float* ws, const Lane& ln) {
+static int run_fwd_upb(Plan* P, const Layer& L, int N, float* ws, const Lane& ln, int n0) {
   hipStream_t s = ln.s;
   const Buf &bs = P->buf(L.src), &bp = P->buf(L.xhat), &by = P->buf(L.y);
   prof_begin(P, PROF_CONV_FWD, layer_flops(L, N) * 9.0 / 16.0, layer_bytes(L, N), s, L.name.c_str());
   UpbFwd a;
   a.N = N; a.h = bs.h; a.w = bs.w;
-  a.src = ws + bs.off; a.xhat = ws + bp.off; a.ld = bp.ld;
+  a.src = ws + sample_off(bs, n0); a.xhat = ws + sample_off(bp, n0); a.ld = bp.ld;
   a.wsets = ws + L.wupb_off; a.Kc = L.Kc; a.ldw = L.ldw; a.bias = ws + L.bias_f_off;
-  a.y = ws + by.off; a.ldy = by.ld; a.y_coff = L.y_coff; a.cout = L.cout;
+  a.y = ws + sample_off(by, n0); a.ldy = by.ld; a.y_coff = L.y_coff; a.cout = L.cout;
   a.act = L.act; a.alpha = L.alpha;
   a.tab = &L.upb_f; a.tab_dev = reinterpret_cast<const ConvTap*>(ws + L.upb_f.tab_off); a.split = L.upb_split;
   a.lane = upb_lane(P, ws, ln.slot);
@@ -182,7 +185,7 @@
 static bool up_form(const Layer& L) { return L.up && L.wu_off; }
 static int fwd_launches(const Layer& L) { return L.transposed ? conv_dgrad_classes(2, 2 * L.H, 2 * L.W) : 1; }
 static bool fwd_is_plain(const Layer& L) { return !L.transposed && !L.up && !L.upb && !L.col2im; }
-static bool fwd_params(Plan* P, const Layer& L, int N, int cls, float* ws, int slot, ConvParams& p) {
+static bool fwd_params(Plan* P, const Layer& L, int N, int cls, float* ws, int slot, ConvParams& p, int n0 = 0) {
   memset(&p, 0, sizeof(p));
   if (L.transposed) {
     if (!conv_setup_dgrad(p, cls, N, 2 * L.H, 2 * L.W, L.kh, L.kw, 2, 1)) return false;
@@ -192,21 +195,25 @@
     conv_setup_fwd(p, N, L.H << (L.up ? 1 : 0), L.W << (L.up ? 1 : 0), L.kh, L.kw, L.stride, L.dil);
     p.up_shift = L.up ? 1 : 0;
   }
-  bind_x(p, P->buf(L.x), L.x_coff, ws);
+  bind_x(p, P->buf(L.x), L.x_coff, ws, n0);
   bind_w(p, up_form(L) ? L.wu_off : L.wp_off, L.Kc, L.ldw, ws); p.bias = ws + L.bias_f_off;
-  bind_y(p, P->buf(L.y), L.y_coff, L.cout, ws);
+  bind_y(p, P->buf(L.y), L.y_coff, L.cout, ws, n0);
   p.act = L.act; p.alpha = L.alpha;
-  if (L.res >= 0) bind_res(p, P->buf(L.res), L.res_coff, ws);
-  if (L.y2 >= 0) bind_y2(p, P->buf(L.y2), ws);
+  if (L.res >= 0) bind_res(p, P->buf(L.res), L.res_coff, ws, n0);
+  if (L.y2 >= 0) bind_y2(p, P->buf(L.y2), ws, n0);
   if (L.wino_off) bind_wino(p, L.wino_off, L.wino_np, ws);
   fill_common(P, p, ws, slot);
   return true;
 }
 
-int run_fwd(Plan* P, const Layer& L, int N, float* ws, const Lane& ln) {
+int run_fwd(Plan* P, const Layer& L, int N, float* ws, const Lane& ln, int n0) {
   hipStream_t s = ln.s;
   if (skip_launch(0, L.net)) return UDET_OK;
-  if (L.upb) return run_fwd_upb(P, L, N, ws, ln);
+  if (n0 < 0 || N < 1 || n0 + N > P->buf(L.y).n) {
+    set_error("run_fwd(%s): samples [%d, %d) outside the layer's %d", L.name.c_str(), n0, n0 + N, P->buf(L.y).n);
+    return UDET_ERR_ARG;
+  }
+  if (L.upb) return run_fwd_upb(P, L, N, ws, ln, n0);
   const Buf &bx = P->buf(L.x), &by = P->buf(L.y);
   prof_begin(P, PROF_CONV_FWD, layer_flops(L, N) * (up_form(L) ? 4.0 / 9.0 : 1.0), layer_bytes(L, N), s, L.name.c_str());
   bool direct_head = false;
@@ -224,9 +231,9 @@
     ConvParams p;
     memset(&p, 0, sizeof(p));
     conv_setup_fwd(p, N, L.H, L.W, 1, 1, 1, 1);
-    bind_x(p, bx, L.x_coff, ws);
+    bind_x(p, bx, L.x_coff, ws, n0);
     bind_w(p, L.wz_off, L.Kc, L.ldz, ws);
-    bind_y(p, bz, 0, L.kh * L.kw * L.cout, ws);
+    bind_y(p, bz, 0, L.kh * L.kw * L.cout, ws, n0);
     fill_common(P, p, ws, ln.slot);
     UDET_TRY(launch_conv(p, s));
     ConvParams g;
@@ -235,14 +242,14 @@
     else conv_setup_fwd(g, N, L.H, L.W, L.kh, L.kw, 1, 1);
     g.H = L.H; g.W = L.W;
     g.bias = ws + L.bias_f_off;
-    bind_y(g, by, L.y_coff, L.cout, ws);
-    UDET_TRY(launch_tap_gather(g, ws + bz.off, bz.ld, s));
+    bind_y(g, by, L.y_coff, L.cout, ws, n0);
+    UDET_TRY(launch_tap_gather(g, ws + sample_off(bz, n0), bz.ld, s));
     prof_end(P, s);
     return UDET_OK;
   }
   for (int cls = 0; cls < fwd_launches(L); ++cls) {
     ConvParams p;
-    if (!fwd_params(P, L, N, cls, ws, ln.slot, p)) continue;
+    if (!fwd_params(P, L, N, cls, ws, ln.slot, p, n0)) continue;
     UDET_TRY(launch_conv(p, s));
     if (P->profiling && (conv_last_config() & 0xff) == FAM_WINO) P->prof.back()->mfma_scale = 4.0 / 9.0;
   }
@@ -339,15 +346,19 @@
   return rc;
 }
 
-int run_fwd_pair(Plan* P, const Layer& La, int Na, const Layer& Lb, int Nb, float* ws, const Lane& ln) {
+int run_fwd_pair(Plan* P, const Layer& La, int Na, const Layer& Lb, int Nb, float* ws, const Lane& ln, int nb0) {
   if (!pairs_on(P) || !fwd_is_plain(La) || !fwd_is_plain(Lb)) {
     UDET_TRY(run_fwd(P, La, Na, ws, ln));
-    return run_fwd(P, Lb, Nb, ws, ln);
+    return run_fwd(P, Lb, Nb, ws, ln, nb0);
   }
   if (skip_launch(0, La.net)) return UDET_OK;
+  if (nb0 < 0 || Nb < 1 || nb0 + Nb > P->buf(Lb.y).n) {
+    set_error("run_fwd_pair(%s): samples [%d, %d) outside the layer's %d", Lb.name.c_str(), nb0, nb0 + Nb, P->buf(Lb.y).n);
+    return UDET_ERR_ARG;
+  }
   ConvParams a, b;
   fwd_params(P, La, Na, 0, ws, ln.slot, a);
-  fwd_params(P, Lb, Nb, 0, ws, ln.slot, b);
+  fwd_params(P, Lb, Nb, 0, ws, ln.slot, b, nb0);
   a.wino_u = b.wino_u = nullptr; a.wino_np = b.wino_np = 0;
   prof_begin(P, PROF_CONV_FWD, layer_flops(La, Na) + layer_flops(Lb, Nb), layer_bytes(La, Na) + layer_bytes(Lb, Nb), ln.s, La.pair_name.c_str());
   const int rc = launch_conv_pair(a, b, ln.s);
diff --git a/unsupervised_detection_amd/csrc/plan_pack.hip b/unsupervised_detection_amd/csrc/plan_pack.hip
--- a/unsupervised_detection_amd/csrc/plan_pack.hip
+++ b/unsupervised_detection_amd/csrc/plan_pack.hip
@@ -92,6 +92,8 @@
       for (const Layer::SegLaunch* g : {&L.upb_f, &L.upb_b})
         if (g == &L.upb_f || L.upb_bwd)
           UDET_HIP(hipMemcpyAsync(ws + g->tab_off, g->taps.data(), g->taps.size() * sizeof(ConvTap), hipMemcpyHostToDevice, s));
+  P->rec_fin_const_valid = false;
+  UDET_TRY(plan_rec_const_input(P, ws, s));
   UDET_HIP(hipStreamSynchronize(s));
   P->pwc_packed = false;
   return UDET_OK;
diff --git a/unsupervised_detection_amd/csrc/plan_run.h b/unsupervised_detection_amd/csrc/plan_run.h
--- a/unsupervised_detection_amd/csrc/plan_run.h
+++ b/unsupervised_detection_amd/csrc/plan_run.h
@@ -23,8 +23,8 @@
   Emit em;
 };
 inline bool pairs_on(const Plan* P, int dir = 0) { return !P->cfg.conv_fp16 && !((plan_knob(UDET_KNOB_NO_PAIRS) >> dir) & 1); }
-int run_fwd(Plan* P, const Layer& L, int N, float* ws, const Lane& ln);
-int run_fwd_pair(Plan* P, const Layer& La, int Na, const Layer& Lb, int Nb, float* ws, const Lane& ln);
+int run_fwd(Plan* P, const Layer& L, int N, float* ws, const Lane& ln, int n0 = 0);
+int run_fwd_pair(Plan* P, const Layer& La, int Na, const Layer& Lb, int Nb, float* ws, const Lane& ln, int nb0 = 0);
 int run_dgrad(Plan* P, const Layer& L, int N, int dy, bool dy_is_du, int dx, int dx_coff, int accumulate, int res, const Emit& em, float* ws,
               const Lane& ln);
 int run_dgrad_pair(Plan* P, const DgradJob& ja, const DgradJob& jb, float* ws, const Lane& ln);
diff --git a/unsupervised_detection_amd/csrc/plan_step.hip b/unsupervised_detection_amd/csrc/plan_step.hip
--- a/unsupervised_detection_amd/csrc/plan_step.hip
+++ b/unsupervised_detection_amd/csrc/plan_step.hip
@@ -95,9 +95,10 @@
   return UDET_OK;
 }
 
-static int rec_resize(Plan* P, int src, int dst, int N, float* ws, hipStream_t s) {
+static int rec_resize(Plan* P, int src, int dst, int N, float* ws, hipStream_t s, int n0 = 0) {
   const Buf &a = P->buf(src), &b = P->buf(dst);
-  return launch_resize_bilinear_fwd(ws + a.off, a.ld, 0, N, a.h, a.w, ws + b.off, b.ld, 0, b.h, b.w, a.ld, 1.f, 1.f, s);
+  return launch_resize_bilinear_fwd(ws + a.off + (size_t)n0 * a.h * a.w * a.ld, a.ld, 0, N, a.h, a.w, ws + b.off + (size_t)n0 * b.h * b.w * b.ld, b.ld,
+                                    0, b.h, b.w, a.ld, 1.f, 1.f, s);
 }
 static int dec_src(const Resolved& R, int k) { return k == 5 ? R.rec_conv6 : R.rec_concat[k + 1]; }
 
@@ -121,15 +122,37 @@
   return UDET_OK;
 }
 
+static int rec_decoder_forward(Plan* P, int n0, int N, float* ws, const Lane& ln) {
+  const Config& c = P->cfg;
+  const Resolved& R = P->R;
+  hipStream_t s = ln.s;
+  for (int k = 5; k >= 1; --k) {
+    const Layer& dcl = P->rec[R.rec.deconv[k]];
+    if (!dcl.upb) UDET_TRY(rec_resize(P, dec_src(R, k), R.rec_r[k + 1], N, ws, s, n0));
+    UDET_TRY(run_fwd(P, dcl, N, ws, ln, n0));
+    if (k < 5) {
+      UDET_TRY(rec_resize(P, R.rec_flow[k + 1], R.rec_rf[k + 1], N, ws, s, n0));
+      UDET_TRY(run_fwd(P, P->rec[R.rec.upflow[k]], N, ws, ln, n0));
+    }
+    UDET_TRY(run_fwd(P, P->rec[R.rec.flow[k]], N, ws, ln, n0));
+  }
+  const Buf& f1 = P->buf(R.rec_flow[1]);
+  return launch_resize_bilinear_fwd(ws + f1.off + (size_t)n0 * f1.h * f1.w * f1.ld, f1.ld, 0, N, f1.h, f1.w,
+                                    ws + P->buf(R.pred).off + (size_t)n0 * c.img_h * c.img_w * 2, 2, 0, c.img_h, c.img_w, 2, 1.f, 1.f, s);
+}
+
 int plan_recover_forward(Plan* P, int ncalls, float* ws, hipStream_t s, bool inputs_prepacked, bool skip_enc_a, bool enc_a_input_packed) {
   const Config& c = P->cfg;
   const Resolved& R = P->R;
   const int B = c.batch, N = ncalls * B;
   const long Ppix = (long)B * c.img_h * c.img_w;
   const Lane L0 = lane_of(P, s, 0);
-  if (!inputs_prepacked)
+  if (inputs_prepacked) P->rec_fin_const_valid = false;
+  if (!inputs_prepacked) {
     UDET_TRY(launch_mask_rec_inputs(ws + P->buf(R.gen_a17).off, ws + P->buf(R.flow).off, ws + P->buf(R.mask).off, ws + P->buf(R.rec_fin).off,
-                                    Ppix, ncalls, s));
+                                    Ppix, ncalls < 2 ? ncalls : 2, s));
+    if (ncalls == 3) UDET_TRY(plan_rec_const_input(P, ws, s));
+  }
   if (ncalls < 1) return UDET_OK;
   auto enc = [&](int e, int i) -> const Layer& { return P->rec[R.rec.enc[e][i]]; };
   if (!skip_enc_a && pairs_on(P)) {
@@ -151,18 +174,64 @@
     }
     for (int i = 0; i < 9; ++i) UDET_TRY(run_fwd(P, enc(1, i), N, ws, L0));
   }
-  for (int k = 5; k >= 1; --k) {
-    const Layer& dcl = P->rec[R.rec.deconv[k]];
-    if (!dcl.upb) UDET_TRY(rec_resize(P, dec_src(R, k), R.rec_r[k + 1], N, ws, s));
-    UDET_TRY(run_fwd(P, dcl, N, ws, L0));
-    if (k < 5) {
-      UDET_TRY(rec_resize(P, R.rec_flow[k + 1], R.rec_rf[k + 1], N, ws, s));
-      UDET_TRY(run_fwd(P, P->rec[R.rec.upflow[k]], N, ws, L0));
-    }
-    UDET_TRY(run_fwd(P, P->rec[R.rec.flow[k]], N, ws, L0));
-  }
-  const Buf& f1 = P->buf(R.rec_flow[1]);
-  return launch_resize_bilinear_fwd(ws + f1.off, f1.ld, 0, N, f1.h, f1.w, ws + P->buf(R.pred).off, 2, 0, c.img_h, c.img_w, 2, 1.f, 1.f, s);
+  return rec_decoder_forward(P, 0, N, ws, L0);
+}
+
+static int g_rec_call2_split = 0;
+void plan_debug_rec_call2_split(int on) { g_rec_call2_split = on ? 1 : 0; }
+static bool call2_split(int ncalls) { return ncalls == 3 && g_rec_call2_split; }
+
+int plan_rec_const_input(Plan* P, float* ws, hipStream_t s) {
+  if (P->rec_fin_const_valid) return UDET_OK;
+  const long Ppix = (long)P->cfg.batch * P->cfg.img_h * P->cfg.img_w;
+  UDET_TRY(launch_rec_const_input(ws + P->buf(P->R.rec_fin).off + 2 * Ppix * 4, Ppix, s));
+  P->rec_fin_const_valid = true;
+  return UDET_OK;
+}
+
+static int plan_rec_call2(Plan* P, float* ws, const Lane& L0, const Lane& LI, hipEvent_t* e_encA, hipEvent_t* e_call2) {
+  const Resolved& R = P->R;
+  const int B = P->cfg.batch;
+  *e_encA = *e_call2 = nullptr;
+  UDET_TRY(plan_rec_const_input(P, ws, LI.s));
+  UDET_TRY(plan_rec_image_branch(P, 3, ws, LI, false));
+  for (int i = 0; i < 9; ++i) {
+    const Layer& La = P->rec[R.rec.enc[0][i]];
+    UDET_TRY(run_fwd_pair(P, La, B, P->rec[R.rec.enc[1][i]], B, ws, LI, 2 * B));
+    UDET_TRY(share_enc_a_output(P, La, 3, ws, LI.s));
+  }
+  P->enc_a_shared = true;
+  if (LI.s != L0.s) {
+    *e_encA = next_event(P);
+    (void)hipEventRecord(*e_encA, LI.s);
+  }
+  UDET_TRY(rec_decoder_forward(P, 2 * B, B, ws, LI));
+  if (LI.s != L0.s) {
+    *e_call2 = next_event(P);
+    (void)hipEventRecord(*e_call2, LI.s);
+  }
+  return UDET_OK;
+}
+static int plan_rec_calls01(Plan* P, float* ws, const Lane& L0, hipEvent_t e_encA, hipEvent_t e_call2) {
+  const Resolved& R = P->R;
+  const int B = P->cfg.batch;
+  hipStream_t s = L0.s;
+  UDET_TRY(launch_mask_rec_inputs(ws + P->buf(R.gen_a17).off, ws + P->buf(R.flow).off, ws + P->buf(R.mask).off, ws + P->buf(R.rec_fin).off,
+                                  (long)B * P->cfg.img_h * P->cfg.img_w, 2, s));
+  for (int i = 0; i < 9; ++i) UDET_TRY(run_fwd(P, P->rec[R.rec.enc[1][i]], 2 * B, ws, L0));
+  if (e_encA) (void)hipStreamWaitEvent(s, e_encA, 0);
+  UDET_TRY(rec_decoder_forward(P, 0, 2 * B, ws, L0));
+  if (e_call2) (void)hipStreamWaitEvent(s, e_call2, 0);
+  return UDET_OK;
+}
+
+int plan_debug_run_fwd(Plan* P, int net, const char* layer, int n0, int n, float* ws, hipStream_t s) {
+  if (!layer || net < NET_PWC || net > NET_REC) { set_error("debug_run_fwd: bad argument"); return UDET_ERR_ARG; }
+  const std::vector<Layer>& v = net == NET_PWC ? P->pwc : (net == NET_GEN ? P->gen : P->rec);
+  for (const Layer& L : v)
+    if (L.name == layer) return run_fwd(P, L, n, ws, lane_of(P, s, 0), n0);
+  set_error("debug_run_fwd: no layer %s in network %d", layer, net);
+  return UDET_ERR_ARG;
 }
 
 int plan_losses(Plan* P, float* ws, hipStream_t s) {
@@ -202,16 +271,23 @@
     e_img = next_event(P);
     (void)hipEventRecord(e_img, LI.s);
   }
+  const bool split = call2_split(ncalls);
+  hipEvent_t e_encA = nullptr, e_call2 = nullptr;
   const bool paired = pairs_on(P);
-  UDET_TRY(plan_rec_image_branch(P, ncalls, ws, LI, !paired));
+  if (split) UDET_TRY(plan_rec_call2(P, ws, L0, LI, &e_encA, &e_call2));
+  else UDET_TRY(plan_rec_image_branch(P, ncalls, ws, LI, !paired));
   if (img1) {
     UDET_TRY(pwc_forward_on(P, img1, img2, ws, L0, lane_of(P, s, 2)));
     UDET_TRY(plan_prepare_flow(P, P->R.flow, ws, s));
   }
   if (e_img) (void)hipStreamWaitEvent(s, e_img, 0);
   UDET_TRY(plan_generator_forward(P, ws, s));
-  order_after(P, LI, L0);
-  UDET_TRY(plan_recover_forward(P, ncalls, ws, s, false, !paired, paired));
+  if (split) {
+    UDET_TRY(plan_rec_calls01(P, ws, L0, e_encA, e_call2));
+  } else {
+    order_after(P, LI, L0);
+    UDET_TRY(plan_recover_forward(P, ncalls, ws, s, false, !paired, paired));
+  }
   if (ncalls == 3) UDET_TRY(plan_losses(P, ws, s));
   return UDET_OK;
 }
```

Result: no change. 502.4 (-0.1%).
